# microsoft/UniVL

Measured on AMD Instinct MI355X. Metric: video-text pairs/sec (retrieval finetune, 48x48), higher is better.
Workload: dtype bf16; 1 GPU; YouCookII-shape retrieval finetune (FT-Joint) training step: BERT-base text encoder (12 L) + 6-layer visual encoder, max_words=48, max_frames=48, bs=4 per GPU, fwd+bwd+clip+BertAdam, dropout 0.10, random-init weights; kind=joint, per_gpu_batch=4, global_batch=4, max_words=48, max_frames=48, parallelism=dp1, hip_graph=True, graph_mode=whole, optimizer_pipelined=True, optimizer_riding=True, params=152602880

## Files before the change

### include/univl_hip.h

```cpp
#ifndef UNIVL_HIP_H
#define UNIVL_HIP_H
#include <stdint.h>

#ifdef __cplusplus
extern "C" {
#endif

#ifndef __HIP__
typedef struct ihipStream_t* hipStream_t;
#endif

#define UNIVL_DT_F32 0
#define UNIVL_DT_BF16 1

const char* univl_last_error(void);
int univl_version(void);
int univl_struct_size(int which);
int univl_device_info(int* cu_count, char* name, int name_len);
int univl_init(int device);
#define UNIVL_ZERO_MAX 16
int univl_zero_many(void* const* ptrs, const int64_t* bytes, int32_t n, hipStream_t stream);
int univl_copy_many(const void* const* srcs, void* const* dsts, const int64_t* bytes, int32_t n, hipStream_t stream);
int univl_destroy(void);
int univl_set_deterministic(int on);
int univl_get_deterministic(void);
int univl_allreduce_bucket(void* buf, size_t n, int dtype, int average, void* comm, hipStream_t side);

#define UNIVL_GEMM_ACCUM 1
#define UNIVL_GEMM_GELU_FWD 2
#define UNIVL_GEMM_GELU_BWD 4
#define UNIVL_GEMM_ATOMIC 8
#define UNIVL_GEMM_DBIAS_ATOMIC 16
#define UNIVL_GEMM_XCD_MAP 64
#define UNIVL_GEMM_PROBE_NOSTORE 128
#define UNIVL_GEMM_PROBE_NT_B 256
#define UNIVL_GEMM_AUX_F32 512
#define UNIVL_GEMM_NT_OUT 32
typedef struct UnivlGemm {
    int32_t dtype, trans_a, trans_b;
    int32_t M, N, K;
    const void* A; int64_t lda;
    const void* B; int64_t ldb;
    float* C32;
    void* C16;
    int64_t ldc;
    const float* bias;
    const float* R;
    int64_t ldr;
    void* aux;
    int64_t ldaux;
    float* dbias;
    float alpha;
    int32_t flags;
    int32_t ksplit;
    int32_t tile;
    float* sumsq; int32_t sumsq_rows; int32_t sumsq_stride;
    int32_t stages;
    int32_t waves;
    const void* A_lo; const void* B_lo; void* C16_lo;
} UnivlGemm;
int univl_gemm(const UnivlGemm* desc, hipStream_t stream);
#define UNIVL_GEMM_GROUP_MAX 4
int univl_gemm_group(const UnivlGemm* descs, int32_t n, hipStream_t stream);
int univl_gemm_group_limited(const UnivlGemm* d, int n, int max_blocks, hipStream_t stream);
int univl_gemm_pair(const UnivlGemm* dgrad, const UnivlGemm* wgrad, int32_t dry_run, hipStream_t stream);
int univl_gemm_tile_map(int32_t what, int32_t nx, int32_t ny, int32_t nz, int32_t gm, int32_t* out);

int univl_gemm256_layout(int32_t what, int32_t trans, int32_t idx, int32_t arg, int32_t* out);

typedef struct UnivlLayerNorm {
    int32_t dtype;
    int32_t rows, N;
    int32_t x_f64;
    const void* x;
    const float* residual;
    const float* pos;
    int32_t pos_period;
    const float* gamma; const float* beta;
    float eps;
    float* y;
    float* stats;
    float* out32;
    void* out16;
    float p_pre, p_post;
    uint64_t seed, off_pre, off_post;
    const uint64_t* seed_dev;
    const float* dout;
    float* dx32;
    float* dxd32;
    void* dxd16;
    float* dgamma; float* dbeta;
    float* dbias;
    float* dpos;
    void* out16_lo;
} UnivlLayerNorm;
int univl_layernorm_fwd(const UnivlLayerNorm* d, hipStream_t stream);
int univl_layernorm_bwd(const UnivlLayerNorm* d, hipStream_t stream);

typedef struct UnivlAttention {
    int32_t dtype;
    int32_t B, H, Sq, Sk;
    const void* q; int64_t ldq;
    const void* k; int64_t ldk;
    const void* v; int64_t ldv;
    const int64_t* key_mask;
    int32_t causal;
    void* out; int64_t ldo;
    float* lse;
    float p_drop; uint64_t seed, offset;
    const uint64_t* seed_dev;
    const void* dout; int64_t lddo;
    void* dq; int64_t lddq;
    void* dk; int64_t lddk;
    void* dv; int64_t lddv;
    int64_t bsk, bsv;
    void* out_lo;
} UnivlAttention;
int univl_attention_fwd(const UnivlAttention* d, hipStream_t stream);
int univl_attention_bwd(const UnivlAttention* d, hipStream_t stream);

int univl_attention_bwd_fused(const UnivlAttention* at, const UnivlGemm* odgrad, const UnivlGemm* owgrad, int32_t dry_run, hipStream_t stream);

int univl_attention_fwd_fused(const UnivlAttention* at, const UnivlGemm* qkv, const struct UnivlAdam* adam, int32_t chunk_begin,
                              int32_t chunk_count, int32_t max_blocks, int32_t dry_run, hipStream_t stream);

typedef struct UnivlEmbedText {
    int32_t dtype;
    int32_t B, S, N;
    const int64_t* ids; const int64_t* type_ids;
    const float* word; const float* pos; const float* type;
    const float* gamma; const float* beta; float eps;
    float* y; float* stats; float* out32; void* out16;
    float p_post; uint64_t seed, off_post;
    const uint64_t* seed_dev;
    const float* dout;
    float* dword; float* dpos; float* dtype_emb; float* dgamma; float* dbeta;
    float* drows;
    void* out16_lo;
} UnivlEmbedText;
int univl_embed_text_fwd(const UnivlEmbedText* d, hipStream_t stream);
int univl_embed_text_bwd(const UnivlEmbedText* d, hipStream_t stream);
int univl_rows_zero(float* table, int64_t rows_total, const int64_t* list, const int32_t* meta, hipStream_t stream);
int univl_rows_append(const int64_t* ids, int32_t n, int64_t* list, int32_t cap, int32_t* meta, int32_t reset, uint8_t* ever,
                      int64_t rows_total, hipStream_t stream);
int univl_rows_sumsq(const float* table, int64_t rows_total, const int64_t* list, const int32_t* meta, float* out, hipStream_t stream);
int univl_rows_gather_sum(const float* rows, int32_t n_rows, int32_t period, int32_t n, float* out, hipStream_t stream);
int univl_embed_scatter(const int64_t* ids, const float* rows, int64_t n, float scale, float* dword, hipStream_t stream);

typedef struct UnivlPool {
    int32_t B, S, N;
    const float* x; int64_t ldx_row;
    const int64_t* mask;
    int32_t skip_first, normalize;
    float* mean;
    float* out;
    const float* dout;
    float* dx;
    int32_t accumulate;
    const float* dsim; int64_t ldsim; const float* other; int32_t n_other; int32_t transpose; const float* gscale;
} UnivlPool;
int univl_pool_fwd(const UnivlPool* d, hipStream_t stream);
int univl_pool_bwd(const UnivlPool* d, hipStream_t stream);
int univl_pool_pair_fwd(const UnivlPool* a, const UnivlPool* b, hipStream_t stream);
int univl_pool_pair_bwd(const UnivlPool* a, const UnivlPool* b, hipStream_t stream);

int univl_maxmargin_loss(const float* sim, int32_t n, int32_t ld, float margin, const float* weight, float* loss,
                         float* dsim, hipStream_t stream);
int univl_crossen_loss(const float* sim, int32_t n, int32_t ld, float* loss, float* dsim, hipStream_t stream);
int univl_milnce_loss(const float* sim, int32_t batch_size, int32_t n_pair, int32_t ld, float* loss, float* dsim,
                      hipStream_t stream);
int univl_rank_counts(const float* sim, int32_t n, int64_t ld, int32_t* gt, int32_t* eq, hipStream_t stream);
int univl_scale_by_device_scalar(float* x, int64_t n, const float* s, hipStream_t stream);

int univl_pair_concat_fwd(const float* seq, const float* vis, const int64_t* amask, const int64_t* vmask,
                          const int32_t* tidx, const int32_t* vidx, int32_t P, int32_t W, int32_t F, float* out,
                          int64_t* out_mask, hipStream_t stream);
int univl_pair_concat_bwd(const float* dout, const int32_t* tidx, const int32_t* vidx, int32_t P, int32_t W, int32_t F,
                          float* dseq, float* dvis, hipStream_t stream);
int univl_postype_fwd(const float* pos, const float* type, int32_t W, int32_t S, float* out, hipStream_t stream);
int univl_postype_bwd(const float* dtable, int32_t W, int32_t S, float* dpos, float* dtype, hipStream_t stream);
int univl_tanh_fwd(const float* x, float* y, int64_t n, hipStream_t stream);
int univl_tanh_bwd(int32_t dtype, const float* dy, const float* y, void* dx, int64_t n, hipStream_t stream);
int univl_gelu_bwd(int32_t dtype, const float* dg, const void* u, void* du, int64_t n, hipStream_t stream);
int univl_colsum(int32_t dtype, const void* x, int64_t ld, int32_t rows, int32_t n, float* out, hipStream_t stream);
int univl_gather_rows(const void* src, void* dst, const int32_t* idx, int32_t rows, int64_t row_stride, int64_t copy_bytes,
                      hipStream_t stream);
int univl_log_softmax_rows(float* x, int32_t rows, int32_t n, int64_t ld, hipStream_t stream);
#define UNIVL_BEAM_MAX 8
#define UNIVL_BEAM_SLICES 8
typedef struct {
    const float* lp; int64_t ld;
    int32_t n_inst, n_bm, V;
    int32_t first_step;
    int32_t eos;
    const int32_t* eos_dev;
    int32_t t, Tmax;
    float* scores;
    uint8_t* done;
    int32_t* length;
    int64_t* tokens;
    int32_t* src;
    int32_t* hist_parents; int32_t* hist_tokens; float* hist_scores;
    void* ws; int64_t ws_bytes;
} UnivlBeamStep;
int univl_beam_step(const UnivlBeamStep* d, hipStream_t stream);
int univl_beam_backtrack(const int32_t* hist_parents, const int32_t* hist_tokens, const float* scores, const int32_t* length,
                         int32_t n_inst, int32_t n_bm, int32_t n_best, int32_t Tmax, int32_t* hyp, float* hyp_scores,
                         hipStream_t stream);
int univl_beam_captions(const int32_t* hyp, const int32_t* length, int32_t n_inst, int32_t n_best, int32_t Tmax, int32_t eos, int32_t pad,
                        const int32_t* eos_dev, int32_t* cap_tokens, int32_t* cap_len, hipStream_t stream);
#define UNIVL_TOPK_MAX 64
#define UNIVL_TOPK_SLICES_MAX 256
typedef struct UnivlSimTopk {
    const float* q; int64_t ldq;
    const float* g; int64_t ldg;
    int32_t Nq, Ng, H, k;
    int32_t slices;
    int32_t reserved;
    int32_t* idx; float* score;
    const int32_t* target;
    int32_t* gt; int32_t* eq;
    void* ws; int64_t ws_bytes;
} UnivlSimTopk;
int univl_sim_topk(const UnivlSimTopk* d, hipStream_t stream);
int64_t univl_sim_topk_workspace(int32_t Nq, int32_t Ng, int32_t k, int32_t slices);
int univl_sumsq_finish(const float* partials, const int32_t* seg, const int32_t* start, const int32_t* count, int32_t n,
                       float* out, hipStream_t stream);
int univl_scale_ct_by_device_scalar(int32_t dtype, void* x, int64_t n, const float* s, hipStream_t stream);
int univl_simdense_fwd(const float* x, const float* w, const float* b, int32_t rows, float* out, hipStream_t stream);
int univl_simdense_bwd(const float* ds, const float* x, const float* w, int32_t rows, float* dx, float* dw, float* db,
                       hipStream_t stream);
int univl_ce_loss(int32_t dtype, const float* logits, int64_t ld, const int64_t* labels, int32_t rows, int32_t V,
                  int32_t ignore_index, float* scratch2, float* loss, void* dlogits, int64_t lddl, hipStream_t stream);
typedef struct UnivlVocabCE {
    int32_t dtype, rows, V, K;
    const void* x; int64_t ldx;
    const void* table; int64_t ldt;
    const float* bias;
    const int64_t* labels;
    int32_t ignore_index, slots;
    float* partial;
    float* label_logit;
    float* lse;
    float* rowloss;
    float* scratch2;
    float* loss;
    const float* gout;
// ... 58 lines not shown
```

### univl_amd/_ab.py

```python
import os

KEYS = {
    "wgrad_ride": (1, "weight gradients ride in their dgrad's launch (univl_gemm_pair); 0: the layer's grouped launch"),
    "group_wgrad": (1, "a layer's non-riding weight gradients as ONE grouped launch; 0: one launch per member"),
    "pair_form": ("", "'square': round 2's 64 x 64 form of the pair launch"),
    "decoder_pair": (1, "pair launches in the decoder stack"),
    "splitk_tiles": (128, "split the contraction of the N = 768 products while the 64 x 64 output grid has fewer tiles than this"),
    "splitk_len": (384, "target slice depth of that split"),
    "splitk_maxwg": (512, "cap on tiles x slices of that split"),
    "splitk_dgrad_maxwg": (0, "cap on tiles x slices of the dgrad half of a pair launch (0: splitk_maxwg) -- so that dgrad + weight-gradient tiles fit one round of resident slots"),
    "splitk_target_wg": (180, "up to 48 output tiles (256 tokens): split the N = 768 products into round(target / tiles) slices of at least 256 (0: the splitk_len / splitk_maxwg policy of rounds 1-5)"),
    "splitk_target_wg_big": (264, "the same from 49 tiles up to splitk_tiles"),
    "ks_o_fwd": (0, "A/B: slices of the attention-output product (0: policy)"), "ks_ffn2_fwd": (0, "A/B: slices of the FFN2 forward product"),
    "ks_ffn1_dgrad": (0, "A/B: slices of the FFN1 dgrad"), "ks_qkv_dgrad": (0, "A/B: slices of the QKV dgrad"),
    "splitk_mid": (1, "three-slice split of the deep (K >= 2304) N = 768 products at 128 .. 255 tiles"),
    "splitk_mid_ks": (3, "slices of the deep (K >= 2304) N = 768 products in the splitk_mid regime up to 160 tiles"),
    "splitk_mid_ks_big": (2, "... from 161 tiles on"),
    "splitk_mid_ks_768": (1, "slices of the K = 768 N = 768 products in the splitk_mid regime"),
    "splitk_mid_tiles": (256, "upper tile bound of that regime"),
    "ln_fold": (1, "LayerNorm forward finished inside its product's launch (univl_gemm_ln) up to ln_fold_max_rows tokens"),
    "ln_fold_max_rows": (640, "... up to this many tokens (the library carries up to 1024).  Round 6, alternating on one box: 576 tokens 3.00 -> 2.92 ms (-2.6 %, both folds), 624 tokens -1.7 %, 672 +-0, 768 +0.5 % (profiles/r06u_ab_fold_768*.txt); rounds 4-5: 512"),
    "ln_fold_bwd": (1, "LayerNorm backward finished inside the dgrad pair launch (univl_gemm_pair_ln)"),
    "ln_fold_bwd_max": (640, "... up to this many tokens (383: round 4's range, the square pair form only)"),
    "wgrad_big_min": (0, "token count from which a layer's grouped weight gradients take the big tile (0: where every dgrad does)"),
    "attn_fuse_fwd": (1, "the q | k | v projection computed inside the attention forward launch (univl_attention_fwd_fused); 0: two launches"),
    "attn_fuse_bwd": (1, "the attention-output dgrad computed inside the attention backward launch (univl_attention_bwd_fused); 0: two launches"),
    "attn_fuse_fwd_max_seq": (64, "longest sequence the fused attention FORWARD launch is used for.  128: the round-6 form for 65 .. 128 positions (two workgroups per (batch row, head), bit-identical) -- measured NEUTRAL: caption 5.150 vs 5.150 ms, pretrain 9.09 vs 9.09, FT-Align 2.90 vs 2.90 with 18 launches fewer (profiles/r06t_ab_attn_big.txt), so the plans keep the two launches"),
    "attn_fuse_fwd_max_rows": (1536, "token count up to which the fused attention FORWARD launch is used (1536: -1.9 %, 3072: +0.7 %, profiles/r05ae)"),
    "attn_fuse_bwd_max_rows": (1535, "token count up to which the fused attention BACKWARD launch is used (1536: +1 %, 6144: +4.9 %)"),
    "g256": (1, "256 x 256 8-phase body (csrc/gemm256.h) for the grouped weight gradients / single products it is picked for; 0: the older tiles"),
    "g256_min_rows": (1536, "token count (a multiple of 256) from which the plans drop the pair launches for separate dgrads + the grouped 256-body launch"),
    "pairs": ("", "default of model.operand_pairs -- operand PAIRS (bf16 hi + lo, include/univl_hip.h: UnivlGemm.A_lo) in the encoder stacks' forward products: 'x' the activation operand, 'w' the weight operand, 'xw' both, '': plain bf16 operands"),
    "pairs_max_rows": (768, "... in stacks of at most this many tokens (16 pairs x 48): beyond, the matrix pipe is the bound and the extra terms cost step time"),
    "pairs_ks": ("same", "split of a paired N = 768 product: 'same' workgroup count as the plain product (slices nterm x as deep) | 'terms': every term cut like the plain product"),
    "gelu_pre_f32": (0, "A/B measurement: the FFN1 pre-activation saved for GELU' in fp32 instead of the compute type (encoder stacks)"),
    "vocab_ce": (1, "K16: the vocabulary classifier with the online log-softmax CE in its epilogue (univl_vocab_ce_fwd / _bwd: no [tokens, 30522] logits in training); 0: product -> logits -> univl_ce_loss"),
    "vocab_dgrad_split": (1, "split-K of the vocabulary dgrad (caption / pretrain heads)"),
    "fused_sim": (1, "pooling + similarity + loss heads as fused launches up to 256 rows"),
    "dpos_gather_min": (32, "rows per position from which position-table gradients are gathered instead of scatter-added"),
    "beam_step": (1, "caption decoding: Beam.advance as the device-side tail of each position's plan (univl_beam_step) -- CaptionBeamSearch's default beam_step='device'; 0: 'host', the ATen top-k / where path with one host read per position (the comparand)"),
    "adam_ride": ("1", "BertAdam chunks ride with the next forward's products; '0': side-stream form; 'force': one graph even with a captured exchange"),
    "tail_ride": (1, "chunks of cross layer 0 / decoder layer 0 ride in the last text / video layer's products; 0: launched in front of the forward"),
    "adam_lazy_rows": (1, "weight-decay-only shortcut for word-table rows that never had a gradient"),
    "adam_chunk": (0, "A/B: elements per workgroup of the BertAdam update (0: optimization.CHUNK = 8192)"),
    "adam_blocks": (0, "grid cap of the overlapped (non-riding) update"),
    "pipeline_opt": (0, "experimental pipelined optimizer"),
    "async_loss": (0, "experimental asynchronous loss read-back"),
    "fused_norms": (1, "gradient norms from the weight-gradient epilogues"),
    "sparse_rows": (1, "sparse bookkeeping of the word-table gradient"),
    "sparse_emb": (1, "sparse exchange of the word-table gradient under data parallelism"),
    "copy_kernel": (1, "input staging / loss hand-off as one copy kernel"),
    "auto_graph": (1, "the unchanged training loop switches to graph replay on its own"),
    "auto_dp": (1, "wrap in the bucketed reducer on its own when torch.distributed is initialised"),
    "dp_capture": (1, "capture the RCCL exchange into the step graph"),
    "dp_dryrun": (0, "measurement: the data-parallel schedule with the collectives not enqueued"),
    "stamps": (0, "device timestamps between the nodes of the step"),
    "probe_skip": ("", "a stack (bert | visual | cross) without its layer kernels"),
    "probe_no_ln": ("", "fwd | bwd | both: the encoder LayerNorm launches left out"),
    "poison": (0, "workspaces filled with NaN patterns"),
    "guard": (0, "guard words around workspaces"),
}

_allowed = False
_parsed = None
_legacy_checked = False

OPERATIONAL = {"auto_graph": "model.auto_graph = False", "auto_dp": "model.auto_dp = False", "dp_capture": "model.dp_capture = False",
               "adam_ride": "model.auto_ride = False"}


def _check_legacy():
    global _legacy_checked
    if _legacy_checked:
        return
    _legacy_checked = True
    for k in KEYS:
        name = "UNIVL_" + k.upper()
        if name in os.environ:
            how = ("set `%s` on the model (or UNIVL_AB=%s=... in a measurement harness)" % (OPERATIONAL[k], k)) if k in OPERATIONAL \
                else ("use UNIVL_AB=%s=... (measurement / test harnesses only)" % k)
            raise RuntimeError("%s is set but no longer read (it would be silently ignored): %s" % (name, how))


def allow():
    global _allowed
    _allowed = True


def _parse():
    global _parsed
    _check_legacy()
    raw = os.environ.get("UNIVL_AB", "")
    if _parsed is not None and _parsed[0] == raw:
        return _parsed[1]
    out = {}
    for item in [x for x in raw.split(",") if x.strip()]:
        if "=" not in item:
            raise RuntimeError("UNIVL_AB: expected key=value, got %r" % item)
        k, v = (s.strip() for s in item.split("=", 1))
        if k not in KEYS:
            raise RuntimeError("UNIVL_AB: unknown key %r (known: %s)" % (k, ", ".join(sorted(KEYS))))
        d = KEYS[k][0]
        out[k] = type(d)(v) if not isinstance(d, int) else int(v)
    if out and not _allowed:
        raise RuntimeError("UNIVL_AB=%r is set, but this process is not a measurement or test harness (univl_amd._ab.allow()): "
                           "A/B overrides of the plan builder are refused in training / evaluation runs" % raw)
    _parsed = (raw, out)
    return out


def get(key):
    if key not in KEYS:
        raise KeyError("univl_amd._ab: unknown key %r" % key)
    return _parse().get(key, KEYS[key][0])


def overrides():
    return dict(_parse())
```

### univl_amd/_lib.py

```python
import ctypes as C
import os

_HERE = os.path.dirname(os.path.abspath(__file__))
LIB_PATH = os.environ.get("UNIVL_LIB") or os.path.join(_HERE, "lib", "libunivl_hip.so")

DT_F32, DT_BF16 = 0, 1
GEMM_ACCUM, GEMM_GELU_FWD, GEMM_GELU_BWD, GEMM_DBIAS_ATOMIC, GEMM_NT_OUT, GEMM_AUX_F32 = 1, 2, 4, 16, 32, 512
GEMM_GROUP_MAX = 4
EUNSUPPORTED = -3

vp, i32, i64, f32, u64 = C.c_void_p, C.c_int32, C.c_int64, C.c_float, C.c_uint64


class Gemm(C.Structure):
    _fields_ = [("dtype", i32), ("trans_a", i32), ("trans_b", i32), ("M", i32), ("N", i32), ("K", i32),
                ("A", vp), ("lda", i64), ("B", vp), ("ldb", i64), ("C32", vp), ("C16", vp), ("ldc", i64),
                ("bias", vp), ("R", vp), ("ldr", i64), ("aux", vp), ("ldaux", i64), ("dbias", vp),
                ("alpha", f32), ("flags", i32), ("ksplit", i32), ("tile", i32), ("sumsq", vp), ("sumsq_rows", i32), ("sumsq_stride", i32),
                ("stages", i32), ("waves", i32), ("A_lo", vp), ("B_lo", vp), ("C16_lo", vp)]


class LayerNorm(C.Structure):
    _fields_ = [("dtype", i32), ("rows", i32), ("N", i32), ("x_f64", i32), ("x", vp), ("residual", vp),
                ("pos", vp), ("pos_period", i32), ("gamma", vp), ("beta", vp), ("eps", f32), ("y", vp),
                ("stats", vp), ("out32", vp), ("out16", vp), ("p_pre", f32), ("p_post", f32), ("seed", u64),
                ("off_pre", u64), ("off_post", u64), ("seed_dev", vp), ("dout", vp), ("dx32", vp), ("dxd32", vp), ("dxd16", vp),
                ("dgamma", vp), ("dbeta", vp), ("dbias", vp), ("dpos", vp), ("out16_lo", vp)]


class Attention(C.Structure):
    _fields_ = [("dtype", i32), ("B", i32), ("H", i32), ("Sq", i32), ("Sk", i32), ("q", vp), ("ldq", i64),
                ("k", vp), ("ldk", i64), ("v", vp), ("ldv", i64), ("key_mask", vp), ("causal", i32),
                ("out", vp), ("ldo", i64), ("lse", vp), ("p_drop", f32), ("seed", u64), ("offset", u64), ("seed_dev", vp),
                ("dout", vp), ("lddo", i64), ("dq", vp), ("lddq", i64), ("dk", vp), ("lddk", i64),
                ("dv", vp), ("lddv", i64), ("bsk", i64), ("bsv", i64), ("out_lo", vp)]


class EmbedText(C.Structure):
    _fields_ = [("dtype", i32), ("B", i32), ("S", i32), ("N", i32), ("ids", vp), ("type_ids", vp), ("word", vp),
                ("pos", vp), ("type", vp), ("gamma", vp), ("beta", vp), ("eps", f32), ("y", vp), ("stats", vp),
                ("out32", vp), ("out16", vp), ("p_post", f32), ("seed", u64), ("off_post", u64), ("seed_dev", vp), ("dout", vp),
                ("dword", vp), ("dpos", vp), ("dtype_emb", vp), ("dgamma", vp), ("dbeta", vp), ("drows", vp), ("out16_lo", vp)]


class Pool(C.Structure):
    _fields_ = [("B", i32), ("S", i32), ("N", i32), ("x", vp), ("ldx_row", i64), ("mask", vp),
                ("skip_first", i32), ("normalize", i32), ("mean", vp), ("out", vp), ("dout", vp), ("dx", vp), ("accumulate", i32),
                ("dsim", vp), ("ldsim", i64), ("other", vp), ("n_other", i32), ("transpose", i32), ("gscale", vp)]


class Seg(C.Structure):
    _fields_ = [("offset", i64), ("numel", i64), ("lr", f32), ("weight_decay", f32), ("max_grad_norm", f32),
                ("active", i32)]


class Adam(C.Structure):
    _fields_ = [("p", vp), ("g", vp), ("m", vp), ("v", vp), ("p16", vp), ("segs", vp), ("nseg", i32),
                ("chunk_seg", vp), ("chunk_off", vp), ("chunk_len", vp), ("nchunk", i32), ("sumsq", vp),
                ("coef", vp), ("step", vp), ("b1", f32), ("b2", f32), ("eps", f32), ("warmup", f32),
                ("t_total", i32), ("seg_scalars", vp), ("schedule", i32), ("row_flags", vp), ("flag_seg", i32), ("row_len", i32), ("p16_lo", vp)]


class VocabCE(C.Structure):
    _fields_ = [("dtype", i32), ("rows", i32), ("V", i32), ("K", i32), ("x", vp), ("ldx", i64), ("table", vp), ("ldt", i64), ("bias", vp),
                ("labels", vp), ("ignore_index", i32), ("slots", i32), ("partial", vp), ("label_logit", vp), ("lse", vp), ("rowloss", vp),
                ("scratch2", vp), ("loss", vp), ("gout", vp), ("dlogits", vp), ("lddl", i64)]


class BeamStep(C.Structure):
    _fields_ = [("lp", vp), ("ld", i64), ("n_inst", i32), ("n_bm", i32), ("V", i32), ("first_step", i32), ("eos", i32), ("eos_dev", vp),
                ("t", i32), ("Tmax", i32), ("scores", vp), ("done", vp), ("length", vp), ("tokens", vp), ("src", vp), ("hist_parents", vp),
                ("hist_tokens", vp), ("hist_scores", vp), ("ws", vp), ("ws_bytes", i64)]


class SimTopk(C.Structure):
    _fields_ = [("q", vp), ("ldq", i64), ("g", vp), ("ldg", i64), ("Nq", i32), ("Ng", i32), ("H", i32), ("k", i32), ("slices", i32),
                ("reserved", i32), ("idx", vp), ("score", vp), ("target", vp), ("gt", vp), ("eq", vp), ("ws", vp), ("ws_bytes", i64)]


BEAM_MAX, BEAM_SLICES = 8, 8
TOPK_MAX, TOPK_SLICES_MAX = 64, 256

_STRUCTS = [Gemm, LayerNorm, Attention, EmbedText, Pool, Seg, Adam, VocabCE, BeamStep, SimTopk]
_lib = None


def available():
    return os.path.exists(LIB_PATH)


def lib():
    global _lib
    if _lib is not None:
        return _lib
    if not os.path.exists(LIB_PATH):
        raise RuntimeError("libunivl_hip.so not found at %s -- run `python -c 'import __graft_entry__ as g; "
                           "g.build()'` (hipcc --offload-arch=gfx950).  univl_amd has no CPU fallback." % LIB_PATH)
    L = C.CDLL(LIB_PATH)
    L.univl_last_error.restype = C.c_char_p
    L.univl_struct_size.argtypes = [i32]
    for k, st in enumerate(_STRUCTS):
        n = L.univl_struct_size(k)
        if n != C.sizeof(st):
            raise RuntimeError("ABI mismatch for %s: library %d bytes, ctypes %d" % (st.__name__, n, C.sizeof(st)))
    for name in ("univl_vocab_ce_fwd", "univl_vocab_ce_bwd", "univl_gemm", "univl_layernorm_fwd", "univl_layernorm_bwd", "univl_attention_fwd",
                 "univl_attention_bwd", "univl_embed_text_fwd", "univl_embed_text_bwd", "univl_pool_fwd",
                 "univl_pool_bwd", "univl_bert_adam", "univl_beam_step", "univl_sim_topk"):
        getattr(L, name).argtypes = [vp, vp]
        getattr(L, name).restype = i32
    L.univl_pool_pair_fwd.argtypes = [vp, vp, vp]
    L.univl_pool_pair_bwd.argtypes = [vp, vp, vp]
    L.univl_gemm_group.argtypes = [vp, i32, vp]
    L.univl_gemm_group.restype = i32
    L.univl_gemm_group_limited.argtypes = [vp, i32, i32, vp]
    L.univl_gemm_pair.argtypes = [vp, vp, i32, vp]
    L.univl_gemm_rider.argtypes = [vp, vp, i32, i32, i32, vp]
    L.univl_gemm_rider_prime.argtypes = [vp]
    L.univl_gemm_rider_fits.argtypes = [vp]
    L.univl_gemm_ln.argtypes = [vp, vp, vp, vp, i32, i32, i32, i32, vp]
    L.univl_gemm_ln.restype = i32
    L.univl_gemm_pair_ln.argtypes = [vp, vp, vp, vp, i32, vp]
    L.univl_gemm_pair_ln.restype = i32
    L.univl_gemm_tile_map.argtypes = [i32, i32, i32, i32, i32, C.POINTER(i32)]
    L.univl_embed_scatter.argtypes = [vp, vp, i64, f32, vp, vp]
    L.univl_rows_gather_sum.argtypes = [vp, i32, i32, i32, vp, vp]
    L.univl_rows_zero.argtypes = [vp, i64, vp, vp, vp]
    L.univl_rows_append.argtypes = [vp, i32, vp, i32, vp, i32, vp, i64, vp]
    L.univl_rows_sumsq.argtypes = [vp, i64, vp, vp, vp, vp]
    L.univl_zero_many.argtypes = [vp, vp, i32, vp]
    L.univl_copy_many.argtypes = [vp, vp, vp, i32, vp]
    L.univl_maxmargin_loss.argtypes = [vp, i32, i32, f32, vp, vp, vp, vp]
    L.univl_crossen_loss.argtypes = [vp, i32, i32, vp, vp, vp]
    L.univl_milnce_loss.argtypes = [vp, i32, i32, i32, vp, vp, vp]
    L.univl_gather_rows.argtypes = [vp, vp, vp, i32, i64, i64, vp]
    L.univl_log_softmax_rows.argtypes = [vp, i32, i32, i64, vp]
    L.univl_beam_backtrack.argtypes = [vp, vp, vp, vp, i32, i32, i32, i32, vp, vp, vp]
    L.univl_beam_backtrack.restype = i32
    L.univl_beam_captions.argtypes = [vp, vp, i32, i32, i32, i32, i32, vp, vp, vp, vp]
    L.univl_beam_captions.restype = i32
    L.univl_rank_counts.argtypes = [vp, i32, i64, vp, vp, vp]
    L.univl_sim_topk_workspace.argtypes = [i32, i32, i32, i32]
    L.univl_sim_topk_workspace.restype = i64
    L.univl_scale_by_device_scalar.argtypes = [vp, i64, vp, vp]
    L.univl_pair_concat_fwd.argtypes = [vp, vp, vp, vp, vp, vp, i32, i32, i32, vp, vp, vp]
    L.univl_pair_concat_bwd.argtypes = [vp, vp, vp, i32, i32, i32, vp, vp, vp]
    L.univl_postype_fwd.argtypes = [vp, vp, i32, i32, vp, vp]
    L.univl_postype_bwd.argtypes = [vp, i32, i32, vp, vp, vp]
    L.univl_tanh_fwd.argtypes = [vp, vp, i64, vp]
    L.univl_tanh_bwd.argtypes = [i32, vp, vp, vp, i64, vp]
    L.univl_gelu_bwd.argtypes = [i32, vp, vp, vp, i64, vp]
    L.univl_colsum.argtypes = [i32, vp, i64, i32, i32, vp, vp]
    L.univl_scale_ct_by_device_scalar.argtypes = [i32, vp, i64, vp, vp]
    L.univl_simdense_fwd.argtypes = [vp, vp, vp, i32, vp, vp]
    L.univl_simdense_bwd.argtypes = [vp, vp, vp, i32, vp, vp, vp, vp]
    L.univl_ce_loss.argtypes = [i32, vp, i64, vp, i32, i32, i32, vp, vp, vp, i64, vp]
    L.univl_mfm_nce_loss.argtypes = [vp, i64, vp, vp, i32, vp, vp, vp, i64, vp]
    L.univl_grad_sumsq.argtypes = [vp, vp, i32, vp, vp, vp, i32, vp, vp]
    L.univl_sumsq_finish.argtypes = [vp, vp, vp, vp, i32, vp, vp]
    L.univl_clip_coef.argtypes = [vp, vp, i32, f32, vp, vp]
    L.univl_scale_grads.argtypes = [vp, vp, vp, vp, vp, i32, vp, vp]
    L.univl_cast_bf16.argtypes = [vp, vp, i64, vp]
    L.univl_cast_bf16_pair.argtypes = [vp, vp, vp, i64, vp]
    L.univl_cast_f32.argtypes = [vp, vp, i64, vp]
    L.univl_bert_adam_range.argtypes = [vp, i32, i32, i32, i32, vp]
    L.univl_bump_counter.argtypes = [vp, vp]
    L.univl_probe_layouts.argtypes = [vp, i32, vp]
    L.univl_stamp.argtypes = [vp, vp]
    L.univl_device_info.argtypes = [C.POINTER(i32), C.c_char_p, i32]
    L.univl_init.argtypes = [i32]
    L.univl_allreduce_bucket.argtypes = [vp, C.c_size_t, i32, i32, vp, vp]
    L.univl_set_deterministic.argtypes = [i32]
    _lib = L
    return L


def deterministic():
    return bool(lib().univl_get_deterministic())


def set_deterministic(on=True):
    check(lib().univl_set_deterministic(1 if on else 0), "set_deterministic")


EXPORTED = ["univl_last_error", "univl_version", "univl_struct_size", "univl_device_info", "univl_init", "univl_destroy",
            "univl_allreduce_bucket", "univl_set_deterministic", "univl_get_deterministic", "univl_gemm", "univl_gemm_group_limited", "univl_gemm_group", "univl_gemm_tile_map", "univl_gemm256_layout", "univl_gemm_pair", "univl_gemm_rider", "univl_gemm_rider_fits", "univl_gemm_rider_prime", "univl_gemm_ln", "univl_gemm_pair_ln",
            "univl_layernorm_fwd", "univl_layernorm_bwd", "univl_attention_fwd", "univl_attention_bwd", "univl_attention_bwd_fused", "univl_attention_fwd_fused",
            "univl_embed_text_fwd", "univl_embed_text_bwd", "univl_embed_scatter", "univl_rows_gather_sum", "univl_rows_zero", "univl_rows_append",
            "univl_rows_sumsq", "univl_zero_many", "univl_copy_many", "univl_pool_fwd", "univl_pool_bwd", "univl_pool_pair_fwd", "univl_pool_pair_bwd",
            "univl_maxmargin_loss", "univl_crossen_loss", "univl_milnce_loss", "univl_rank_counts", "univl_sim_topk", "univl_sim_topk_workspace", "univl_gather_rows", "univl_log_softmax_rows", "univl_beam_step", "univl_beam_backtrack", "univl_beam_captions", "univl_scale_by_device_scalar", "univl_pair_concat_fwd", "univl_pair_concat_bwd", "univl_postype_fwd", "univl_postype_bwd", "univl_tanh_fwd",
            "univl_tanh_bwd", "univl_gelu_bwd", "univl_colsum", "univl_scale_ct_by_device_scalar", "univl_simdense_fwd", "univl_simdense_bwd", "univl_ce_loss", "univl_vocab_ce_fwd", "univl_vocab_ce_bwd", "univl_mfm_nce_loss", "univl_grad_sumsq", "univl_sumsq_finish",
            "univl_clip_coef", "univl_scale_grads", "univl_bert_adam", "univl_bert_adam_range", "univl_cast_bf16", "univl_cast_bf16_pair", "univl_cast_f32", "univl_bump_counter", "univl_probe_layouts", "univl_stamp"]


def check(rc, what=""):
    if rc != 0:
        raise RuntimeError("libunivl_hip %s failed (%d): %s" % (what, rc, lib().univl_last_error().decode()))
```

### univl_amd/csrc/embed.hip

```cpp
#include "common.h"
#include "univl_hip.h"

namespace {

constexpr int N = 768;
constexpr int NV = N / 256;

template <typename TO>
__global__ __launch_bounds__(256) void embed_fwd_kernel(UnivlEmbedText p) {
    const int lane = threadIdx.x & 63, wave = threadIdx.x >> 6;
    const int row = blockIdx.x * 4 + wave;
    if (row >= p.B * p.S) return;
    const int s = row % p.S;
    const long id = p.ids[row];
    const long tt = (p.type && p.type_ids) ? p.type_ids[row] : 0;
    float v[NV][4];
#pragma unroll
    for (int j = 0; j < NV; ++j) {
        const int col = 4 * lane + 256 * j;
        const float4 a = *reinterpret_cast<const float4*>(p.word + id * N + col);
        const float4 b = *reinterpret_cast<const float4*>(p.pos + (long)s * N + col);
        v[j][0] = a.x + b.x; v[j][1] = a.y + b.y; v[j][2] = a.z + b.z; v[j][3] = a.w + b.w;
        if (p.type) {
            const float4 c = *reinterpret_cast<const float4*>(p.type + tt * N + col);
            v[j][0] += c.x; v[j][1] += c.y; v[j][2] += c.z; v[j][3] += c.w;
        }
        if (p.y) *reinterpret_cast<float4*>(p.y + (long)row * N + col) = make_float4(v[j][0], v[j][1], v[j][2], v[j][3]);
    }
    float sm = 0.f;
#pragma unroll
    for (int j = 0; j < NV; ++j) sm += (v[j][0] + v[j][1]) + (v[j][2] + v[j][3]);
    const float mean = wave_sum(sm) * (1.0f / N);
    float q = 0.f;
#pragma unroll
    for (int j = 0; j < NV; ++j)
#pragma unroll
        for (int e = 0; e < 4; ++e) { const float c = v[j][e] - mean; q += c * c; }
    const float rstd = 1.0f / sqrtf(wave_sum(q) * (1.0f / N) + p.eps);
    if (p.stats && lane == 0) { p.stats[2 * (long)row] = mean; p.stats[2 * (long)row + 1] = rstd; }
    const uint64_t* sp = p.seed_dev ? p.seed_dev : reinterpret_cast<const uint64_t*>(p.gamma);
    const uint64_t sdv = *sp;
    const uint64_t seed = p.seed + (p.seed_dev ? sdv : 0ull);
    const float inv_keep = p.p_post > 0.f ? 1.0f / (1.0f - p.p_post) : 1.0f;
#pragma unroll
    for (int j = 0; j < NV; ++j) {
        const int col = 4 * lane + 256 * j;
        const long o = (long)row * N + col;
        const float4 ga = *reinterpret_cast<const float4*>(p.gamma + col);
        const float4 be = *reinterpret_cast<const float4*>(p.beta + col);
        float r[4];
        r[0] = (v[j][0] - mean) * rstd * ga.x + be.x;
        r[1] = (v[j][1] - mean) * rstd * ga.y + be.y;
        r[2] = (v[j][2] - mean) * rstd * ga.z + be.z;
        r[3] = (v[j][3] - mean) * rstd * ga.w + be.w;
        if (p.p_post > 0.f) {
#pragma unroll
            for (int e = 0; e < 4; ++e) r[e] *= dropout_scale(seed, p.off_post, (uint64_t)(o + e), p.p_post, inv_keep);
        }
        if (p.out32) *reinterpret_cast<float4*>(p.out32 + o) = make_float4(r[0], r[1], r[2], r[3]);
        if (p.out16) {
            TO* d = reinterpret_cast<TO*>(p.out16) + o;
            if (sizeof(TO) == 2) {
                bf16x4_t w;
                w[0] = (__bf16)r[0]; w[1] = (__bf16)r[1]; w[2] = (__bf16)r[2]; w[3] = (__bf16)r[3];
                *reinterpret_cast<bf16x4_t*>(d) = w;
                if (p.out16_lo) {
                    bf16x4_t l;
                    l[0] = (__bf16)(r[0] - (float)w[0]); l[1] = (__bf16)(r[1] - (float)w[1]);
                    l[2] = (__bf16)(r[2] - (float)w[2]); l[3] = (__bf16)(r[3] - (float)w[3]);
                    *reinterpret_cast<bf16x4_t*>(reinterpret_cast<TO*>(p.out16_lo) + o) = l;
                }
            } else {
                *reinterpret_cast<float4*>(d) = make_float4(r[0], r[1], r[2], r[3]);
            }
        }
    }
}

template <bool DET = false>
__global__ __launch_bounds__(256) void embed_bwd_kernel(UnivlEmbedText p, float* det_part = nullptr, int* det_counter = nullptr) {
    __shared__ float red[4][N];
    const int lane = threadIdx.x & 63, wave = threadIdx.x >> 6;
    const int row = blockIdx.x * 4 + wave;
    const bool valid = row < p.B * p.S;
    float dgm[NV][4], dbt[NV][4], dxs[NV][4];
    int row_type = -1;
#pragma unroll
    for (int j = 0; j < NV; ++j)
#pragma unroll
        for (int e = 0; e < 4; ++e) { dgm[j][e] = 0.f; dbt[j][e] = 0.f; dxs[j][e] = 0.f; }
    if (valid) {
        const int s = row % p.S;
        const long id = p.ids[row];
        const long tt = (p.dtype_emb && p.type_ids) ? p.type_ids[row] : 0;
        const float mean = p.stats[2 * (long)row], rstd = p.stats[2 * (long)row + 1];
        const uint64_t* sp = p.seed_dev ? p.seed_dev : reinterpret_cast<const uint64_t*>(p.gamma);
    const uint64_t sdv = *sp;
    const uint64_t seed = p.seed + (p.seed_dev ? sdv : 0ull);
    const float inv_keep = p.p_post > 0.f ? 1.0f / (1.0f - p.p_post) : 1.0f;
        float dy[NV][4], xh[NV][4], ga[NV][4];
        float s1 = 0.f, s2 = 0.f;
#pragma unroll
        for (int j = 0; j < NV; ++j) {
            const int col = 4 * lane + 256 * j;
            const long o = (long)row * N + col;
            const float4 a = *reinterpret_cast<const float4*>(p.dout + o);
            const float4 yy = *reinterpret_cast<const float4*>(p.y + o);
            const float4 gg = *reinterpret_cast<const float4*>(p.gamma + col);
            dy[j][0] = a.x; dy[j][1] = a.y; dy[j][2] = a.z; dy[j][3] = a.w;
            ga[j][0] = gg.x; ga[j][1] = gg.y; ga[j][2] = gg.z; ga[j][3] = gg.w;
            xh[j][0] = (yy.x - mean) * rstd; xh[j][1] = (yy.y - mean) * rstd;
            xh[j][2] = (yy.z - mean) * rstd; xh[j][3] = (yy.w - mean) * rstd;
#pragma unroll
            for (int e = 0; e < 4; ++e) {
                if (p.p_post > 0.f) dy[j][e] *= dropout_scale(seed, p.off_post, (uint64_t)(o + e), p.p_post, inv_keep);
                const float gq = dy[j][e] * ga[j][e];
                s1 += gq; s2 += gq * xh[j][e];
                dgm[j][e] = dy[j][e] * xh[j][e];
                dbt[j][e] = dy[j][e];
            }
        }
        s1 = wave_sum(s1) * (1.0f / N);
        s2 = wave_sum(s2) * (1.0f / N);
#pragma unroll
        for (int j = 0; j < NV; ++j) {
            const int col = 4 * lane + 256 * j;
#pragma unroll
            for (int e = 0; e < 4; ++e) {
                const float dx = rstd * (dy[j][e] * ga[j][e] - s1 - xh[j][e] * s2);
                if (p.drows) p.drows[(long)row * N + col + e] = dx;
                else unsafeAtomicAdd(p.dword + id * N + col + e, dx);
                if (!DET && p.dpos) unsafeAtomicAdd(p.dpos + (long)s * N + col + e, dx);
                if (p.dtype_emb && tt > 1) unsafeAtomicAdd(p.dtype_emb + tt * N + col + e, dx);
                dxs[j][e] = dx;
            }
        }
        row_type = (int)tt;
    }
    if constexpr (DET) {
        __shared__ int last_flag;
        const long nb = gridDim.x;
#pragma unroll
        for (int t = 0; t < 2; ++t) {
            __syncthreads();
#pragma unroll
            for (int j = 0; j < NV; ++j)
#pragma unroll
                for (int e = 0; e < 4; ++e) red[wave][4 * lane + 256 * j + e] = t == 0 ? dgm[j][e] : dbt[j][e];
            __syncthreads();
            float* slot = det_part + ((long)t * nb + blockIdx.x) * N;
            for (int c = threadIdx.x; c < N; c += 256) slot[c] = (red[0][c] + red[1][c]) + (red[2][c] + red[3][c]);
        }
        if (det_last_block(det_counter, (int)nb, &last_flag)) {
#pragma unroll
            for (int t = 0; t < 2; ++t) {
                float* dst = t == 0 ? p.dgamma : p.dbeta;
                for (int c = threadIdx.x; c < N; c += 256) {
                    const float* q = det_part + (long)t * nb * N + c;
                    float acc = 0.f;
                    for (long b = 0; b < nb; ++b) acc += q[b * N];
                    dst[c] += acc;
                }
            }
        }
// ... 19 lines not shown

}

extern "C" int univl_embed_text_fwd(const UnivlEmbedText* d, hipStream_t stream) {
    UNIVL_ON_STREAM_DEVICE(stream);
    UNIVL_CHECK_ARG(d != nullptr, UNIVL_EINVAL, "univl_embed_text_fwd: null descriptor");
    UNIVL_CHECK_ARG(d->N == 768, UNIVL_EUNSUPPORTED, "univl_embed_text_fwd: N=%d (768 supported)", d->N);
    UNIVL_CHECK_ARG(d->B > 0 && d->S > 0 && d->ids && d->word && d->pos && d->gamma && d->beta && (d->out32 || d->out16),
                    UNIVL_EINVAL, "univl_embed_text_fwd: null / empty argument");
    dim3 grid((d->B * d->S + 3) / 4), block(256);
    if (d->dtype == UNIVL_DT_BF16) hipLaunchKernelGGL((embed_fwd_kernel<__bf16>), grid, block, 0, stream, *d);
    else hipLaunchKernelGGL((embed_fwd_kernel<float>), grid, block, 0, stream, *d);
    UNIVL_LAUNCH_CHECK();
    return UNIVL_OK;
}

namespace {
__global__ __launch_bounds__(256) void embed_scatter_det_kernel(const int64_t* ids, const float* rows, long n, float scale, float* dword) {
    const long t = blockIdx.x;
    const int64_t id = ids[t];
    int dup = 0;
    for (long j = threadIdx.x; j < t; j += 256) dup |= (ids[j] == id) ? 1 : 0;
    if (__syncthreads_or(dup)) return;
    float acc[NV] = {0.f, 0.f, 0.f};
    for (long u = t; u < n; ++u) {
        if (ids[u] != id) continue;
#pragma unroll
        for (int j = 0; j < NV; ++j) acc[j] += rows[u * N + threadIdx.x + 256 * j] * scale;
    }
#pragma unroll
    for (int j = 0; j < NV; ++j) dword[id * N + threadIdx.x + 256 * j] += acc[j];
}

__global__ __launch_bounds__(256) void embed_dpos_gather_kernel(const float* rows, int B, int S, float* dpos) {
    const long i = (long)blockIdx.x * 256 + threadIdx.x;
    if (i >= (long)S * N) return;
    const int s = (int)(i / N), c = (int)(i % N);
    float acc = 0.f;
    for (int b = 0; b < B; ++b) acc += rows[((long)b * S + s) * N + c];
    dpos[i] += acc;
}

__global__ __launch_bounds__(256) void embed_dtype_gather_kernel(const int64_t* type_ids, const float* rows, long n, float* dtype_emb) {
    const int c = blockIdx.x * 256 + threadIdx.x, k = blockIdx.y;
    float acc = 0.f;
    for (long t = 0; t < n; ++t) {
        const int64_t tt = type_ids ? type_ids[t] : 0;
        if (tt == k) acc += rows[t * N + c];
    }
    if (acc != 0.0f) dtype_emb[(long)k * N + c] += acc;
}

__global__ __launch_bounds__(256) void embed_scatter_kernel(const int64_t* ids, const float* rows, float scale, float* dword) {
    const long t = blockIdx.x;
    const long id = ids[t];
    for (int c = threadIdx.x; c < N; c += 256) unsafeAtomicAdd(dword + id * N + c, rows[t * N + c] * scale);
}
}

extern "C" int univl_embed_scatter(const int64_t* ids, const float* rows, int64_t n, float scale, float* dword, hipStream_t stream) {
    UNIVL_ON_STREAM_DEVICE(stream);
    UNIVL_CHECK_ARG(ids && rows && dword && n > 0, UNIVL_EINVAL, "univl_embed_scatter: bad argument");
    if (univl_deterministic()) hipLaunchKernelGGL(embed_scatter_det_kernel, dim3((unsigned)n), dim3(256), 0, stream, ids, rows, (long)n, scale, dword);
    else hipLaunchKernelGGL(embed_scatter_kernel, dim3((unsigned)n), dim3(256), 0, stream, ids, rows, scale, dword);
    UNIVL_LAUNCH_CHECK();
    return UNIVL_OK;
}

namespace {
constexpr int ROWS_GRID = 8192;

__global__ __launch_bounds__(256) void rows_zero_kernel(float* table, long rows_total, const int64_t* list, const int* meta) {
    const int n = meta[0], over = meta[1];
    if (!over && (int)blockIdx.x >= n) return;
    for (long r = over ? blockIdx.x : list[blockIdx.x]; r < rows_total; r += ROWS_GRID) {
        float4* p = reinterpret_cast<float4*>(table + r * N);
        for (int c = threadIdx.x; c < N / 4; c += 256) p[c] = float4{0.f, 0.f, 0.f, 0.f};
        if (!over) break;
    }
}

__global__ __launch_bounds__(256) void rows_append_kernel(const int64_t* ids, int n, int64_t* list, int cap, int* meta, int reset,
                                                          uint8_t* ever, long rows_total) {
    __shared__ int base, over;
    if (threadIdx.x == 0) {
        const int cur = reset ? 0 : meta[0];
        int ov = reset ? 0 : meta[1];
        if (cur + n > cap) ov = 1;
        base = cur; over = ov;
        meta[1] = ov;
        meta[0] = ov ? cur : cur + n;
    }
    __syncthreads();
    if (!over) for (int i = threadIdx.x; i < n; i += 256) list[base + i] = ids[i];
    if (ever) {
        if (over) for (long r = threadIdx.x; r < rows_total; r += 256) ever[r] = 1;
        else for (int i = threadIdx.x; i < n; i += 256) ever[ids[i]] = 1;
    }
}

__global__ __launch_bounds__(256) void rows_sumsq_kernel(const float* table, long rows_total, const int64_t* list, const int* meta,
                                                         float* out, float* det_part) {
    __shared__ float red[4];
    const int n = meta[0], over = meta[1];
    if (!over && (int)blockIdx.x >= n) { if (det_part && threadIdx.x == 0) det_part[blockIdx.x] = 0.f; return; }
    float acc = 0.f;
    if (over) {
        for (long r = blockIdx.x; r < rows_total; r += ROWS_GRID) {
            const float4* p = reinterpret_cast<const float4*>(table + r * N);
            for (int c = threadIdx.x; c < N / 4; c += 256) { const float4 v = p[c]; acc += (v.x * v.x + v.y * v.y) + (v.z * v.z + v.w * v.w); }
        }
    } else {
        const int64_t r = list[blockIdx.x];
        int dup = 0;
        for (int j = threadIdx.x; j < (int)blockIdx.x; j += 256) dup |= (list[j] == r) ? 1 : 0;
        if (__syncthreads_or(dup)) { if (det_part && threadIdx.x == 0) det_part[blockIdx.x] = 0.f; return; }
        const float4* p = reinterpret_cast<const float4*>(table + r * N);
        for (int c = threadIdx.x; c < N / 4; c += 256) { const float4 v = p[c]; acc += (v.x * v.x + v.y * v.y) + (v.z * v.z + v.w * v.w); }
    }
    acc = wave_sum(acc);
    if ((threadIdx.x & 63) == 0) red[threadIdx.x >> 6] = acc;
    __syncthreads();
    if (threadIdx.x == 0) {
        const float s = (red[0] + red[1]) + (red[2] + red[3]);
        if (det_part) det_part[blockIdx.x] = s;
        else unsafeAtomicAdd(out, s);
    }
}

__global__ __launch_bounds__(256) void rows_sumsq_finish_kernel(const float* part, int n, float* out) {
    __shared__ float red[4];
    float acc = 0.f;
    for (int i = threadIdx.x; i < n; i += 256) acc += part[i];
    acc = wave_sum(acc);
    if ((threadIdx.x & 63) == 0) red[threadIdx.x >> 6] = acc;
    __syncthreads();
    if (threadIdx.x == 0) out[0] += (red[0] + red[1]) + (red[2] + red[3]);
}
}

extern "C" int univl_rows_zero(float* table, int64_t rows_total, const int64_t* list, const int32_t* meta, hipStream_t stream) {
    UNIVL_ON_STREAM_DEVICE(stream);
    UNIVL_CHECK_ARG(table && list && meta && rows_total > 0 && aligned16(table), UNIVL_EINVAL, "univl_rows_zero: bad argument");
    hipLaunchKernelGGL(rows_zero_kernel, dim3(ROWS_GRID), dim3(256), 0, stream, table, (long)rows_total, list, meta);
    UNIVL_LAUNCH_CHECK();
    return UNIVL_OK;
}

extern "C" int univl_rows_append(const int64_t* ids, int32_t n, int64_t* list, int32_t cap, int32_t* meta, int32_t reset,
                                 uint8_t* ever, int64_t rows_total, hipStream_t stream) {
    UNIVL_ON_STREAM_DEVICE(stream);
    UNIVL_CHECK_ARG(ids && list && meta && n > 0 && cap > 0 && cap <= ROWS_GRID && (!ever || rows_total > 0), UNIVL_EINVAL,
                    "univl_rows_append: bad argument (cap <= %d)", ROWS_GRID);
    hipLaunchKernelGGL(rows_append_kernel, dim3(1), dim3(256), 0, stream, ids, n, list, cap, meta, reset, ever, (long)rows_total);
    UNIVL_LAUNCH_CHECK();
    return UNIVL_OK;
}

extern "C" int univl_rows_sumsq(const float* table, int64_t rows_total, const int64_t* list, const int32_t* meta, float* out,
                                hipStream_t stream) {
    UNIVL_ON_STREAM_DEVICE(stream);
    UNIVL_CHECK_ARG(table && list && meta && out && rows_total > 0 && aligned16(table), UNIVL_EINVAL, "univl_rows_sumsq: bad argument");
    float* part = nullptr;
    if (univl_deterministic()) {
        part = static_cast<float*>(univl_det_alloc(ROWS_GRID * sizeof(float)));
        if (!part) return UNIVL_EINVAL;
    }
    hipLaunchKernelGGL(rows_sumsq_kernel, dim3(ROWS_GRID), dim3(256), 0, stream, table, (long)rows_total, list, meta, out, part);
    if (part) hipLaunchKernelGGL(rows_sumsq_finish_kernel, dim3(1), dim3(256), 0, stream, part, ROWS_GRID, out);
    UNIVL_LAUNCH_CHECK();
    return UNIVL_OK;
}

extern "C" int univl_embed_text_bwd(const UnivlEmbedText* d, hipStream_t stream) {
    UNIVL_ON_STREAM_DEVICE(stream);
    UNIVL_CHECK_ARG(d != nullptr, UNIVL_EINVAL, "univl_embed_text_bwd: null descriptor");
    UNIVL_CHECK_ARG(d->N == 768, UNIVL_EUNSUPPORTED, "univl_embed_text_bwd: N=%d (768 supported)", d->N);
    UNIVL_CHECK_ARG(d->B > 0 && d->S > 0 && d->ids && d->dout && d->y && d->stats && d->gamma && d->dword && (d->dpos || d->drows) &&
                        d->dgamma && d->dbeta,
                    UNIVL_EINVAL, "univl_embed_text_bwd: null / empty argument");
    dim3 grid((d->B * d->S + 3) / 4), block(256);
    if (univl_deterministic()) {
        UnivlEmbedText q = *d;
        const long T = (long)d->B * d->S;
        float* part = static_cast<float*>(univl_det_alloc((size_t)2 * grid.x * N * sizeof(float)));
        int* counter = univl_det_counter();
        if (!part || !counter) return UNIVL_EINVAL;
        if (!q.drows) {
            q.drows = static_cast<float*>(univl_det_alloc((size_t)T * N * sizeof(float)));
            if (!q.drows) return UNIVL_EINVAL;
        }
        hipLaunchKernelGGL(embed_bwd_kernel<true>, grid, block, 0, stream, q, part, counter);
        if (!d->drows)
            hipLaunchKernelGGL(embed_scatter_det_kernel, dim3((unsigned)T), block, 0, stream, d->ids, q.drows, T, 1.0f, d->dword);
        if (d->dpos)
            hipLaunchKernelGGL(embed_dpos_gather_kernel, dim3((unsigned)(((long)d->S * N + 255) / 256)), block, 0, stream, q.drows, d->B, d->S, d->dpos);
        if (d->dtype_emb)
            hipLaunchKernelGGL(embed_dtype_gather_kernel, dim3(N / 256, 2), block, 0, stream, d->type_ids, q.drows, T, d->dtype_emb);
        UNIVL_LAUNCH_CHECK();
        return UNIVL_OK;
    }
    hipLaunchKernelGGL(embed_bwd_kernel<false>, grid, block, 0, stream, *d);
    UNIVL_LAUNCH_CHECK();
    return UNIVL_OK;
}
```

### univl_amd/csrc/misc.hip

```cpp
#include <stdarg.h>
#include <stdio.h>
#include <string.h>
#include <dlfcn.h>
#include <stdlib.h>
#include "common.h"
#include "univl_hip.h"

static thread_local char g_err[512] = "";

void univl_set_error(const char* fmt, ...) {
    va_list ap;
    va_start(ap, fmt);
    vsnprintf(g_err, sizeof(g_err), fmt, ap);
    va_end(ap);
}

extern "C" const char* univl_last_error(void) { return g_err; }
extern "C" int univl_version(void) { return 100; }

extern "C" int univl_struct_size(int which) {
    switch (which) {
        case 0: return (int)sizeof(UnivlGemm);
        case 1: return (int)sizeof(UnivlLayerNorm);
        case 2: return (int)sizeof(UnivlAttention);
        case 3: return (int)sizeof(UnivlEmbedText);
        case 4: return (int)sizeof(UnivlPool);
        case 5: return (int)sizeof(UnivlSeg);
        case 6: return (int)sizeof(UnivlAdam);
        case 7: return (int)sizeof(UnivlVocabCE);
        case 8: return (int)sizeof(UnivlBeamStep);
        case 9: return (int)sizeof(UnivlSimTopk);
        default: return -1;
    }
}

extern "C" int univl_device_info(int* cu_count, char* name, int name_len) {
    int dev = 0;
    hipError_t e = hipGetDevice(&dev);
    if (e != hipSuccess) { univl_set_error("hipGetDevice: %s", hipGetErrorString(e)); return (int)e; }
    hipDeviceProp_t prop;
    e = hipGetDeviceProperties(&prop, dev);
    if (e != hipSuccess) { univl_set_error("hipGetDeviceProperties: %s", hipGetErrorString(e)); return (int)e; }
    if (cu_count) *cu_count = prop.multiProcessorCount;
    if (name && name_len > 0) { strncpy(name, prop.gcnArchName, name_len - 1); name[name_len - 1] = 0; }
    return 0;
}

#include <mutex>
namespace {
struct DetArena { unsigned char* base = nullptr; size_t size = 0, head = 0; int* counters = nullptr; int next_counter = 0; };
constexpr int DET_COUNTERS = 1 << 16;
DetArena g_det[UNIVL_MAX_DEVICES];
std::mutex g_det_mutex;
int g_deterministic = 0;

DetArena* det_arena() {
    int dev = 0;
    if (hipGetDevice(&dev) != hipSuccess || dev < 0 || dev >= UNIVL_MAX_DEVICES) return nullptr;
    DetArena& a = g_det[dev];
    if (a.base == nullptr) {
        const char* e = getenv("UNIVL_DET_ARENA_MB");
        const size_t mb = e ? (size_t)atol(e) : 1024;
        void* p = nullptr;
        void* c = nullptr;
        if (hipMalloc(&p, mb << 20) != hipSuccess) { (void)hipGetLastError(); return nullptr; }
        if (hipMalloc(&c, DET_COUNTERS * sizeof(int)) != hipSuccess || hipMemset(c, 0, DET_COUNTERS * sizeof(int)) != hipSuccess ||
            hipDeviceSynchronize() != hipSuccess) {
            (void)hipGetLastError(); (void)hipFree(p); if (c) (void)hipFree(c); return nullptr;
        }
        a.base = static_cast<unsigned char*>(p); a.size = mb << 20; a.head = 0;
        a.counters = static_cast<int*>(c); a.next_counter = 0;
    }
    return &a;
}
}

bool univl_deterministic() { return g_deterministic != 0; }

void* univl_det_alloc(size_t bytes) {
    std::lock_guard<std::mutex> lock(g_det_mutex);
    DetArena* a = det_arena();
    bytes = (bytes + 255) & ~(size_t)255;
    if (a == nullptr || bytes > a->size / 4) {
        univl_set_error("deterministic mode: no scratch ring on this device (call univl_set_deterministic(1) on it outside a stream "
                        "capture; a single request must fit a quarter of UNIVL_DET_ARENA_MB), %zu bytes asked", bytes);
        return nullptr;
    }
    if (a->head + bytes > a->size) a->head = 0;
    void* p = a->base + a->head;
    a->head += bytes;
    return p;
}

int* univl_det_counter() {
    std::lock_guard<std::mutex> lock(g_det_mutex);
    DetArena* a = det_arena();
    if (a == nullptr) { univl_set_error("deterministic mode: no counter pool on this device"); return nullptr; }
    int* c = a->counters + a->next_counter;
    a->next_counter = (a->next_counter + 1) % DET_COUNTERS;
    return c;
}

extern "C" int univl_set_deterministic(int on) {
    std::lock_guard<std::mutex> lock(g_det_mutex);
    g_deterministic = on ? 1 : 0;
    if (on && det_arena() == nullptr) {
        univl_set_error("univl_set_deterministic: cannot allocate the scratch ring (UNIVL_DET_ARENA_MB) on the current device");
        return UNIVL_EINVAL;
    }
    return UNIVL_OK;
}

extern "C" int univl_get_deterministic(void) { return g_deterministic; }

namespace {
struct ZeroList { unsigned char* ptr[UNIVL_ZERO_MAX]; long bytes[UNIVL_ZERO_MAX]; };
__global__ __launch_bounds__(256) void zero_many_kernel(ZeroList z) {
    unsigned char* p = z.ptr[blockIdx.y];
    const long n16 = z.bytes[blockIdx.y] >> 4;
    u32x4_t* q = reinterpret_cast<u32x4_t*>(p);
    for (long i = (long)blockIdx.x * 256 + threadIdx.x; i < n16; i += (long)gridDim.x * 256) q[i] = u32x4_t{0u, 0u, 0u, 0u};
    if (blockIdx.x == 0) for (long i = (n16 << 4) + threadIdx.x; i < z.bytes[blockIdx.y]; i += 256) p[i] = 0;
}
}

extern "C" int univl_zero_many(void* const* ptrs, const int64_t* bytes, int32_t n, hipStream_t stream) {
    UNIVL_ON_STREAM_DEVICE(stream);
    UNIVL_CHECK_ARG(ptrs && bytes && n >= 1 && n <= UNIVL_ZERO_MAX, UNIVL_EINVAL, "univl_zero_many: n=%d (1..%d)", n, UNIVL_ZERO_MAX);
    ZeroList z;
    long most = 0;
    for (int i = 0; i < n; ++i) {
        UNIVL_CHECK_ARG(ptrs[i] && bytes[i] > 0 && aligned16(ptrs[i]), UNIVL_EALIGN, "univl_zero_many: buffer %d must be non-empty and 16-byte aligned", i);
        z.ptr[i] = static_cast<unsigned char*>(ptrs[i]);
        z.bytes[i] = bytes[i];
        most = bytes[i] > most ? bytes[i] : most;
    }
    long gx = (most / 16 + 2047) / 2048;
    gx = gx < 1 ? 1 : (gx > 1024 ? 1024 : gx);
    hipLaunchKernelGGL(zero_many_kernel, dim3((unsigned)gx, n), dim3(256), 0, stream, z);
    UNIVL_LAUNCH_CHECK();
    return UNIVL_OK;
}

namespace {
struct CopyList { const unsigned char* src[UNIVL_ZERO_MAX]; unsigned char* dst[UNIVL_ZERO_MAX]; long bytes[UNIVL_ZERO_MAX]; };
__global__ __launch_bounds__(256) void copy_many_kernel(CopyList c) {
    const unsigned char* s = c.src[blockIdx.y];
    unsigned char* d = c.dst[blockIdx.y];
    const long nb = c.bytes[blockIdx.y];
    const bool vec = ((((uintptr_t)s) | ((uintptr_t)d)) & 15) == 0;
    const long n16 = vec ? (nb >> 4) : 0;
    const u32x4_t* sv = reinterpret_cast<const u32x4_t*>(s);
    u32x4_t* dv = reinterpret_cast<u32x4_t*>(d);
    for (long i = (long)blockIdx.x * 256 + threadIdx.x; i < n16; i += (long)gridDim.x * 256) dv[i] = sv[i];
    if (blockIdx.x == 0) for (long i = (n16 << 4) + threadIdx.x; i < nb; i += 256) d[i] = s[i];
}
}

extern "C" int univl_copy_many(const void* const* srcs, void* const* dsts, const int64_t* bytes, int32_t n, hipStream_t stream) {
    UNIVL_ON_STREAM_DEVICE(stream);
    UNIVL_CHECK_ARG(srcs && dsts && bytes && n >= 1 && n <= UNIVL_ZERO_MAX, UNIVL_EINVAL, "univl_copy_many: n=%d (1..%d)", n, UNIVL_ZERO_MAX);
    CopyList c;
    long most = 0;
    for (int i = 0; i < n; ++i) {
        UNIVL_CHECK_ARG(srcs[i] && dsts[i] && bytes[i] > 0, UNIVL_EINVAL, "univl_copy_many: buffer %d is null or empty", i);
        c.src[i] = static_cast<const unsigned char*>(srcs[i]);
        c.dst[i] = static_cast<unsigned char*>(dsts[i]);
        c.bytes[i] = bytes[i];
        most = bytes[i] > most ? bytes[i] : most;
    }
    for (int i = n; i < UNIVL_ZERO_MAX; ++i) { c.src[i] = c.src[0]; c.dst[i] = c.dst[0]; c.bytes[i] = 0; }
    long gx = (most / 16 + 1023) / 1024;
    gx = gx < 1 ? 1 : (gx > 2048 ? 2048 : gx);
    hipLaunchKernelGGL(copy_many_kernel, dim3((unsigned)gx, n), dim3(256), 0, stream, c);
    UNIVL_LAUNCH_CHECK();
    return UNIVL_OK;
}

extern "C" int univl_init(int device) {
    int n = 0;
    hipError_t e = hipGetDeviceCount(&n);
    if (e != hipSuccess) { univl_set_error("hipGetDeviceCount: %s", hipGetErrorString(e)); return (int)e; }
    UNIVL_CHECK_ARG(device >= 0 && device < n, UNIVL_EINVAL, "univl_init: device %d of %d", device, n);
    hipDeviceProp_t prop;
    e = hipGetDeviceProperties(&prop, device);
    if (e != hipSuccess) { univl_set_error("hipGetDeviceProperties: %s", hipGetErrorString(e)); return (int)e; }
    UNIVL_CHECK_ARG(strncmp(prop.gcnArchName, "gfx950", 6) == 0, UNIVL_EUNSUPPORTED,
                    "univl_init: device %d is %s; libunivl_hip holds gfx950 (MI355X) code only", device, prop.gcnArchName);
    return UNIVL_OK;
}

typedef int (*nccl_allreduce_fn)(const void*, void*, size_t, int, int, void*, hipStream_t);
static void* g_rccl_handle = nullptr;
static nccl_allreduce_fn g_allreduce = nullptr;

extern "C" int univl_destroy(void) {
    {
        std::lock_guard<std::mutex> lock(g_det_mutex);
        for (DetArena& a : g_det) {
            if (a.base) (void)hipFree(a.base);
            if (a.counters) (void)hipFree(a.counters);
            a = DetArena();
        }
    }
    g_allreduce = nullptr;
    if (g_rccl_handle) { dlclose(g_rccl_handle); g_rccl_handle = nullptr; }
    return UNIVL_OK;
}

extern "C" int univl_allreduce_bucket(void* buf, size_t n, int dtype, int average, void* comm, hipStream_t side) {
    UNIVL_ON_STREAM_DEVICE(side);
    UNIVL_CHECK_ARG(buf && comm && n > 0 && (dtype == UNIVL_F32 || dtype == UNIVL_BF16), UNIVL_EINVAL,
                    "univl_allreduce_bucket: bad argument");
    if (!g_allreduce) {
        void* sym = dlsym(RTLD_DEFAULT, "ncclAllReduce");
        if (!sym) {
            for (const char* name : {"librccl.so.1", "librccl.so", "/opt/rocm/lib/librccl.so.1"}) {
                g_rccl_handle = dlopen(name, RTLD_NOW | RTLD_LOCAL);
                if (g_rccl_handle) break;
            }
            if (g_rccl_handle) sym = dlsym(g_rccl_handle, "ncclAllReduce");
        }
// ... 78 lines not shown
```

### univl_amd/csrc/simloss.hip

```cpp
#include "common.h"
#include "univl_hip.h"

namespace {

__device__ __forceinline__ float block_sum(float v, float* red) {
    v = wave_sum(v);
    const int lane = threadIdx.x & 63, wave = threadIdx.x >> 6;
    __syncthreads();
    if (lane == 0) red[wave] = v;
    __syncthreads();
    return (red[0] + red[1]) + (red[2] + red[3]);
}
__device__ __forceinline__ float block_max(float v, float* red) {
    v = wave_max(v);
    const int lane = threadIdx.x & 63, wave = threadIdx.x >> 6;
    __syncthreads();
    if (lane == 0) red[wave] = v;
    __syncthreads();
    return fmaxf(fmaxf(red[0], red[1]), fmaxf(red[2], red[3]));
}

constexpr int PN = 768, PC = PN / 256;

__device__ __forceinline__ float pool_weight(const UnivlPool& p, int b, int s) {
    float w = p.mask ? (float)p.mask[(long)b * p.S + s] : 1.0f;
    if (p.skip_first && s == 0) w = 0.0f;
    return w;
}

constexpr int PCHUNK = 256;

__device__ __forceinline__ float stage_weights(const UnivlPool& p, int b, int s0, float* wts, float* red) {
    const int s = s0 + threadIdx.x;
    const float w = (s < p.S) ? pool_weight(p, b, s) : 0.0f;
    wts[threadIdx.x] = w;
    return block_sum(w, red);
}

__device__ __forceinline__ void pool_fwd_body(const UnivlPool& p, const int b, float* red, float* wts) {
    const int t = threadIdx.x;
    float acc[PC] = {0.f, 0.f, 0.f};
    float cnt = 0.f;
    for (int s0 = 0; s0 < p.S; s0 += PCHUNK) {
        cnt += stage_weights(p, b, s0, wts, red);
        const int n = min(PCHUNK, p.S - s0);
        const float* x = p.x + ((long)b * p.S + s0) * p.ldx_row + t;
#pragma unroll 8
        for (int s = 0; s < n; ++s) {
            const float w = wts[s];
#pragma unroll
            for (int j = 0; j < PC; ++j) {
                const float v = x[(long)s * p.ldx_row + 256 * j];
                acc[j] += (w != 0.0f) ? v * w : 0.0f;
            }
        }
        __syncthreads();
    }
    if (!p.skip_first && cnt == 0.0f) cnt = 1.0f;
    float sq = 0.f;
#pragma unroll
    for (int j = 0; j < PC; ++j) { acc[j] /= cnt; sq += acc[j] * acc[j]; }
    float inv = 1.0f;
    if (p.normalize) inv = 1.0f / fmaxf(sqrtf(block_sum(sq, red)), 1e-12f);
#pragma unroll
    for (int j = 0; j < PC; ++j) {
        if (p.mean) p.mean[(long)b * PN + t + 256 * j] = acc[j];
        p.out[(long)b * PN + t + 256 * j] = acc[j] * inv;
    }
}

__global__ __launch_bounds__(256) void pool_fwd_kernel(UnivlPool p) {
    __shared__ float red[4];
    __shared__ float wts[PCHUNK];
    pool_fwd_body(p, blockIdx.x, red, wts);
}

__global__ __launch_bounds__(256) void pool_pair_fwd_kernel(UnivlPool a, UnivlPool b) {
    __shared__ float red[4];
    __shared__ float wts[PCHUNK];
    if ((int)blockIdx.x < a.B) pool_fwd_body(a, blockIdx.x, red, wts);
    else pool_fwd_body(b, (int)blockIdx.x - a.B, red, wts);
}

__device__ __forceinline__ void pool_bwd_body(const UnivlPool& p, const int b, const int chunk, float* red, float* wts, float* mine) {
    const int t = threadIdx.x;
    if (chunk * PCHUNK >= p.S) return;
    float cnt = 0.f;
    for (int s0 = 0; s0 < p.S; s0 += PCHUNK) {
        cnt += stage_weights(p, b, s0, wts, red);
        if (s0 == chunk * PCHUNK) mine[t] = wts[t];
        __syncthreads();
    }
    if (!p.skip_first && cnt == 0.0f) cnt = 1.0f;
    float m[PC], d[PC];
    float sq = 0.f, dot = 0.f;
#pragma unroll
    for (int j = 0; j < PC; ++j) {
        m[j] = p.mean[(long)b * PN + t + 256 * j];
        d[j] = p.dsim ? 0.0f : p.dout[(long)b * PN + t + 256 * j];
    }
    if (p.dsim) {
        const float gs = p.gscale ? p.gscale[0] : 1.0f;
        for (int k = 0; k < p.n_other; ++k) {
            const float w = p.transpose ? p.dsim[(long)k * p.ldsim + b] : p.dsim[(long)b * p.ldsim + k];
#pragma unroll
            for (int j = 0; j < PC; ++j) d[j] += w * p.other[(long)k * PN + t + 256 * j];
        }
#pragma unroll
        for (int j = 0; j < PC; ++j) d[j] *= gs;
    }
#pragma unroll
    for (int j = 0; j < PC; ++j) {
        sq += m[j] * m[j];
        dot += m[j] * d[j];
    }
    if (p.normalize) {
        const float nrm = fmaxf(sqrtf(block_sum(sq, red)), 1e-12f);
        const float dd = block_sum(dot, red) / (nrm * nrm);
#pragma unroll
        for (int j = 0; j < PC; ++j) d[j] = (d[j] - m[j] * dd) / nrm;
    }
    const float inv_cnt = 1.0f / cnt;
    const int s0 = chunk * PCHUNK, n = min(PCHUNK, p.S - s0);
    float* dx = p.dx + ((long)b * p.S + s0) * PN + t;
    if (p.accumulate) {
        constexpr int UB = 8;
        for (int s0b = 0; s0b < n; s0b += UB) {
            float old[UB][PC];
#pragma unroll
            for (int u = 0; u < UB; ++u) {
                const int s = min(s0b + u, n - 1);
#pragma unroll
                for (int j = 0; j < PC; ++j) old[u][j] = dx[(long)s * PN + 256 * j];
            }
#pragma unroll
            for (int u = 0; u < UB; ++u) {
                const int s = s0b + u;
                if (s < n) {
                    const float w = mine[s] * inv_cnt;
#pragma unroll
                    for (int j = 0; j < PC; ++j) dx[(long)s * PN + 256 * j] = old[u][j] + d[j] * w;
                }
            }
        }
    } else {
#pragma unroll 4
        for (int s = 0; s < n; ++s) {
            const float w = mine[s] * inv_cnt;
#pragma unroll
            for (int j = 0; j < PC; ++j) dx[(long)s * PN + 256 * j] = d[j] * w;
        }
    }
}

__global__ __launch_bounds__(256) void pool_bwd_kernel(UnivlPool p) {
    __shared__ float red[4];
    __shared__ float wts[PCHUNK];
    __shared__ float mine[PCHUNK];
    pool_bwd_body(p, blockIdx.x, blockIdx.y, red, wts, mine);
}

__global__ __launch_bounds__(256) void pool_pair_bwd_kernel(UnivlPool a, UnivlPool b) {
    __shared__ float red[4];
    __shared__ float wts[PCHUNK];
    __shared__ float mine[PCHUNK];
    if ((int)blockIdx.x < a.B) pool_bwd_body(a, blockIdx.x, blockIdx.y, red, wts, mine);
    else pool_bwd_body(b, (int)blockIdx.x - a.B, blockIdx.y, red, wts, mine);
}

__global__ __launch_bounds__(256) void maxmargin_kernel(const float* x, int n, int ld, float margin, const float* w,
                                                        float* loss, float* dx) {
    extern __shared__ float diag_acc[];
    __shared__ float red[4];
    const float inv = 1.0f / ((float)n * (float)n);
    for (int i = threadIdx.x; i < n; i += 256) diag_acc[i] = 0.f;
    __syncthreads();
    float acc = 0.f;
    for (int e = threadIdx.x; e < n * n; e += 256) {
        const int i = e / n, j = e % n;
        const float v = x[(long)i * ld + j], wi = w ? w[e] : 1.0f;
        const float a = margin + v - x[(long)i * ld + i];
        const float b = margin + v - x[(long)j * ld + j];
        float g = 0.f;
        if (a > 0.f) { acc += wi * a; g += wi; atomicAdd(&diag_acc[i], -wi); }
        if (b > 0.f) { acc += wi * b; g += wi; atomicAdd(&diag_acc[j], -wi); }
        dx[(long)i * ld + j] = g * inv;
    }
    const float total = block_sum(acc, red);
    if (threadIdx.x == 0) loss[0] = total * inv;
    __syncthreads();
    for (int i = threadIdx.x; i < n; i += 256) dx[(long)i * ld + i] += diag_acc[i] * inv;
}

__global__ __launch_bounds__(256) void crossen_kernel(const float* x, int n, int ld, float* loss, float* dx) {
    __shared__ float red[4];
    float total = 0.f;
    for (int i = 0; i < n; ++i) {
        float mx = -INFINITY;
        for (int j = threadIdx.x; j < n; j += 256) mx = fmaxf(mx, x[(long)i * ld + j]);
        mx = block_max(mx, red);
        float s = 0.f;
        for (int j = threadIdx.x; j < n; j += 256) s += expf(x[(long)i * ld + j] - mx);
        s = block_sum(s, red);
        const float lse = mx + logf(s);
        total += lse - x[(long)i * ld + i];
        for (int j = threadIdx.x; j < n; j += 256)
            dx[(long)i * ld + j] = (expf(x[(long)i * ld + j] - lse) - (i == j ? 1.0f : 0.0f)) / (float)n;
    }
    if (threadIdx.x == 0) loss[0] = total / (float)n;
}

__global__ __launch_bounds__(256) void milnce_kernel(const float* x, int bs, int np, int ld, float* loss, float* dx) {
    __shared__ float red[4];
    const int n = bs * np;
    for (int e = threadIdx.x; e < n * n; e += 256) dx[(long)(e / n) * ld + (e % n)] = 0.f;
    __syncthreads();
    float total = 0.f;
    for (int bb = 0; bb < bs; ++bb) {
        const int i = bb * np + np / 2;
        const int lo = bb * np, hi = lo + np;
        float mx = -INFINITY;
        for (int j = threadIdx.x; j < 2 * n; j += 256) {
            float v;
            if (j < n) v = x[(long)j * ld + i];
            else { const int jj = j - n; v = (jj >= lo && jj < hi) ? -INFINITY : x[(long)i * ld + jj]; }
            mx = fmaxf(mx, v);
        }
        mx = block_max(mx, red);
        float sden = 0.f, snum = 0.f;
        for (int j = threadIdx.x; j < 2 * n; j += 256) {
            if (j < n) {
                const float e = expf(x[(long)j * ld + i] - mx);
                sden += e;
                if (j >= lo && j < hi) snum += e;
            } else {
                const int jj = j - n;
                if (!(jj >= lo && jj < hi)) sden += expf(x[(long)i * ld + jj] - mx);
            }
        }
        sden = block_sum(sden, red);
        snum = block_sum(snum, red);
        total += logf(sden) - logf(snum);
        const float wgt = 1.0f / (float)bs;
        __syncthreads();
        for (int j = threadIdx.x; j < 2 * n; j += 256) {
            if (j < n) {
                const float e = expf(x[(long)j * ld + i] - mx);
                float g = e / sden;
                if (j >= lo && j < hi) g -= e / snum;
                dx[(long)j * ld + i] += wgt * g;
            }
        }
        __syncthreads();
        for (int j = threadIdx.x; j < n; j += 256) {
            if (!(j >= lo && j < hi)) dx[(long)i * ld + j] += wgt * expf(x[(long)i * ld + j] - mx) / sden;
        }
        __syncthreads();
    }
    if (threadIdx.x == 0) loss[0] = total / (float)bs;
}

__global__ void scale_dev_kernel(float* x, long n, const float* s) {
    const float k = s[0];
    for (long i = (long)blockIdx.x * 256 + threadIdx.x; i < n; i += (long)gridDim.x * 256) x[i] *= k;
}

}

extern "C" int univl_scale_by_device_scalar(float* x, int64_t n, const float* s, hipStream_t stream) {
    UNIVL_ON_STREAM_DEVICE(stream);
    UNIVL_CHECK_ARG(x && s && n > 0, UNIVL_EINVAL, "univl_scale_by_device_scalar: bad argument");
    long blocks = (n + 255) / 256;
    if (blocks > 1024) blocks = 1024;
    hipLaunchKernelGGL(scale_dev_kernel, dim3((unsigned)blocks), dim3(256), 0, stream, x, (long)n, s);
    UNIVL_LAUNCH_CHECK();
    return UNIVL_OK;
}

__global__ __launch_bounds__(256) void rank_counts_kernel(const float* x, int n, long ld, int* gt, int* eq) {
    __shared__ int red[8];
    const int i = blockIdx.x, t = threadIdx.x;
    const float* row = x + (long)i * ld;
    const float d = row[i];
    int g = 0, e = 0;
    for (int j = t; j < n; j += 256) {
        const float v = row[j];
        g += v > d ? 1 : 0;
        e += v == d ? 1 : 0;
    }
#pragma unroll
    for (int o = 32; o > 0; o >>= 1) { g += __shfl_down(g, o, 64); e += __shfl_down(e, o, 64); }
    if ((t & 63) == 0) { red[t >> 6] = g; red[4 + (t >> 6)] = e; }
    __syncthreads();
    if (t == 0) {
        gt[i] = (red[0] + red[1]) + (red[2] + red[3]);
        eq[i] = (red[4] + red[5]) + (red[6] + red[7]);
    }
}

extern "C" int univl_rank_counts(const float* sim, int32_t n, int64_t ld, int32_t* gt, int32_t* eq, hipStream_t stream) {
    UNIVL_ON_STREAM_DEVICE(stream);
    UNIVL_CHECK_ARG(sim && gt && eq && n > 0 && ld >= n, UNIVL_EINVAL, "univl_rank_counts: bad argument");
    hipLaunchKernelGGL(rank_counts_kernel, dim3(n), dim3(256), 0, stream, sim, n, (long)ld, gt, eq);
    UNIVL_LAUNCH_CHECK();
    return UNIVL_OK;
}

extern "C" int univl_pool_fwd(const UnivlPool* d, hipStream_t stream) {
    UNIVL_ON_STREAM_DEVICE(stream);
    UNIVL_CHECK_ARG(d && d->N == 768 && d->B > 0 && d->S > 0 && d->x && d->out, UNIVL_EINVAL, "univl_pool_fwd: bad argument (N must be 768)");
    hipLaunchKernelGGL(pool_fwd_kernel, dim3(d->B), dim3(256), 0, stream, *d);
    UNIVL_LAUNCH_CHECK();
    return UNIVL_OK;
}

static int pool_bwd_check(const UnivlPool* d, const char* who) {
    UNIVL_CHECK_ARG(d && d->N == 768 && d->B > 0 && d->S > 0 && d->mean && d->dx && (d->dout || (d->dsim && d->other && d->n_other > 0)),
                    UNIVL_EINVAL, "%s: bad argument", who);
    return UNIVL_OK;
}

extern "C" int univl_pool_bwd(const UnivlPool* d, hipStream_t stream) {
    UNIVL_ON_STREAM_DEVICE(stream);
    const int rc = pool_bwd_check(d, "univl_pool_bwd");
    if (rc) return rc;
    hipLaunchKernelGGL(pool_bwd_kernel, dim3(d->B, (d->S + PCHUNK - 1) / PCHUNK), dim3(256), 0, stream, *d);
    UNIVL_LAUNCH_CHECK();
    return UNIVL_OK;
}

extern "C" int univl_pool_pair_fwd(const UnivlPool* a, const UnivlPool* b, hipStream_t stream) {
    UNIVL_ON_STREAM_DEVICE(stream);
    UNIVL_CHECK_ARG(a && b && a->N == 768 && b->N == 768 && a->B > 0 && b->B > 0 && a->S > 0 && b->S > 0 && a->x && b->x && a->out && b->out,
                    UNIVL_EINVAL, "univl_pool_pair_fwd: bad argument (N must be 768)");
    hipLaunchKernelGGL(pool_pair_fwd_kernel, dim3(a->B + b->B), dim3(256), 0, stream, *a, *b);
    UNIVL_LAUNCH_CHECK();
    return UNIVL_OK;
}

extern "C" int univl_pool_pair_bwd(const UnivlPool* a, const UnivlPool* b, hipStream_t stream) {
    UNIVL_ON_STREAM_DEVICE(stream);
    int rc = pool_bwd_check(a, "univl_pool_pair_bwd");
    if (rc) return rc;
    rc = pool_bwd_check(b, "univl_pool_pair_bwd");
    if (rc) return rc;
    const int smax = a->S > b->S ? a->S : b->S;
    hipLaunchKernelGGL(pool_pair_bwd_kernel, dim3(a->B + b->B, (smax + PCHUNK - 1) / PCHUNK), dim3(256), 0, stream, *a, *b);
    UNIVL_LAUNCH_CHECK();
    return UNIVL_OK;
}

extern "C" int univl_maxmargin_loss(const float* sim, int32_t n, int32_t ld, float margin, const float* weight, float* loss,
                                    float* dsim, hipStream_t stream) {
    UNIVL_ON_STREAM_DEVICE(stream);
    UNIVL_CHECK_ARG(sim && loss && dsim && n > 0 && n <= 8192 && ld >= n, UNIVL_EINVAL, "univl_maxmargin_loss: bad argument");
    hipLaunchKernelGGL(maxmargin_kernel, dim3(1), dim3(256), n * sizeof(float), stream, sim, n, ld, margin, weight, loss, dsim);
    UNIVL_LAUNCH_CHECK();
    return UNIVL_OK;
}

extern "C" int univl_crossen_loss(const float* sim, int32_t n, int32_t ld, float* loss, float* dsim, hipStream_t stream) {
    UNIVL_ON_STREAM_DEVICE(stream);
    UNIVL_CHECK_ARG(sim && loss && dsim && n > 0 && ld >= n, UNIVL_EINVAL, "univl_crossen_loss: bad argument");
    hipLaunchKernelGGL(crossen_kernel, dim3(1), dim3(256), 0, stream, sim, n, ld, loss, dsim);
    UNIVL_LAUNCH_CHECK();
    return UNIVL_OK;
}

extern "C" int univl_milnce_loss(const float* sim, int32_t batch_size, int32_t n_pair, int32_t ld, float* loss, float* dsim,
                                 hipStream_t stream) {
    UNIVL_ON_STREAM_DEVICE(stream);
    UNIVL_CHECK_ARG(sim && loss && dsim && batch_size > 0 && n_pair > 0 && ld >= batch_size * n_pair, UNIVL_EINVAL, "univl_milnce_loss: bad argument");
    hipLaunchKernelGGL(milnce_kernel, dim3(1), dim3(256), 0, stream, sim, batch_size, n_pair, ld, loss, dsim);
    UNIVL_LAUNCH_CHECK();
    return UNIVL_OK;
}
```

### univl_amd/engine.py

```python
import contextlib
import ctypes as C
import gc
import os
import weakref

import torch

from . import _ab, _lib, ops

@contextlib.contextmanager
def no_gc():
    was = gc.isenabled()
    gc.disable()
    try:
        yield
    finally:
        if was:
            gc.enable()


GUARDED = []


def _workspace(dev, zeros=False):
# ... 181 lines not shown
                ops.cast_bf16_pair(self.p32, self.p16, self.p16lo)
            else:
                ops.cast_bf16(self.p32, self.p16)
        self.shadow_valid = True

    def attach_grads(self, used_names):
        for n in used_names:
            p, gv = self.params[n], self.g(n)
            if p.grad is not gv:
                p.grad = gv


class GradState:

    def __init__(self, flat, fresh, fuse_sumsq=False):
        self.flat, self.fresh, self.written = flat, fresh, set()
        self.fuse_sumsq, self.covered = bool(fuse_sumsq), set()
        self.slots, self.entries = 0, []

    def sumsq_args(self, names, rows_per_tensor, cols):
        if isinstance(names, str):
            names = [names]
        if not self.fuse_sumsq or any(self.flat.is_atomic(n) for n in names) or rows_per_tensor % 128 != 0:
            return {}
        if any(n in self.covered for n in names):
            raise RuntimeError("fused gradient norms: %s has a second writer in this backward" % (names,))
        self.covered.update(names)
        stride = (rows_per_tensor // 64) * ((cols + 63) // 64) * 4
        start = self.slots
        for t, n in enumerate(names):
            self.entries.append((self.flat.seg_of[n], start + t * stride, stride))
        self.slots += stride * len(names)
        if self.slots > self.flat.partials.numel():
            raise RuntimeError("fused gradient norms: partial-sum buffer too small")
        return dict(sumsq=self.flat.partials[start:], sumsq_rows=rows_per_tensor if len(names) > 1 else 0, sumsq_stride=stride)

    def acc(self, name):
        if self.flat.is_atomic(name):
            return True
        a = (not self.fresh) or (name in self.written)
        self.written.add(name)
        return a

    def finish(self, plan):
        if not self.entries:
            return
        dev = self.flat.device
        seg, start, count = (torch.tensor(x, dtype=torch.int32, device=dev) for x in zip(*self.entries))
        out = self.flat.sumsq
        plan.add_callable(lambda: ops.sumsq_finish(self.flat.partials, seg, start, count, out))


class Plan:

    def __init__(self):
        self.ops = []
        self.keep = []
        self.descs = {}
        self.external = {}
        self._side = {}
        self._segments = None
        self.rider_keys = set()
        self.riders = None

    def add_gemm_rider(self, desc, key, slot, nslots, stream=0):
        self.keep.append(desc)
        self.descs[len(self.ops)] = [desc]
        self.rider_keys.add(key)
        self.ops.append(("rider", _lib.lib().univl_gemm_rider, (desc, key, int(slot), int(nslots)), "univl_gemm_rider", stream))

    def add_gemm_ln(self, desc, ln_desc, counters, key=None, slot=0, nslots=1, stream=0):
        self.keep += [desc, ln_desc, counters]
        self.descs[len(self.ops)] = [desc]
        if key is not None:
            self.rider_keys.add(key)
        self.ops.append(("gemm_ln", _lib.lib().univl_gemm_ln, (desc, ln_desc, counters, key, int(slot), int(nslots)), "univl_gemm_ln", stream))

    def add(self, fn_name, desc, stream=0):
        fn = getattr(_lib.lib(), fn_name)
        self.keep.append(desc)
        self.descs[len(self.ops)] = [desc]
        self.ops.append(("call", fn, C.byref(desc), fn_name, stream))

    def add_pair_call(self, fn_name, da, db, stream=0):
        fn = getattr(_lib.lib(), fn_name)
        self.keep += [da, db]
        self.descs[len(self.ops)] = [da, db]
        self.ops.append(("call2", fn, (da, db), fn_name, stream))

    def add_gemm_group(self, descs, stream=0, max_blocks=0):
        fn = _lib.lib().univl_gemm_group_limited
        if not _ab.get("group_wgrad"):
            for d in descs:
                self.add("univl_gemm", d, stream)
            return
        for i in range(0, len(descs), _lib.GEMM_GROUP_MAX):
            chunk = descs[i:i + _lib.GEMM_GROUP_MAX]
            arr = (_lib.Gemm * len(chunk))(*chunk)
            self.keep.append(arr)
            self.descs[len(self.ops)] = list(chunk)
            self.ops.append(("group", fn, (arr, len(chunk), int(max_blocks)), "univl_gemm_group", stream))

    def add_gemm_pair(self, dgrad, wgrad, stream=0):
        fn = _lib.lib().univl_gemm_pair
        arr = (_lib.Gemm * 2)(dgrad, wgrad)
        self.keep.append(arr)
        self.descs[len(self.ops)] = [dgrad, wgrad]
        self.ops.append(("pair", fn, arr, "univl_gemm_pair", stream))

    def add_attn_fwd_fused(self, attn, qkv, key=None, slot=0, nslots=1, stream=0):
        self.keep += [attn, qkv]
        self.descs[len(self.ops)] = [qkv]
        if key is not None:
            self.rider_keys.add(key)
        self.ops.append(("attn_fwd_fused", _lib.lib().univl_attention_fwd_fused, (attn, qkv, key, int(slot), int(nslots)), "univl_attention_fwd_fused", stream))

    def add_attn_bwd_fused(self, attn, odgrad, owgrad, stream=0):
        self.keep += [attn, odgrad, owgrad]
        self.descs[len(self.ops)] = [odgrad] + ([owgrad] if owgrad is not None else [])
        self.ops.append(("attn_fused", _lib.lib().univl_attention_bwd_fused, (attn, odgrad, owgrad), "univl_attention_bwd_fused", stream))

    def add_gemm_pair_ln(self, dgrad, wgrad, ln_desc, counters, stream=0):
        arr = (_lib.Gemm * 2)(dgrad, wgrad)
        self.keep += [arr, ln_desc, counters]
        self.descs[len(self.ops)] = [dgrad, wgrad]
        self.ops.append(("pair_ln", _lib.lib().univl_gemm_pair_ln, (arr, ln_desc, counters), "univl_gemm_pair_ln", stream))

    def add_zeros(self, tensors, stream=0):
        ts = [t for t in tensors if t is not None and t.numel() > 0]
        if ts:
            self.add_callable(lambda: ops.zero_many(ts), stream)

    def add_callable(self, f, stream=0, eager=False, with_streams=False):
        kind = "eager" if eager else ("pys" if with_streams else "py")
        self.ops.append((kind, f, None, getattr(f, "__name__", "callable"), stream))

    def wait_point(self, key, stream=0):
        self.ops.append(("wait", key, None, "wait", stream))

    def record(self, key, stream=0):
        self.ops.append(("record", key, None, "record", stream))

    def fork(self, src, dst):
        if src != dst:
            self.ops.append(("dep", src, dst, "dep", 0))

    def join(self, src, dst):
        self.fork(src, dst)

    def _stream(self, idx, cur):
        if idx == 0:
            return cur
        st = self._side.get(idx)
        if st is None or st.device != cur.device:
            st = torch.cuda.Stream(device=cur.device)
            self._side[idx] = st
        return st

    def _run_ops(self, ops_, cur, forked=None):
        handles, events = {}, {}
        forked = set() if forked is None else set(forked)
        for op in ops_:
            kind, a, b, name, sidx = op
            if kind == "call":
                h = handles.get(sidx)
                if h is None:
                    h = handles[sidx] = C.c_void_p(self._stream(sidx, cur).cuda_stream)
                rc = a(b, h)
                if rc != 0:
                    _lib.check(rc, name)
            elif kind == "call2":
                h = handles.get(sidx)
                if h is None:
                    h = handles[sidx] = C.c_void_p(self._stream(sidx, cur).cuda_stream)
                rc = a(C.byref(b[0]), C.byref(b[1]), h)
                if rc != 0:
                    _lib.check(rc, name)
            elif kind == "group":
                h = handles.get(sidx)
                if h is None:
                    h = handles[sidx] = C.c_void_p(self._stream(sidx, cur).cuda_stream)
                rc = a(b[0], b[1], b[2], h)
                if rc != 0:
                    _lib.check(rc, name)
            elif kind == "rider":
                h = handles.get(sidx)
                if h is None:
                    h = handles[sidx] = C.c_void_p(self._stream(sidx, cur).cuda_stream)
                desc, key, slot, nslots = b
                rd = self.riders
                rng = rd["ranges"].get(key) if rd else None
                if rng is not None and (key, slot) in rd["used"]:
                    rng = None
                if rng is None:
                    rc = _lib.lib().univl_gemm(C.byref(desc), h)
                else:
                    rd["used"].add((key, slot))
                    lo, hi = rng[0] + rng[1] * slot // nslots, rng[0] + rng[1] * (slot + 1) // nslots
                    rc = a(C.byref(desc), C.byref(rd["desc"]), lo, hi - lo, int(rd.get("max_blocks", 0)), h)
                if rc != 0:
                    _lib.check(rc, name)
            elif kind == "gemm_ln":
                h = handles.get(sidx)
                if h is None:
                    h = handles[sidx] = C.c_void_p(self._stream(sidx, cur).cuda_stream)
                desc, lnd, ctr, key, slot, nslots = b
                rd = self.riders
                rng = rd["ranges"].get(key) if (rd and key is not None) else None
                if rng is not None and (key, slot) in rd["used"]:
                    rng = None
                L_ = _lib.lib()
                if rng is None:
                    rc = a(C.byref(desc), C.byref(lnd), C.c_void_p(ctr.data_ptr()), None, 0, 0, 0, 0, h)
                    if rc == _lib.EUNSUPPORTED:
                        rc = L_.univl_gemm(C.byref(desc), h) or L_.univl_layernorm_fwd(C.byref(lnd), h)
                else:
                    rd["used"].add((key, slot))
                    lo, hi = rng[0] + rng[1] * slot // nslots, rng[0] + rng[1] * (slot + 1) // nslots
                    rc = a(C.byref(desc), C.byref(lnd), C.c_void_p(ctr.data_ptr()), C.byref(rd["desc"]), lo, hi - lo, int(rd.get("max_blocks", 0)), 0, h)
                    if rc == _lib.EUNSUPPORTED:
                        rc = (L_.univl_gemm_rider(C.byref(desc), C.byref(rd["desc"]), lo, hi - lo, int(rd.get("max_blocks", 0)), h)
                              or L_.univl_layernorm_fwd(C.byref(lnd), h))
                if rc != 0:
                    _lib.check(rc, name)
            elif kind == "pair_ln":
                h = handles.get(sidx)
                if h is None:
                    h = handles[sidx] = C.c_void_p(self._stream(sidx, cur).cuda_stream)
                arr, lnd, ctr = b
                rc = a(C.byref(arr[0]), C.byref(arr[1]), C.byref(lnd), C.c_void_p(ctr.data_ptr()), 0, h)
                if rc == _lib.EUNSUPPORTED:
                    rc = _lib.lib().univl_gemm_pair(C.byref(arr[0]), C.byref(arr[1]), 0, h) or _lib.lib().univl_layernorm_bwd(C.byref(lnd), h)
                if rc != 0:
                    _lib.check(rc, name)
            elif kind == "pair":
                h = handles.get(sidx)
                if h is None:
                    h = handles[sidx] = C.c_void_p(self._stream(sidx, cur).cuda_stream)
                rc = a(C.byref(b[0]), C.byref(b[1]), 0, h)
                if rc != 0:
                    _lib.check(rc, name)
            elif kind == "attn_fwd_fused":
                h = handles.get(sidx)
                if h is None:
                    h = handles[sidx] = C.c_void_p(self._stream(sidx, cur).cuda_stream)
                at, qd, key, slot, nslots = b
                rd = self.riders
                rng = rd["ranges"].get(key) if (rd and key is not None) else None
                if rng is not None and (key, slot) in rd["used"]:
                    rng = None
                if rng is None:
                    rc = a(C.byref(at), C.byref(qd), None, 0, 0, 0, 0, h)
                else:
                    rd["used"].add((key, slot))
                    lo, hi = rng[0] + rng[1] * slot // nslots, rng[0] + rng[1] * (slot + 1) // nslots
                    rc = a(C.byref(at), C.byref(qd), C.byref(rd["desc"]), lo, hi - lo, int(rd.get("max_blocks", 0)), 0, h)
                if rc != 0:
                    _lib.check(rc, name)
# ... 637 lines not shown
```

### univl_amd/ops.py

```python
import ctypes as C

import torch

from . import _lib
from ._lib import DT_BF16, DT_F32

_BYREF = C.byref


def _stream():
    return C.c_void_p(torch.cuda.current_stream().cuda_stream)


def _p(t):
    return None if t is None else C.c_void_p(t.data_ptr())


def dtype_code(dtype):
    if dtype == torch.float32:
        return DT_F32
    if dtype == torch.bfloat16:
        return DT_BF16
    raise RuntimeError("univl_amd: unsupported compute dtype %s (float32 or bfloat16)" % dtype)

# ... 84 lines not shown
    rc = _lib.lib().univl_gemm_pair_ln(_BYREF(dgrad), _BYREF(wgrad), _BYREF(ln), C.c_void_p(counters.data_ptr()), int(bool(dry_run)), _stream())
    if rc == _lib.EUNSUPPORTED:
        return False
    _lib.check(rc, "gemm_pair_ln")
    return True


def layernorm_desc(dtype, rows, N, *, x=None, x_f64=False, residual=None, pos=None, pos_period=0, gamma=None,
                   beta=None, eps=1e-12, y=None, stats=None, out32=None, out16=None, p_pre=0.0, p_post=0.0, seed=0,
                   off_pre=0, off_post=0, seed_dev=None, dout=None, dx32=None, dxd32=None, dxd16=None, dgamma=None,
                   dbeta=None, dbias=None, dpos=None, out16_lo=None):
    d = _lib.LayerNorm()
    d.dtype, d.rows, d.N, d.x_f64 = dtype, rows, N, int(x_f64)
    d.x, d.residual, d.pos, d.pos_period = _p(x), _p(residual), _p(pos), pos_period
    d.gamma, d.beta, d.eps = _p(gamma), _p(beta), eps
    d.y, d.stats, d.out32, d.out16 = _p(y), _p(stats), _p(out32), _p(out16)
    d.p_pre, d.p_post, d.seed, d.off_pre, d.off_post, d.seed_dev = p_pre, p_post, seed, off_pre, off_post, _p(seed_dev)
    d.dout, d.dx32, d.dxd32, d.dxd16 = _p(dout), _p(dx32), _p(dxd32), _p(dxd16)
    d.dgamma, d.dbeta, d.dbias, d.dpos = _p(dgamma), _p(dbeta), _p(dbias), _p(dpos)
    d.out16_lo = _p(out16_lo)
    return d


def layernorm_fwd(**kw):
    d = layernorm_desc(**kw)
    _lib.check(_lib.lib().univl_layernorm_fwd(_BYREF(d), _stream()), "layernorm_fwd")


def layernorm_bwd(**kw):
    d = layernorm_desc(**kw)
    _lib.check(_lib.lib().univl_layernorm_bwd(_BYREF(d), _stream()), "layernorm_bwd")


def attention_desc(dtype, B, H, Sq, Sk, q, ldq, k, ldk, v, ldv, out, ldo, lse, *, key_mask=None, causal=False,
                   p_drop=0.0, seed=0, offset=0, seed_dev=None, dout=None, lddo=0, dq=None, lddq=0, dk=None, lddk=0,
                   dv=None, lddv=0, bsk=0, bsv=0, out_lo=None):
    def ptr(t):
        if t is None:
            return None
        if isinstance(t, tuple):
            return C.c_void_p(t[0].data_ptr() + t[1] * t[0].element_size())
        return C.c_void_p(t.data_ptr())
    d = _lib.Attention()
    d.dtype, d.B, d.H, d.Sq, d.Sk = dtype, B, H, Sq, Sk
    d.q, d.ldq, d.k, d.ldk, d.v, d.ldv = ptr(q), ldq, ptr(k), ldk, ptr(v), ldv
    d.key_mask, d.causal = _p(key_mask), int(causal)
    d.out, d.ldo, d.lse = ptr(out), ldo, _p(lse)
    d.p_drop, d.seed, d.offset, d.seed_dev = p_drop, seed, offset, _p(seed_dev)
    d.dout, d.lddo, d.dq, d.lddq, d.dk, d.lddk, d.dv, d.lddv = ptr(dout), lddo, ptr(dq), lddq, ptr(dk), lddk, ptr(dv), lddv
    d.bsk, d.bsv = bsk, bsv
    d.out_lo = ptr(out_lo)
    return d


def attention_fwd(*a, **kw):
    d = attention_desc(*a, **kw)
    _lib.check(_lib.lib().univl_attention_fwd(_BYREF(d), _stream()), "attention_fwd")


def attention_bwd(*a, **kw):
    d = attention_desc(*a, **kw)
    _lib.check(_lib.lib().univl_attention_bwd(_BYREF(d), _stream()), "attention_bwd")


def attention_bwd_fused(attn, odgrad, owgrad=None, dry_run=False):
    rc = _lib.lib().univl_attention_bwd_fused(_BYREF(attn), _BYREF(odgrad), _BYREF(owgrad) if owgrad is not None else None,
                                              int(bool(dry_run)), _stream())
    if rc == _lib.EUNSUPPORTED:
        return False
    _lib.check(rc, "attention_bwd_fused")
    return True


def attention_fwd_fused(attn, qkv, dry_run=False):
    rc = _lib.lib().univl_attention_fwd_fused(_BYREF(attn), _BYREF(qkv), None, 0, 0, 0, int(bool(dry_run)), _stream())
    if rc == _lib.EUNSUPPORTED:
        return False
    _lib.check(rc, "attention_fwd_fused")
    return True


def embed_text_desc(dtype, B, S, ids, word, pos, gamma, beta, *, type_ids=None, type_emb=None, eps=1e-12, y=None,
                    stats=None, out32=None, out16=None, p_post=0.0, seed=0, off_post=0, seed_dev=None, dout=None,
                    dword=None, dpos=None, dtype_emb=None, dgamma=None, dbeta=None, drows=None, out16_lo=None):
    d = _lib.EmbedText()
    d.dtype, d.B, d.S, d.N = dtype, B, S, 768
    d.ids, d.type_ids = _p(ids), _p(type_ids)
    d.word, d.pos, d.type = _p(word), _p(pos), _p(type_emb)
    d.gamma, d.beta, d.eps = _p(gamma), _p(beta), eps
    d.y, d.stats, d.out32, d.out16 = _p(y), _p(stats), _p(out32), _p(out16)
    d.p_post, d.seed, d.off_post, d.seed_dev = p_post, seed, off_post, _p(seed_dev)
    d.dout, d.dword, d.dpos, d.dtype_emb, d.dgamma, d.dbeta = _p(dout), _p(dword), _p(dpos), _p(dtype_emb), _p(dgamma), _p(dbeta)
    d.drows = _p(drows)
    d.out16_lo = _p(out16_lo)
    return d


def embed_text_fwd(*a, **kw):
    d = embed_text_desc(*a, **kw)
    _lib.check(_lib.lib().univl_embed_text_fwd(_BYREF(d), _stream()), "embed_text_fwd")


def embed_text_bwd(*a, **kw):
    d = embed_text_desc(*a, **kw)
    _lib.check(_lib.lib().univl_embed_text_bwd(_BYREF(d), _stream()), "embed_text_bwd")


def pool_desc(B, S, x, mask, *, skip_first, normalize, mean=None, out=None, dout=None, dx=None, ldx_row=768, accumulate=False,
              dsim=None, other=None, n_other=0, transpose=False, gscale=None):
    d = _lib.Pool()
    d.B, d.S, d.N = B, S, 768
    d.x, d.ldx_row, d.mask = _p(x), ldx_row, _p(mask)
    d.skip_first, d.normalize = int(skip_first), int(normalize)
    d.mean, d.out, d.dout, d.dx = _p(mean), _p(out), _p(dout), _p(dx)
    d.accumulate = int(accumulate)
    d.dsim, d.ldsim = _p(dsim), (dsim.stride(0) if dsim is not None else 0)
    d.other, d.n_other, d.transpose, d.gscale = _p(other), int(n_other), int(bool(transpose)), _p(gscale)
    return d


def pool_fwd(*a, **kw):
    d = pool_desc(*a, **kw)
    _lib.check(_lib.lib().univl_pool_fwd(_BYREF(d), _stream()), "pool_fwd")


def pool_bwd(*a, **kw):
    d = pool_desc(*a, **kw)
    _lib.check(_lib.lib().univl_pool_bwd(_BYREF(d), _stream()), "pool_bwd")


def pool_pair_fwd(da, db):
    _lib.check(_lib.lib().univl_pool_pair_fwd(_BYREF(da), _BYREF(db), _stream()), "pool_pair_fwd")


def pool_pair_bwd(da, db):
    _lib.check(_lib.lib().univl_pool_pair_bwd(_BYREF(da), _BYREF(db), _stream()), "pool_pair_bwd")


def maxmargin_loss(sim, margin, weight, loss, dsim):
    n = sim.shape[0]
    assert dsim.stride(0) == sim.stride(0)
    _lib.check(_lib.lib().univl_maxmargin_loss(_p(sim), n, sim.stride(0), margin, _p(weight), _p(loss), _p(dsim), _stream()), "maxmargin")


def crossen_loss(sim, loss, dsim):
    assert dsim.stride(0) == sim.stride(0)
    _lib.check(_lib.lib().univl_crossen_loss(_p(sim), sim.shape[0], sim.stride(0), _p(loss), _p(dsim), _stream()), "crossen")


def milnce_loss(sim, batch_size, n_pair, loss, dsim):
    assert dsim.stride(0) == sim.stride(0)
    _lib.check(_lib.lib().univl_milnce_loss(_p(sim), batch_size, n_pair, sim.stride(0), _p(loss), _p(dsim), _stream()), "milnce")


def scale_by_device_scalar(x, s):
    _lib.check(_lib.lib().univl_scale_by_device_scalar(_p(x), x.numel(), _p(s), _stream()), "scale_by_device_scalar")


def zero_many(tensors):
    import ctypes as C
    L = _lib.lib()
    for i in range(0, len(tensors), 16):
        ts = tensors[i:i + 16]
        ptrs = (C.c_void_p * len(ts))(*[t.data_ptr() for t in ts])
        sizes = (C.c_int64 * len(ts))(*[t.numel() * t.element_size() for t in ts])
        _lib.check(L.univl_zero_many(ptrs, sizes, len(ts), _stream()), "zero_many")


def copy_many(pairs):
    import ctypes as C
    L = _lib.lib()
    for i in range(0, len(pairs), 16):
        ps = pairs[i:i + 16]
        srcs = (C.c_void_p * len(ps))(*[s.data_ptr() for _, s in ps])
        dsts = (C.c_void_p * len(ps))(*[d.data_ptr() for d, _ in ps])
        sizes = (C.c_int64 * len(ps))(*[d.numel() * d.element_size() for d, _ in ps])
        _lib.check(L.univl_copy_many(srcs, dsts, sizes, len(ps), _stream()), "copy_many")


def rows_zero(table, lst, meta):
    _lib.check(_lib.lib().univl_rows_zero(_p(table), table.shape[0], _p(lst), _p(meta), _stream()), "rows_zero")


def rows_append(ids, lst, meta, reset, ever=None):
    _lib.check(_lib.lib().univl_rows_append(_p(ids), ids.numel(), _p(lst), lst.numel(), _p(meta), int(bool(reset)), _p(ever),
                                            0 if ever is None else ever.numel(), _stream()), "rows_append")


def rows_sumsq(table, lst, meta, out):
    _lib.check(_lib.lib().univl_rows_sumsq(_p(table), table.shape[0], _p(lst), _p(meta), _p(out), _stream()), "rows_sumsq")


def embed_scatter(ids, rows, scale, dword):
    _require_gpu(ids, rows, dword)
    _lib.check(_lib.lib().univl_embed_scatter(_p(ids), _p(rows), ids.numel(), float(scale), _p(dword), _stream()), "embed_scatter")


def rows_gather_sum(rows, period, out):
    _require_gpu(rows, out)
    _lib.check(_lib.lib().univl_rows_gather_sum(_p(rows), rows.shape[0], int(period), rows.shape[1], _p(out), _stream()), "rows_gather_sum")


def sumsq_finish(partials, seg, start, count, out):
    _lib.check(_lib.lib().univl_sumsq_finish(_p(partials), _p(seg), _p(start), _p(count), seg.numel(), _p(out), _stream()),
               "sumsq_finish")


def gather_rows(src, dst, idx, rows, row_stride_bytes, copy_bytes):
    _require_gpu(src, dst, idx)
    _lib.check(_lib.lib().univl_gather_rows(_p(src), _p(dst), _p(idx), rows, row_stride_bytes, copy_bytes, _stream()), "gather_rows")


def log_softmax_rows(x, n):
    _require_gpu(x)
    _lib.check(_lib.lib().univl_log_softmax_rows(_p(x), x.shape[0], n, x.stride(0), _stream()), "log_softmax_rows")


def beam_ws(n_inst, n_bm, device):
    return torch.empty(n_inst * n_bm * _lib.BEAM_SLICES * n_bm * 2, dtype=torch.float32, device=device)


def beam_step_desc(lp, V, n_inst, n_bm, t, *, scores, done, length, tokens, src, hist_parents, hist_tokens, hist_scores, ws, eos=-1,
                   eos_dev=None, first_step=None):
    _require_gpu(lp, scores, done, length, tokens, src, hist_parents, hist_tokens, hist_scores, ws, eos_dev)
    R = n_inst * n_bm
    assert lp.dtype == torch.float32 and lp.dim() == 2 and lp.stride(1) == 1 and lp.shape[0] >= R
    assert scores.dtype == torch.float32 and scores.numel() == R and scores.is_contiguous()
    assert done.dtype in (torch.uint8, torch.bool) and done.numel() == n_inst
    assert length.dtype == torch.int32 and length.numel() == n_inst
    assert tokens.dtype == torch.int64 and tokens.numel() == R and src.dtype == torch.int32 and src.numel() == R
    Tmax = hist_parents.shape[0]
    for h, dt_ in ((hist_parents, torch.int32), (hist_tokens, torch.int32), (hist_scores, torch.float32)):
        assert h.dtype == dt_ and h.is_contiguous() and h.shape[0] == Tmax and h.numel() == Tmax * R
    assert eos_dev is None or eos_dev.dtype == torch.int32
    d = _lib.BeamStep()
    d.lp, d.ld, d.n_inst, d.n_bm, d.V = _p(lp), lp.stride(0), n_inst, n_bm, V
    d.first_step, d.eos, d.eos_dev, d.t, d.Tmax = int(t == 0 if first_step is None else first_step), int(eos), _p(eos_dev), t, Tmax
    d.scores, d.done, d.length, d.tokens, d.src = _p(scores), _p(done), _p(length), _p(tokens), _p(src)
    d.hist_parents, d.hist_tokens, d.hist_scores = _p(hist_parents), _p(hist_tokens), _p(hist_scores)
    d.ws, d.ws_bytes = _p(ws), ws.numel() * ws.element_size()
    return d


def beam_step(*a, **kw):
    d = beam_step_desc(*a, **kw)
    _lib.check(_lib.lib().univl_beam_step(_BYREF(d), _stream()), "beam_step")


def beam_backtrack(hist_parents, hist_tokens, scores, length, n_best):
# ... 164 lines not shown
```

### univl_amd/steps.py

```python
import os

import numpy as np
import torch

from . import _ab, _lib, ops
from .engine import DecoderStack, EncoderStack, GradState, Plan, _SiteCounter, _gemm_desc

H = 768


def _e(dev):
    from .engine import _workspace
    return _workspace(dev, zeros=True)


class Ctx:

    def __init__(self, model, training):
        self.model, self.fl, self.training = model, model.flat, training
        self.tc = model.task_config
        self.dev, self.ct, self.dt = self.fl.device, self.fl.compute_dtype, self.fl.dt
        self.bf = self.ct == torch.bfloat16
        self.p = model.dropout_prob if training else 0.0
        self.seed, self.seed_dev = model._seed, model._seed_dev
        self.sites = _SiteCounter()
        self.e = _e(self.dev)
        self.red = model._reducer
        self.stamps = {} if _ab.get("stamps") else None
        if self.stamps is not None:
            self.stamp_buf = torch.zeros(64, dtype=torch.int64, device=self.dev)
            model._stamps = (self.stamps, self.stamp_buf)

    def stamp(self, plan, name, stream=0):
        if self.stamps is None:
            return
        slot = self.stamps.setdefault(name, len(self.stamps))
        buf = self.stamp_buf
        plan.add_callable(lambda: ops.stamp(buf[slot:slot + 1]), stream)


def stage_input(dst, src):
    src = torch.as_tensor(src)
    if src.dtype != dst.dtype:
        src = src.to(dst.dtype)
    dst.copy_(src.reshape(dst.shape), non_blocking=True)


def stage_inputs(pairs):
    fast = []
    use_kernel = bool(_ab.get("copy_kernel"))
    for dst, src in pairs:
        src = torch.as_tensor(src)
        if (use_kernel and src.device == dst.device and dst.is_cuda and src.dtype == dst.dtype and src.numel() == dst.numel()
                and src.is_contiguous() and dst.is_contiguous()):
            if src.data_ptr() != dst.data_ptr():
                fast.append((dst, src))
        else:
            stage_input(dst, src)
    if fast:
        ops.copy_many(fast)


class EncoderPass:

    def __init__(self, cx, B, W, F, s_text=0, s_vis=2, normalized_input=False, branches=("text", "vis")):
        self.cx, self.B, self.W, self.F = cx, B, W, F
        self.branches = tuple(branches)
        assert self.branches in (("text", "vis"), ("text",), ("vis",)), branches
        if self.branches != ("text", "vis"):
            self._init_single(cx, B, W, F, s_text, bool(normalized_input))
            return
        self.normalized_input = bool(normalized_input)
        e, ct, bf, fl = cx.e, cx.ct, cx.bf, cx.fl
        D = cx.tc.video_dim
        self.D, self.Tt, self.Tv = D, B * W, B * F
        self.ST, self.SV = s_text, s_vis
        i64 = torch.int64
        self.ids, self.type_ids, self.amask = e(B, W, dtype=i64), e(B, W, dtype=i64), e(B, W, dtype=i64)
        self.video, self.vmask = e(B * F, D, dtype=torch.float64), e(B, F, dtype=i64)
        self.vy, self.vst, self.vn32 = e(self.Tv, D), e(self.Tv, 2), e(self.Tv, D)
        self.vn_op = e(self.Tv, D, dtype=ct) if bf else self.vn32
        self.ve, self.vest, self.v0_32 = e(self.Tv, H), e(self.Tv, 2), e(self.Tv, H)
        self.v0_16 = e(self.Tv, H, dtype=ct) if bf else self.v0_32
        self.te, self.test, self.t0_32 = e(self.Tt, H), e(self.Tt, 2), e(self.Tt, H)
        self.t0_16 = e(self.Tt, H, dtype=ct) if bf else self.t0_32
        self.dseq, self.dvis = e(self.Tt, H), e(self.Tv, H)
        self.de_op = e(self.Tv, H, dtype=ct)
        self.dvnorm = e(self.Tv, D)
        m = cx.model
        self.text = EncoderStack(fl, "bert", m.bert_config.num_hidden_layers, B, W, self.amask, cx.p, cx.seed_dev, cx.sites,
                                 s_main=s_text, s_side=s_text)
        self.vis = EncoderStack(fl, "visual", m.visual_config.num_hidden_layers, B, F, self.vmask, cx.p, cx.seed_dev, cx.sites,
                                s_main=s_vis, s_side=s_vis)
        self.off_t, self.off_v = cx.sites.next(), cx.sites.next()
        self.t0_lo = e(self.Tt, H, dtype=ct) if self.text.pair_x else None
        self.v0_lo = e(self.Tv, H, dtype=ct) if self.vis.pair_x else None
        self.vn_lo = e(self.Tv, D, dtype=ct) if (self.vis.pair_x and not self.normalized_input) else None
        self.seq_out, self.seq_out16 = self.text.output()
        self.vis_out, self.vis_out16 = self.vis.output()

    def _init_single(self, cx, B, W, F, stream, normalized_input):
        self.normalized_input = normalized_input
        e, ct, bf, fl, m = cx.e, cx.ct, cx.bf, cx.fl, cx.model
        D = cx.tc.video_dim
        self.D, self.Tt, self.Tv = D, B * W, B * F
        self.ST = self.SV = stream
        i64 = torch.int64
        self.text = self.vis = self.seq_out = self.seq_out16 = self.vis_out = self.vis_out16 = None
        self.t0_lo = self.v0_lo = self.vn_lo = None
        if self.branches == ("text",):
            self.ids, self.type_ids, self.amask = e(B, W, dtype=i64), e(B, W, dtype=i64), e(B, W, dtype=i64)
            self.te, self.test, self.t0_32 = e(self.Tt, H), e(self.Tt, 2), e(self.Tt, H)
            self.t0_16 = e(self.Tt, H, dtype=ct) if bf else self.t0_32
            self.text = EncoderStack(fl, "bert", m.bert_config.num_hidden_layers, B, W, self.amask, cx.p, cx.seed_dev, cx.sites,
                                     s_main=stream, s_side=stream)
            self.off_t = cx.sites.next()
            self.t0_lo = e(self.Tt, H, dtype=ct) if self.text.pair_x else None
            self.seq_out, self.seq_out16 = self.text.output()
        else:
            self.video, self.vmask = e(B * F, D, dtype=torch.float64), e(B, F, dtype=i64)
            self.vy, self.vst, self.vn32 = e(self.Tv, D), e(self.Tv, 2), e(self.Tv, D)
            self.vn_op = e(self.Tv, D, dtype=ct) if bf else self.vn32
            self.ve, self.vest, self.v0_32 = e(self.Tv, H), e(self.Tv, 2), e(self.Tv, H)
            self.v0_16 = e(self.Tv, H, dtype=ct) if bf else self.v0_32
            self.vis = EncoderStack(fl, "visual", m.visual_config.num_hidden_layers, B, F, self.vmask, cx.p, cx.seed_dev, cx.sites,
                                    s_main=stream, s_side=stream)
            self.off_v = cx.sites.next()
            self.v0_lo = e(self.Tv, H, dtype=ct) if self.vis.pair_x else None
            self.vn_lo = e(self.Tv, D, dtype=ct) if (self.vis.pair_x and not normalized_input) else None
            self.vis_out, self.vis_out16 = self.vis.output()

    def load_text(self, input_ids, token_type_ids, attention_mask):
        stage_inputs([(self.ids, input_ids), (self.type_ids, token_type_ids), (self.amask, attention_mask)])

    def load_video(self, video, video_mask):
        stage_inputs([(self.vn32 if self.normalized_input else self.video, video), (self.vmask, video_mask)])

    N = dict(nv_g="normalize_video.visual_norm2d.weight", nv_b="normalize_video.visual_norm2d.bias",
             vw="visual.embeddings.word_embeddings.weight", vb="visual.embeddings.word_embeddings.bias",
             vpos="visual.embeddings.position_embeddings.weight", vlg="visual.embeddings.LayerNorm.weight",
             vlb="visual.embeddings.LayerNorm.bias", bw="bert.embeddings.word_embeddings.weight",
             bp="bert.embeddings.position_embeddings.weight", bt="bert.embeddings.token_type_embeddings.weight",
             blg="bert.embeddings.LayerNorm.weight", blb="bert.embeddings.LayerNorm.bias")

    def load(self, input_ids, token_type_ids, attention_mask, video, video_mask):
        B, W, F = self.B, self.W, self.F
        stage_inputs([(self.ids, input_ids), (self.type_ids, token_type_ids), (self.amask, attention_mask),
                      (self.vn32 if self.normalized_input else self.video, video), (self.vmask, video_mask)])

    def build_forward(self, fwd):
        cx, n, fl, dt, bf = self.cx, self.N, self.cx.fl, self.cx.dt, self.cx.bf
        W32, p, B, W, F, D, Tv = fl.w32, cx.p, self.B, self.W, self.F, self.D, self.Tv
        ST, SV = self.ST, self.SV
        both, stacks = self.branches == ("text", "vis"), [st for st in (self.text, self.vis) if st is not None]
        fwd.add_zeros([st.yarena for st in stacks if st.zero_y] + [st.ln_ctr for st in stacks if st.ln_ctr is not None], ST)
        if both:
            cx.stamp(fwd, "f_fork", ST)
            fwd.fork(ST, SV)
            cx.stamp(fwd, "f_vis_start", SV)
        if self.vis is not None:
            if self.normalized_input:
                if bf:
                    fwd.add_callable(lambda: ops.cast_bf16(self.vn32, self.vn_op), SV)
            else:
                fwd.add("univl_layernorm_fwd", ops.layernorm_desc(
                    dt, Tv, D, x=self.video, x_f64=True, gamma=W32(n["nv_g"]), beta=W32(n["nv_b"]), y=self.vy, stats=self.vst,
                    out32=self.vn32, out16=self.vn_op if bf else None, out16_lo=self.vn_lo), SV)
            fwd.add("univl_gemm", _gemm_desc(dt, self.vn_op, D, fl.wop(n["vw"]), D, Tv, H, D, out32=self.ve, ldc=H, bias=W32(n["vb"]),
                                             a_lo=self.vn_lo, b_lo=fl.wlo(n["vw"]) if self.vis.pair_w else None), SV)
            fwd.add("univl_layernorm_fwd", ops.layernorm_desc(
                dt, Tv, H, x=self.ve, pos=W32(n["vpos"]), pos_period=F, gamma=W32(n["vlg"]), beta=W32(n["vlb"]), y=self.ve,
                stats=self.vest, out32=self.v0_32, out16=self.v0_16 if bf else None, p_post=p, seed=cx.seed, off_post=self.off_v,
                seed_dev=cx.seed_dev, out16_lo=self.v0_lo), SV)
        if self.text is not None:
            cx.stamp(fwd, "f_text_start", ST)
            fwd.add("univl_embed_text_fwd", ops.embed_text_desc(
                dt, B, W, self.ids, W32(n["bw"]), W32(n["bp"]), W32(n["blg"]), W32(n["blb"]), type_ids=self.type_ids,
                type_emb=W32(n["bt"]), y=self.te, stats=self.test, out32=self.t0_32, out16=self.t0_16 if bf else None, p_post=p,
                seed=cx.seed, off_post=self.off_t, seed_dev=cx.seed_dev, out16_lo=self.t0_lo), ST)
        if self.vis is not None:
            self.vis.build_forward(fwd, self.v0_32, self.v0_16, cx.training, zero_arena=False, x16_lo=self.v0_lo)
            cx.stamp(fwd, "f_vis_end", SV)
        if self.text is not None:
            self.text.build_forward(fwd, self.t0_32, self.t0_16, cx.training, zero_arena=False, x16_lo=self.t0_lo)
            cx.stamp(fwd, "f_text_end", ST)
        if both:
            fwd.join(SV, ST)
            cx.stamp(fwd, "f_join", ST)

    def zero_list(self):
        return ([self.dseq, self.dvis, self.dvnorm] + [st.garena for st in (self.text, self.vis) if st.zero_g] +
                [st.ln_ctr_b for st in (self.text, self.vis) if st.ln_ctr_b is not None])

    def build_backward(self, bwd, gs, hook=None):
        cx, n, fl, dt = self.cx, self.N, self.cx.fl, self.cx.dt
        W32, G, p, B, W, F, D, Tv = fl.w32, fl.g, cx.p, self.B, self.W, self.F, self.D, self.Tv
        ST, SV = self.ST, self.SV
        cx.stamp(bwd, "b_fork", ST)
        bwd.fork(ST, SV)
        cx.stamp(bwd, "b_vis_start", SV)
        cx.stamp(bwd, "b_text_start", ST)
        gv = self.vis.backward_layers(bwd, self.dvis, self.v0_32, self.v0_16, gs, cx.training, layer_hook=hook, zero_arena=False)
        gt = self.text.backward_layers(bwd, self.dseq, self.t0_32, self.t0_16, gs, cx.training, layer_hook=hook, zero_arena=False)
        ratio = max(1, int(round(self.text.L / max(1, self.vis.L))))
        done_t = done_v = False
        while not (done_t and done_v):
            for _ in range(ratio):
                if not done_t and next(gt, None) is None:
                    done_t = True
                    self._text_tail(bwd, self.text.bwd_out)
                    cx.stamp(bwd, "b_text_end", ST)
            if not done_v and next(gv, None) is None:
                done_v = True
                self._video_tail(bwd, gs, self.vis.bwd_out)
                cx.stamp(bwd, "b_vis_end", SV)
        bwd.join(SV, ST)
        cx.stamp(bwd, "b_join", ST)

    def _gather_dpos(self):
        thr = _ab.get("dpos_gather_min")
        return thr > 0 and self.B >= thr

    def _video_tail(self, bwd, gs, dxv):
        cx, n, fl, dt = self.cx, self.N, self.cx.fl, self.cx.dt
        W32, G, p, F, D, Tv, SV = fl.w32, fl.g, cx.p, self.F, self.D, self.Tv, self.SV
        gather = self._gather_dpos()
        if gather and getattr(self, "dxe", None) is None:
            self.dxe = cx.e(Tv, H)
        bwd.add("univl_layernorm_bwd", ops.layernorm_desc(
            dt, Tv, H, gamma=W32(n["vlg"]), y=self.ve, stats=self.vest, dout=dxv, dxd16=self.de_op, dgamma=G(n["vlg"]),
            dbeta=G(n["vlb"]), dbias=G(n["vb"]), dpos=None if gather else G(n["vpos"]), dx32=self.dxe if gather else None,
            pos_period=F, p_post=p, seed=cx.seed, off_post=self.off_v, seed_dev=cx.seed_dev), SV)
        if gather:
            bwd.add_callable(lambda: ops.rows_gather_sum(self.dxe, F, G(n["vpos"])[:F]), SV)
        bwd.add("univl_gemm", _gemm_desc(dt, self.de_op, H, self.vn_op, D, H, D, Tv, trans_a=1, trans_b=1, out32=G(n["vw"]),
                                         ldc=D, accumulate=gs.acc(n["vw"])), SV)
        bwd.add("univl_gemm", _gemm_desc(dt, self.de_op, H, fl.wop(n["vw"]), D, Tv, D, H, trans_b=1, out32=self.dvnorm, ldc=D,
                                         accumulate=True), SV)
        bwd.add("univl_layernorm_bwd", ops.layernorm_desc(
            dt, Tv, D, gamma=W32(n["nv_g"]), y=self.vy, stats=self.vst, dout=self.dvnorm, dgamma=G(n["nv_g"]), dbeta=G(n["nv_b"])), SV)

    def _text_tail(self, bwd, dxt):
        cx, n, fl, dt = self.cx, self.N, self.cx.fl, self.cx.dt
        W32, G, p, B, W, ST = fl.w32, fl.g, cx.p, self.B, self.W, self.ST
        sparse = getattr(self, "sparse_word_grad", False)
        gather = self._gather_dpos()
        if (sparse or gather) and getattr(self, "drows", None) is None:
            self.drows = cx.e(self.Tt, H)
        bwd.add("univl_embed_text_bwd", ops.embed_text_desc(
            dt, B, W, self.ids, W32(n["bw"]), W32(n["bp"]), W32(n["blg"]), W32(n["blb"]), type_ids=self.type_ids,
            type_emb=W32(n["bt"]), y=self.te, stats=self.test, p_post=p, seed=cx.seed, off_post=self.off_t,
            seed_dev=cx.seed_dev, dout=dxt, dword=G(n["bw"]), dpos=None if gather else G(n["bp"]), dtype_emb=G(n["bt"]),
            dgamma=G(n["blg"]), dbeta=G(n["blb"]), drows=self.drows if (sparse or gather) else None), ST)
        if gather:
            bwd.add_callable(lambda: ops.rows_gather_sum(self.drows, W, G(n["bp"])[:W]), ST)
            if not sparse:
                bwd.add_callable(lambda: ops.embed_scatter(self.ids.view(-1), self.drows, 1.0, G(n["bw"])), ST)
        rows = getattr(self, "word_rows", None)
        if rows is not None and not sparse:
            lst, meta, reset = rows
            bwd.add_callable(lambda: ops.rows_append(self.ids.view(-1), lst, meta, reset, cx.fl.word_ever), ST)


class SimLoss:

    def __init__(self, cx, kind, n):
        self.cx, self.kind, self.n = cx, kind, n
        self.loss = cx.e(1)
        tc = cx.tc
        self.wts = None
        if kind == "maxmargin":
            bsz = tc.batch_size // tc.n_gpu
            if tc.negative_weighting and tc.n_pair > 1 and bsz > 1:
                easy = 1 - tc.hard_negative_rate
                alpha = easy / ((bsz - 1) * (1 - easy))
                mm = np.kron((1 - alpha) * np.eye(bsz) + alpha, np.ones((tc.n_pair, tc.n_pair))) * (bsz * (1 - easy))
                self.wts = torch.tensor(mm, dtype=torch.float32, device=cx.dev).contiguous()

    def build(self, fwd, sim, dsim):
        tc, n = self.cx.tc, self.n
        if self.kind == "milnce":
            bs, npair = n // tc.n_pair, tc.n_pair
            fwd.add_callable(lambda: ops.milnce_loss(sim, bs, npair, self.loss, dsim))
        elif self.kind == "crossen":
            fwd.add_callable(lambda: ops.crossen_loss(sim, self.loss, dsim))
        else:
            margin, wts = float(tc.margin), self.wts
            fwd.add_callable(lambda: ops.maxmargin_loss(sim, margin, wts, self.loss, dsim))


class JointSim:

    def __init__(self, cx, enc, loss_kind):
        self.cx, self.enc = cx, enc
        B = enc.B
        e = cx.e
        self.ldp = (B + 3) // 4 * 4
        self.tmean, self.tn, self.vmean, self.vn = e(B, H), e(self.ldp, H), e(B, H), e(self.ldp, H)
        self.sim, self.dsim = e(self.ldp, self.ldp), e(self.ldp, self.ldp)
        self.dtn, self.dvn = e(B, H), e(B, H)
        self.norm = not bool(cx.tc.use_mil)
        self.fused = bool(_ab.get("fused_sim")) and B <= 256
        self.lossfn = SimLoss(cx, loss_kind, B)
        self.loss = self.lossfn.loss

    def build_forward(self, fwd):
        enc, B = self.enc, self.enc.B
        dt_ = ops.pool_desc(B, enc.W, enc.seq_out, enc.amask, skip_first=True, normalize=self.norm, mean=self.tmean, out=self.tn)
        dv_ = ops.pool_desc(B, enc.F, enc.vis_out, enc.vmask, skip_first=False, normalize=self.norm, mean=self.vmean, out=self.vn)
        if self.fused:
            fwd.add_pair_call("univl_pool_pair_fwd", dt_, dv_)
        else:
            fwd.add("univl_pool_fwd", dt_)
            fwd.add("univl_pool_fwd", dv_)
        fwd.add("univl_gemm", _gemm_desc(_lib.DT_F32, self.tn, H, self.vn, H, B, B, H, out32=self.sim, ldc=self.ldp))
        self.lossfn.build(fwd, self.sim[:B], self.dsim[:B])

    def build_backward(self, bwd, gout):
        enc, B, ldp = self.enc, self.enc.B, self.ldp
        if self.fused:
            bwd.add_pair_call(
                "univl_pool_pair_bwd",
                ops.pool_desc(B, enc.W, enc.seq_out, enc.amask, skip_first=True, normalize=self.norm, mean=self.tmean, out=self.tn,
                              dx=enc.dseq, accumulate=True, dsim=self.dsim, other=self.vn, n_other=B, transpose=False, gscale=gout),
                ops.pool_desc(B, enc.F, enc.vis_out, enc.vmask, skip_first=False, normalize=self.norm, mean=self.vmean, out=self.vn,
                              dx=enc.dvis, accumulate=True, dsim=self.dsim, other=self.tn, n_other=B, transpose=True, gscale=gout))
            return
        bwd.add_callable(lambda: ops.scale_by_device_scalar(self.dsim, gout))
        bwd.add("univl_gemm", _gemm_desc(_lib.DT_F32, self.dsim, ldp, self.vn, H, B, H, B, trans_b=1, out32=self.dtn, ldc=H))
        bwd.add("univl_gemm", _gemm_desc(_lib.DT_F32, self.dsim, ldp, self.tn, H, B, H, B, trans_a=1, trans_b=1, out32=self.dvn, ldc=H))
        bwd.add("univl_pool_bwd", ops.pool_desc(B, enc.W, enc.seq_out, enc.amask, skip_first=True, normalize=self.norm,
                                                mean=self.tmean, out=self.tn, dout=self.dtn, dx=enc.dseq, accumulate=True))
        bwd.add("univl_pool_bwd", ops.pool_desc(B, enc.F, enc.vis_out, enc.vmask, skip_first=False, normalize=self.norm,
                                                mean=self.vmean, out=self.vn, dout=self.dvn, dx=enc.dvis, accumulate=True))


class CrossRun:

    def __init__(self, cx, enc, tidx, vidx, stream=0):
        self.cx, self.enc = cx, enc
        self.P = len(tidx)
        self.W, self.F = enc.W, enc.F
        self.S = S = enc.W + enc.F
        self.T = T = self.P * S
        e, ct, bf, fl = cx.e, cx.ct, cx.bf, cx.fl
        self.sm = stream
        self.tidx = torch.tensor(list(tidx), dtype=torch.int32, device=cx.dev)
        self.vidx = torch.tensor(list(vidx), dtype=torch.int32, device=cx.dev)
        self.cmask = e(self.P, S, dtype=torch.int64)
        self.concat, self.cst = e(T, H), e(T, 2)
        self.c0_32 = e(T, H)
        self.c0_16 = e(T, H, dtype=ct) if bf else self.c0_32
        self.postype, self.dpostype = e(S, H), e(S, H)
        self.dcross = e(T, H)
        self.dconcat = e(T, H)
        L = cx.model.cross_config.num_hidden_layers
        self.stack = EncoderStack(fl, "cross", L, self.P, S, self.cmask, cx.p, cx.seed_dev, cx.sites, s_main=stream, s_side=stream)
        self.off = cx.sites.next()
        self.out32, self.out16 = self.stack.output()

    N = dict(pos="cross.embeddings.position_embeddings.weight", typ="cross.embeddings.token_type_embeddings.weight",
             lg="cross.embeddings.LayerNorm.weight", lb="cross.embeddings.LayerNorm.bias")

    def build_forward(self, fwd):
        cx, enc, n, fl, dt, sm = self.cx, self.enc, self.N, self.cx.fl, self.cx.dt, self.sm
        W32 = fl.w32
        P, W, F, S, T = self.P, self.W, self.F, self.S, self.T
        fwd.add_callable(lambda: ops.postype_fwd(W32(n["pos"]), W32(n["typ"]), W, S, self.postype), sm)
        fwd.add_callable(lambda: ops.pair_concat_fwd(enc.seq_out, enc.vis_out, enc.amask, enc.vmask, self.tidx, self.vidx, P, W, F,
                                                     self.concat, self.cmask), sm)
        fwd.add("univl_layernorm_fwd", ops.layernorm_desc(
            dt, T, H, x=self.concat, pos=self.postype, pos_period=S, gamma=W32(n["lg"]), beta=W32(n["lb"]), y=self.concat,
            stats=self.cst, out32=self.c0_32, out16=self.c0_16 if cx.bf else None, p_post=cx.p, seed=cx.seed, off_post=self.off,
            seed_dev=cx.seed_dev), sm)
        self.stack.build_forward(fwd, self.c0_32, self.c0_16, cx.training)

    def zero_list(self):
        return [self.dcross, self.dpostype]

    def build_backward(self, bwd, gs, hook=None):
        cx, enc, n, fl, dt, sm = self.cx, self.enc, self.N, self.cx.fl, self.cx.dt, self.sm
        W32, G = fl.w32, fl.g
        P, W, F, S, T = self.P, self.W, self.F, self.S, self.T
        dx0 = self.stack.build_backward(bwd, self.dcross, self.c0_32, self.c0_16, gs, cx.training, layer_hook=hook)
        bwd.add("univl_layernorm_bwd", ops.layernorm_desc(
            dt, T, H, gamma=W32(n["lg"]), y=self.concat, stats=self.cst, dout=dx0, dx32=self.dconcat, dgamma=G(n["lg"]),
            dbeta=G(n["lb"]), dpos=self.dpostype, pos_period=S, p_post=cx.p, seed=cx.seed, off_post=self.off,
            seed_dev=cx.seed_dev), sm)
        bwd.add_callable(lambda: ops.pair_concat_bwd(self.dconcat, self.tidx, self.vidx, P, W, F, enc.dseq, enc.dvis), sm)
        bwd.add_callable(lambda: ops.postype_bwd(self.dpostype, W, S, G(n["pos"]), G(n["typ"])), sm)


class PoolerSim:

    def __init__(self, cx, run, Bt, Bv, loss_kind):
        self.cx, self.run, self.Bt, self.Bv = cx, run, Bt, Bv
        e, ct = cx.e, cx.ct
        P = run.P
        self.pre, self.pooled, self.sim, self.dsim = e(P, H), e(P, H), e(P), e(P)
        self.dpooled, self.dpre = e(P, H), e(P, H, dtype=ct)
        self.lossfn = SimLoss(cx, loss_kind, Bt) if loss_kind else None
        self.loss = self.lossfn.loss if self.lossfn else None

    N = dict(pw="cross.pooler.dense.weight", pb="cross.pooler.dense.bias", sw="similarity_dense.weight", sb="similarity_dense.bias")

    def build_forward(self, fwd):
        cx, run, n, fl, dt = self.cx, self.run, self.N, self.cx.fl, self.cx.dt
        P, S = run.P, run.S
        x0 = run.out16
# ... 234 lines not shown
        W32, G = fl.w32, fl.g
        B, W, F, Tv, D, ldl = self.B, self.W, self.F, self.Tv, self.D, self.ldl
        dl = self.dlogits_ct
        bwd.add_callable(lambda: ops.scale_ct(dl, gout), sm)
        bwd.add("univl_gemm", _gemm_desc(dt, dl, ldl, self.clean.vn_op, D, Tv, D, Tv, trans_b=1, out16=self.dscores, ldc=D), sm)
        bwd.add("univl_gemm", _gemm_desc(dt, dl, ldl, self.scores, D, Tv, D, Tv, trans_a=1, trans_b=1, out32=self.clean.dvnorm, ldc=D,
                                         accumulate=True), sm)
        bwd.add_callable(lambda: ops.colsum(self.dscores, G(n["bias"])), sm)
        bwd.add("univl_gemm", _gemm_desc(dt, self.dscores, D, fl.wop(n["vw"]), D, Tv, H, D, out32=self.dh, ldc=H), sm)
        bwd.add("univl_gemm", _gemm_desc(dt, self.h16, H, self.dscores, D, H, D, Tv, trans_a=1, trans_b=1, out32=G(n["vw"]), ldc=D,
                                         accumulate=gs.acc(n["vw"])), sm)
        bwd.add("univl_layernorm_bwd", ops.layernorm_desc(dt, Tv, H, gamma=W32(n["lg"]), y=self.hy, stats=self.hst, dout=self.dh,
                                                          dx32=self.dg, dgamma=G(n["lg"]), dbeta=G(n["lb"])), sm)
        bwd.add_callable(lambda: ops.gelu_bwd(self.dg, self.u, self.du), sm)
        bwd.add("univl_gemm", _gemm_desc(dt, self.du, H, self.vpart16, H, H, H, Tv, trans_a=1, trans_b=1, out32=G(n["tw"]), ldc=H,
                                         accumulate=gs.acc(n["tw"]), dbias=G(n["tb"])), sm)
        bwd.add("univl_gemm", _gemm_desc(dt, self.du, H, fl.wop(n["tw"]), H, Tv, H, H, trans_b=1, out32=self.dvpart, ldc=H), sm)
        self.mlm.build_backward(bwd, gs, gout, self.tpart16, self.dtpart, accumulate_dx=False)
        bwd.add_callable(lambda: ops.pair_concat_fwd(self.dtpart, self.dvpart, run.enc.amask, run.enc.vmask, self.arange, self.arange,
                                                     B, W, F, run.dcross, None), sm)


class Step:

    def __init__(self, cx):
        self.cx = cx
        self.loss, self.gout = cx.e(1), cx.e(1)
        self.gout.fill_(1.0)
        self.fwd = Plan()
        self.bwd = {}
        self.loss_terms = []
        self.calls = 0

    def finish_forward(self):
        self.fwd.wait_point("all")
        terms = self.loss_terms
        if len(terms) == 1:
            self.loss = terms[0]
        else:
            def add():
                torch.add(terms[0], terms[1], out=self.loss)
                for t in terms[2:]:
                    self.loss.add_(t)
            self.fwd.add_callable(add)

    def backward_plan(self, fresh):
        if fresh not in self.bwd:
            self.bwd[fresh] = self._build_bwd(fresh)
        return self.bwd[fresh]


def _ddp_hook(cx, fl, model, kind):
    red = cx.red
    if red is None:
        return None, None, None
    from .parallel import BucketSchedule, layer_buckets
    buckets = layer_buckets(fl, model.used_parameter_names(kind))
    sched = BucketSchedule(float(os.environ.get("UNIVL_BUCKET_MB", "80")) * 2 ** 20)

    def emit(plan):
        ranges = sched.take()
        if ranges:
            if red.capturable:
                plan.add_callable(lambda streams: red.reduce_ranges(ranges, after=streams), with_streams=True)
            else:
                plan.add_callable(lambda: red.reduce_ranges(ranges), eager=True)

    def hook(plan, prefix, l, stream):
        key = (prefix, l)
        if key in buckets["layers"] and sched.add(*buckets["layers"][key]):
            emit(plan)
    return hook, buckets, (sched, emit)


def build_step(model, kind, B, W, F, training):
    cx = Ctx(model, training)
    fl, tc = cx.fl, cx.tc
    st = Step(cx)
    st.kind, st.B, st.W, st.F = kind, B, W, F
    fwd = st.fwd
    fwd.external = model._param_events
    fwd.wait_point("base")
    cx.stamp(fwd, "f_begin")
    if cx.p > 0:
        fwd.add_callable(lambda: ops.bump_counter(cx.seed_dev))
    branches = {"features_text": ("text",), "features_vis": ("vis",), "features_vis_shaped": ("vis",)}.get(kind, ("text", "vis"))
    st.enc = enc = EncoderPass(cx, B, W, F, normalized_input=kind in ("features_shaped", "features_vis_shaped"), branches=branches)
    if _ab.get("tail_ride"):
        if kind in ("align", "caption", "pretrain", "pretrain_nocap") and model.cross is not None:
            enc.text.tail_key = ("layer", "cross", 0)
        if kind in ("caption", "pretrain") and model.decoder is not None:
            enc.vis.tail_key = ("layer", "decoder", 0)
    enc.build_forward(fwd)
    st.fwd_encoders_len = len(fwd)
    stage_two = bool(model._stage_two)
    loss_kind = "crossen" if stage_two else ("milnce" if tc.use_mil else "maxmargin")
    pre_kind = "milnce" if tc.use_mil else "maxmargin"
    st.enc_m = st.joint = st.run_pairs = st.pooler = st.run_rows = st.decoder = st.heads = st.run_heads = None
    pairs = [(i, j) for i in range(B) for j in range(B)]
    rows = list(range(B))
    if kind == "joint":
        st.joint = JointSim(cx, enc, loss_kind)
        st.joint.build_forward(fwd)
        st.loss_terms.append(st.joint.loss)
    elif kind == "align":
        st.run_pairs = CrossRun(cx, enc, [a for a, _ in pairs], [b for _, b in pairs])
        st.run_pairs.build_forward(fwd)
        st.pooler = PoolerSim(cx, st.run_pairs, B, B, loss_kind)
        st.pooler.build_forward(fwd)
        st.loss_terms.append(st.pooler.loss)
    elif kind == "caption":
        st.run_rows = CrossRun(cx, enc, rows, rows)
        st.run_rows.build_forward(fwd)
        st.decoder = DecoderRun(cx, st.run_rows, W)
        st.decoder.build_forward(fwd)
        st.loss_terms.append(st.decoder.loss)
    elif kind in ("pretrain", "pretrain_nocap"):
        st.enc_m = enc_m = EncoderPass(cx, B, W, F)
        enc_m.build_forward(fwd)
        st.run_heads = CrossRun(cx, enc_m, rows, rows)
        st.run_heads.build_forward(fwd)
        st.heads = PretrainHeads(cx, st.run_heads, enc)
        st.heads.build_forward(fwd)
        st.loss_terms += [st.heads.mlm.loss, st.heads.nce_loss]
        st.joint = JointSim(cx, enc, pre_kind)
        st.joint.build_forward(fwd)
        st.loss_terms.append(st.joint.loss)
        if kind == "pretrain":
            st.run_rows = CrossRun(cx, enc_m, rows, rows)
            st.run_rows.build_forward(fwd)
            st.decoder = DecoderRun(cx, st.run_rows, W)
            st.decoder.build_forward(fwd)
            st.loss_terms.append(st.decoder.loss)
        st.run_pairs = CrossRun(cx, enc_m, [a for a, _ in pairs], [b for _, b in pairs])
        st.run_pairs.build_forward(fwd)
        st.pooler = PoolerSim(cx, st.run_pairs, B, B, loss_kind)
        st.pooler.build_forward(fwd)
        st.loss_terms.append(st.pooler.loss)
    elif kind in ("features", "features_shaped", "features_text", "features_vis", "features_vis_shaped"):
        pass
    else:
        raise ValueError(kind)
    cx.stamp(fwd, "f_end")
    if st.loss_terms:
        st.finish_forward()
    else:
        fwd.wait_point("all")

    def build_bwd(fresh):
        bwd = Plan()
        sparse = (cx.red is not None and kind in ("joint", "align") and bool(_ab.get("sparse_emb")))
        enc.sparse_word_grad = sparse
        fuse = (cx.red is None and kind in ("joint", "align", "caption") and bool(_ab.get("fused_norms")))
        gs = GradState(fl, fresh, fuse_sumsq=fuse)
        hook, buckets, sched = _ddp_hook(cx, fl, model, kind)
        cross_runs = [r for r in (st.run_pairs, st.run_rows, st.run_heads) if r is not None]
        last_cross = cross_runs[-1] if cross_runs else None
        hook_for = lambda r: hook if r is last_cross else None
        world = 1 if cx.red is None else max(1, cx.red.world)
        rows_mode = (kind in ("joint", "align") and bool(_ab.get("sparse_rows"))
                     and (cx.red is None or sparse)
                     and enc.Tt * (world if sparse else 1) <= fl.WORD_ROWS_CAP)
        zeros = [fl.sumsq, fl.partials] if fuse else []
        enc.word_rows = None
        if rows_mode:
            lst, meta = fl.word_rows()
            enc.word_rows = (lst, meta, fresh)
            if fresh:
                zeros += fl.v_region_without_word_table()
                bwd.add_callable(lambda: ops.rows_zero(fl.g(fl.WORD), lst, meta))
        elif fresh:
            zeros.append(fl.g32[:fl.v_end])
        zeros += enc.zero_list()
        if st.enc_m is not None:
            zeros += st.enc_m.zero_list()
        for r in (st.run_pairs, st.run_rows):
            if r is not None:
                zeros += r.zero_list()
        if st.run_heads is not None:
            zeros.append(st.run_heads.dpostype)
        cx.stamp(bwd, "b_begin")
        bwd.add_zeros(zeros)
        g = st.gout
        if st.pooler is not None:
            st.pooler.build_backward(bwd, gs, g)
            st.run_pairs.build_backward(bwd, gs, hook_for(st.run_pairs))
        if st.decoder is not None:
            st.decoder.build_backward(bwd, gs, g)
            st.run_rows.build_backward(bwd, gs, hook_for(st.run_rows))
        if st.heads is not None:
            st.heads.build_backward(bwd, gs, g)
            st.run_heads.build_backward(bwd, gs, hook_for(st.run_heads))
        if st.joint is not None:
            st.joint.build_backward(bwd, g)
        if st.enc_m is not None:
            st.enc_m.build_backward(bwd, gs, None)
        enc.build_backward(bwd, gs, hook)
        if cx.red is not None:
            red, tail = cx.red, buckets["tail"]
            if sparse:
                from .parallel import subtract_range
                wname = EncoderPass.N["bw"]
                wo, wk, _ = fl.index[wname]
                tail = subtract_range(tail, wo, wo + (wk + 63) // 64 * 64)
                world = max(1, red.world)
                ids_all = torch.zeros(world, enc.Tt, dtype=torch.int64, device=cx.dev)
                rows_all = torch.zeros(world, enc.Tt, H, device=cx.dev)
                st.sparse_exchange = dict(tokens=enc.Tt, bytes=rows_all.numel() * 4 + ids_all.numel() * 8)

                def gather_tokens():
                    red.gather(enc.ids.view(-1), ids_all)
                    red.gather(enc.drows, rows_all)
                if red.capturable:
                    bwd.add_callable(lambda streams: (red.gather(enc.ids.view(-1), ids_all, after=streams),
                                                      red.gather(enc.drows, rows_all)), with_streams=True)
                else:
                    bwd.add_callable(gather_tokens, eager=True)
            for (s0, e0) in tail:
                sched[0].add(s0, e0)
            sched[1](bwd)
            bwd.add_callable(red.join, eager=not red.capturable)
            if sparse:
                bwd.add_callable(lambda: ops.embed_scatter(ids_all.view(-1), rows_all.view(-1, H), 1.0 / world, fl.g(wname)))
                if rows_mode:
                    bwd.add_callable(lambda: ops.rows_append(ids_all.view(-1), lst, meta, fresh, fl.word_ever))
            st.exchange_points = list(sched[0].cuts)
        gs.finish(bwd)
        cx.stamp(bwd, "b_end")
        bwd.fused_names = frozenset(gs.covered)
        bwd.rows_mode = rows_mode
        return bwd

    st._build_bwd = build_bwd
    return st
```

Before: 1860 pairs/s.

## Fold joint head, backward clears, counter bump and row bookkeeping into existing launches

The FT-Joint similarity head forward (pooling, similarity product, loss and dsim) becomes one launch. The buffer clears at the start of backward now run inside the similarity-head backward, which writes dseq/dvis directly instead of accumulating into cleared buffers. The dropout counter bump moves into the forward clearing kernel, and word-row bookkeeping becomes an extra workgroup of the embedding backward. Together these remove several small launches and graph nodes from a step that is dominated by launch latency at batch 4. The cost is larger, more complex kernels and new ordering dependencies, since the clears now wait on the head backward.

```diff
diff --git a/include/univl_hip.h b/include/univl_hip.h
--- a/include/univl_hip.h
+++ b/include/univl_hip.h
@@ -19,7 +19,7 @@
 int univl_device_info(int* cu_count, char* name, int name_len);
 int univl_init(int device);
 #define UNIVL_ZERO_MAX 16
-int univl_zero_many(void* const* ptrs, const int64_t* bytes, int32_t n, hipStream_t stream);
+int univl_zero_many(void* const* ptrs, const int64_t* bytes, int32_t n, uint64_t* bump, hipStream_t stream);
 int univl_copy_many(const void* const* srcs, void* const* dsts, const int64_t* bytes, int32_t n, hipStream_t stream);
 int univl_destroy(void);
 int univl_set_deterministic(int on);
@@ -137,6 +137,7 @@
     float* dword; float* dpos; float* dtype_emb; float* dgamma; float* dbeta;
     float* drows;
     void* out16_lo;
+    int64_t* rows_list; int32_t* rows_meta; uint8_t* rows_ever; int64_t rows_total; int32_t rows_cap, rows_reset;
 } UnivlEmbedText;
 int univl_embed_text_fwd(const UnivlEmbedText* d, hipStream_t stream);
 int univl_embed_text_bwd(const UnivlEmbedText* d, hipStream_t stream);
@@ -162,7 +163,14 @@
 int univl_pool_fwd(const UnivlPool* d, hipStream_t stream);
 int univl_pool_bwd(const UnivlPool* d, hipStream_t stream);
 int univl_pool_pair_fwd(const UnivlPool* a, const UnivlPool* b, hipStream_t stream);
-int univl_pool_pair_bwd(const UnivlPool* a, const UnivlPool* b, hipStream_t stream);
+typedef struct UnivlClears {
+    void* ptr[UNIVL_ZERO_MAX]; int64_t bytes[UNIVL_ZERO_MAX]; int32_t n_zero;
+    float* table; int64_t rows_total; const int64_t* list; const int32_t* meta;
+} UnivlClears;
+int univl_pool_pair_bwd(const UnivlPool* a, const UnivlPool* b, const UnivlClears* clears, hipStream_t stream);
+enum { UNIVL_SIM_MAXMARGIN = 0, UNIVL_SIM_CROSSEN = 1, UNIVL_SIM_MILNCE = 2 };
+int univl_pool_pair_sim_loss(const UnivlPool* a, const UnivlPool* b, float* sim, float* dsim, int32_t ld, int32_t kind, float margin,
+                             const float* weight, int32_t n_pair, float* loss, int32_t* counter, hipStream_t stream);
 
 int univl_maxmargin_loss(const float* sim, int32_t n, int32_t ld, float margin, const float* weight, float* loss,
                          float* dsim, hipStream_t stream);
diff --git a/univl_amd/_ab.py b/univl_amd/_ab.py
--- a/univl_amd/_ab.py
+++ b/univl_amd/_ab.py
@@ -37,6 +37,11 @@
     "vocab_ce": (1, "K16: the vocabulary classifier with the online log-softmax CE in its epilogue (univl_vocab_ce_fwd / _bwd: no [tokens, 30522] logits in training); 0: product -> logits -> univl_ce_loss"),
     "vocab_dgrad_split": (1, "split-K of the vocabulary dgrad (caption / pretrain heads)"),
     "fused_sim": (1, "pooling + similarity + loss heads as fused launches up to 256 rows"),
+    "sim_fold": (1, "FT-Joint head forward: pooling, similarity, loss and d loss / d sim in ONE launch (univl_pool_pair_sim_loss) up to sim_fold_max_rows pairs; 0: pooling, fp32 product and loss as three launches"),
+    "sim_fold_max_rows": (16, "... up to this many pairs: ONE workgroup multiplies the B x B x 768 similarity (the library carries up to 32; measurements: profiles/sim_head_fold.txt)"),
+    "bwd_clears_ride": (1, "the clears at the head of the FT-Joint backward (univl_zero_many, univl_rows_zero) ride in the similarity-head backward launch, which then writes dseq / dvis instead of adding to cleared buffers; 0: two launches in front of it"),
+    "bump_in_clear": (1, "the dropout counter is advanced by the forward's clearing launch; 0: a univl_bump_counter launch in front of it"),
+    "rows_append_in_embed": (1, "the word-table row bookkeeping (univl_rows_append) as an extra workgroup of the text-embedding backward; 0: a launch behind it"),
     "dpos_gather_min": (32, "rows per position from which position-table gradients are gathered instead of scatter-added"),
     "beam_step": (1, "caption decoding: Beam.advance as the device-side tail of each position's plan (univl_beam_step) -- CaptionBeamSearch's default beam_step='device'; 0: 'host', the ATen top-k / where path with one host read per position (the comparand)"),
     "adam_ride": ("1", "BertAdam chunks ride with the next forward's products; '0': side-stream form; 'force': one graph even with a captured exchange"),
diff --git a/univl_amd/_lib.py b/univl_amd/_lib.py
--- a/univl_amd/_lib.py
+++ b/univl_amd/_lib.py
@@ -7,6 +7,7 @@
 DT_F32, DT_BF16 = 0, 1
 GEMM_ACCUM, GEMM_GELU_FWD, GEMM_GELU_BWD, GEMM_DBIAS_ATOMIC, GEMM_NT_OUT, GEMM_AUX_F32 = 1, 2, 4, 16, 32, 512
 GEMM_GROUP_MAX = 4
+SIM_KIND = {"maxmargin": 0, "crossen": 1, "milnce": 2}
 EUNSUPPORTED = -3
 
 vp, i32, i64, f32, u64 = C.c_void_p, C.c_int32, C.c_int64, C.c_float, C.c_uint64
@@ -40,13 +41,18 @@
     _fields_ = [("dtype", i32), ("B", i32), ("S", i32), ("N", i32), ("ids", vp), ("type_ids", vp), ("word", vp),
                 ("pos", vp), ("type", vp), ("gamma", vp), ("beta", vp), ("eps", f32), ("y", vp), ("stats", vp),
                 ("out32", vp), ("out16", vp), ("p_post", f32), ("seed", u64), ("off_post", u64), ("seed_dev", vp), ("dout", vp),
-                ("dword", vp), ("dpos", vp), ("dtype_emb", vp), ("dgamma", vp), ("dbeta", vp), ("drows", vp), ("out16_lo", vp)]
+                ("dword", vp), ("dpos", vp), ("dtype_emb", vp), ("dgamma", vp), ("dbeta", vp), ("drows", vp), ("out16_lo", vp),
+                ("rows_list", vp), ("rows_meta", vp), ("rows_ever", vp), ("rows_total", i64), ("rows_cap", i32), ("rows_reset", i32)]
 
 
 class Pool(C.Structure):
     _fields_ = [("B", i32), ("S", i32), ("N", i32), ("x", vp), ("ldx_row", i64), ("mask", vp),
                 ("skip_first", i32), ("normalize", i32), ("mean", vp), ("out", vp), ("dout", vp), ("dx", vp), ("accumulate", i32),
                 ("dsim", vp), ("ldsim", i64), ("other", vp), ("n_other", i32), ("transpose", i32), ("gscale", vp)]
+
+
+class Clears(C.Structure):
+    _fields_ = [("ptr", vp * 16), ("bytes", i64 * 16), ("n_zero", i32), ("table", vp), ("rows_total", i64), ("list", vp), ("meta", vp)]
 
 
 class Seg(C.Structure):
@@ -81,7 +87,7 @@
 BEAM_MAX, BEAM_SLICES = 8, 8
 TOPK_MAX, TOPK_SLICES_MAX = 64, 256
 
-_STRUCTS = [Gemm, LayerNorm, Attention, EmbedText, Pool, Seg, Adam, VocabCE, BeamStep, SimTopk]
+_STRUCTS = [Gemm, LayerNorm, Attention, EmbedText, Pool, Seg, Adam, VocabCE, BeamStep, SimTopk, Clears]
 _lib = None
 
 
@@ -109,7 +115,8 @@
         getattr(L, name).argtypes = [vp, vp]
         getattr(L, name).restype = i32
     L.univl_pool_pair_fwd.argtypes = [vp, vp, vp]
-    L.univl_pool_pair_bwd.argtypes = [vp, vp, vp]
+    L.univl_pool_pair_bwd.argtypes = [vp, vp, vp, vp]
+    L.univl_pool_pair_sim_loss.argtypes = [vp, vp, vp, vp, i32, i32, f32, vp, i32, vp, vp, vp]
     L.univl_gemm_group.argtypes = [vp, i32, vp]
     L.univl_gemm_group.restype = i32
     L.univl_gemm_group_limited.argtypes = [vp, i32, i32, vp]
@@ -127,7 +134,7 @@
     L.univl_rows_zero.argtypes = [vp, i64, vp, vp, vp]
     L.univl_rows_append.argtypes = [vp, i32, vp, i32, vp, i32, vp, i64, vp]
     L.univl_rows_sumsq.argtypes = [vp, i64, vp, vp, vp, vp]
-    L.univl_zero_many.argtypes = [vp, vp, i32, vp]
+    L.univl_zero_many.argtypes = [vp, vp, i32, vp, vp]
     L.univl_copy_many.argtypes = [vp, vp, vp, i32, vp]
     L.univl_maxmargin_loss.argtypes = [vp, i32, i32, f32, vp, vp, vp, vp]
     L.univl_crossen_loss.argtypes = [vp, i32, i32, vp, vp, vp]
@@ -186,7 +193,7 @@
             "univl_allreduce_bucket", "univl_set_deterministic", "univl_get_deterministic", "univl_gemm", "univl_gemm_group_limited", "univl_gemm_group", "univl_gemm_tile_map", "univl_gemm256_layout", "univl_gemm_pair", "univl_gemm_rider", "univl_gemm_rider_fits", "univl_gemm_rider_prime", "univl_gemm_ln", "univl_gemm_pair_ln",
             "univl_layernorm_fwd", "univl_layernorm_bwd", "univl_attention_fwd", "univl_attention_bwd", "univl_attention_bwd_fused", "univl_attention_fwd_fused",
             "univl_embed_text_fwd", "univl_embed_text_bwd", "univl_embed_scatter", "univl_rows_gather_sum", "univl_rows_zero", "univl_rows_append",
-            "univl_rows_sumsq", "univl_zero_many", "univl_copy_many", "univl_pool_fwd", "univl_pool_bwd", "univl_pool_pair_fwd", "univl_pool_pair_bwd",
+            "univl_rows_sumsq", "univl_zero_many", "univl_copy_many", "univl_pool_fwd", "univl_pool_bwd", "univl_pool_pair_fwd", "univl_pool_pair_bwd", "univl_pool_pair_sim_loss",
             "univl_maxmargin_loss", "univl_crossen_loss", "univl_milnce_loss", "univl_rank_counts", "univl_sim_topk", "univl_sim_topk_workspace", "univl_gather_rows", "univl_log_softmax_rows", "univl_beam_step", "univl_beam_backtrack", "univl_beam_captions", "univl_scale_by_device_scalar", "univl_pair_concat_fwd", "univl_pair_concat_bwd", "univl_postype_fwd", "univl_postype_bwd", "univl_tanh_fwd",
             "univl_tanh_bwd", "univl_gelu_bwd", "univl_colsum", "univl_scale_ct_by_device_scalar", "univl_simdense_fwd", "univl_simdense_bwd", "univl_ce_loss", "univl_vocab_ce_fwd", "univl_vocab_ce_bwd", "univl_mfm_nce_loss", "univl_grad_sumsq", "univl_sumsq_finish",
             "univl_clip_coef", "univl_scale_grads", "univl_bert_adam", "univl_bert_adam_range", "univl_cast_bf16", "univl_cast_bf16_pair", "univl_cast_f32", "univl_bump_counter", "univl_probe_layouts", "univl_stamp"]
diff --git a/univl_amd/csrc/clear_body.h b/univl_amd/csrc/clear_body.h
--- /dev/null
+++ b/univl_amd/csrc/clear_body.h
@@ -0,0 +1,29 @@
+#pragma once
+#include "common.h"
+#include "univl_hip.h"
+
+struct ZeroList { unsigned char* ptr[UNIVL_ZERO_MAX]; long bytes[UNIVL_ZERO_MAX]; };
+
+__device__ __forceinline__ void zero_many_body(const ZeroList& z, const long x, const int y, const long gx) {
+    unsigned char* p = z.ptr[y];
+    const long n16 = z.bytes[y] >> 4;
+    u32x4_t* q = reinterpret_cast<u32x4_t*>(p);
+    for (long i = x * 256 + threadIdx.x; i < n16; i += gx * 256) q[i] = u32x4_t{0u, 0u, 0u, 0u};
+    if (x == 0) for (long i = (n16 << 4) + threadIdx.x; i < z.bytes[y]; i += 256) p[i] = 0;
+}
+
+static inline long zero_many_gx(long most) {
+    long gx = (most / 16 + 2047) / 2048;
+    return gx < 1 ? 1 : (gx > 1024 ? 1024 : gx);
+}
+
+__device__ __forceinline__ void rows_zero_body(float* table, const long rows_total, const int64_t* list, const int* meta, const long x,
+                                               const long gx) {
+    const int over = meta[1];
+    const long n = over ? rows_total : (long)meta[0];
+    for (long k = x; k < n; k += gx) {
+        const long r = over ? k : (long)list[k];
+        float4* p = reinterpret_cast<float4*>(table + r * 768);
+        for (int c = threadIdx.x; c < 768 / 4; c += 256) p[c] = float4{0.f, 0.f, 0.f, 0.f};
+    }
+}
diff --git a/univl_amd/csrc/embed.hip b/univl_amd/csrc/embed.hip
--- a/univl_amd/csrc/embed.hip
+++ b/univl_amd/csrc/embed.hip
@@ -77,9 +77,33 @@
     }
 }
 
+__device__ __forceinline__ void rows_append_body(const int64_t* ids, int n, int64_t* list, int cap, int* meta, int reset, uint8_t* ever,
+                                                 long rows_total, int* base_over) {
+    if (threadIdx.x == 0) {
+        const int cur = reset ? 0 : meta[0];
+        int ov = reset ? 0 : meta[1];
+        if (cur + n > cap) ov = 1;
+        base_over[0] = cur; base_over[1] = ov;
+        meta[1] = ov;
+        meta[0] = ov ? cur : cur + n;
+    }
+    __syncthreads();
+    const int base = base_over[0], over = base_over[1];
+    if (!over) for (int i = threadIdx.x; i < n; i += 256) list[base + i] = ids[i];
+    if (ever) {
+        if (over) for (long r = threadIdx.x; r < rows_total; r += 256) ever[r] = 1;
+        else for (int i = threadIdx.x; i < n; i += 256) ever[ids[i]] = 1;
+    }
+}
+
 template <bool DET = false>
 __global__ __launch_bounds__(256) void embed_bwd_kernel(UnivlEmbedText p, float* det_part = nullptr, int* det_counter = nullptr) {
     __shared__ float red[4][N];
+    if (!DET && p.rows_list && (int)blockIdx.x * 4 >= p.B * p.S) {
+        rows_append_body(p.ids, p.B * p.S, p.rows_list, p.rows_cap, p.rows_meta, p.rows_reset, p.rows_ever, (long)p.rows_total,
+                         reinterpret_cast<int*>(&red[0][0]));
+        return;
+    }
     const int lane = threadIdx.x & 63, wave = threadIdx.x >> 6;
     const int row = blockIdx.x * 4 + wave;
     const bool valid = row < p.B * p.S;
@@ -265,21 +289,8 @@
 
 __global__ __launch_bounds__(256) void rows_append_kernel(const int64_t* ids, int n, int64_t* list, int cap, int* meta, int reset,
                                                           uint8_t* ever, long rows_total) {
-    __shared__ int base, over;
-    if (threadIdx.x == 0) {
-        const int cur = reset ? 0 : meta[0];
-        int ov = reset ? 0 : meta[1];
-        if (cur + n > cap) ov = 1;
-        base = cur; over = ov;
-        meta[1] = ov;
-        meta[0] = ov ? cur : cur + n;
-    }
-    __syncthreads();
-    if (!over) for (int i = threadIdx.x; i < n; i += 256) list[base + i] = ids[i];
-    if (ever) {
-        if (over) for (long r = threadIdx.x; r < rows_total; r += 256) ever[r] = 1;
-        else for (int i = threadIdx.x; i < n; i += 256) ever[ids[i]] = 1;
-    }
+    __shared__ int base_over[2];
+    rows_append_body(ids, n, list, cap, meta, reset, ever, rows_total, base_over);
 }
 
 __global__ __launch_bounds__(256) void rows_sumsq_kernel(const float* table, long rows_total, const int64_t* list, const int* meta,
@@ -362,6 +373,8 @@
     UNIVL_CHECK_ARG(d->B > 0 && d->S > 0 && d->ids && d->dout && d->y && d->stats && d->gamma && d->dword && (d->dpos || d->drows) &&
                         d->dgamma && d->dbeta,
                     UNIVL_EINVAL, "univl_embed_text_bwd: null / empty argument");
+    UNIVL_CHECK_ARG(!d->rows_list || (d->rows_meta && d->rows_cap > 0 && d->rows_cap <= ROWS_GRID && (!d->rows_ever || d->rows_total > 0)),
+                    UNIVL_EINVAL, "univl_embed_text_bwd: bad row-list argument (cap <= %d)", ROWS_GRID);
     dim3 grid((d->B * d->S + 3) / 4), block(256);
     if (univl_deterministic()) {
         UnivlEmbedText q = *d;
@@ -380,9 +393,13 @@
             hipLaunchKernelGGL(embed_dpos_gather_kernel, dim3((unsigned)(((long)d->S * N + 255) / 256)), block, 0, stream, q.drows, d->B, d->S, d->dpos);
         if (d->dtype_emb)
             hipLaunchKernelGGL(embed_dtype_gather_kernel, dim3(N / 256, 2), block, 0, stream, d->type_ids, q.drows, T, d->dtype_emb);
+        if (d->rows_list)
+            hipLaunchKernelGGL(rows_append_kernel, dim3(1), block, 0, stream, d->ids, (int)T, d->rows_list, d->rows_cap, d->rows_meta, d->rows_reset,
+                               d->rows_ever, (long)d->rows_total);
         UNIVL_LAUNCH_CHECK();
         return UNIVL_OK;
     }
+    if (d->rows_list) grid.x += 1;
     hipLaunchKernelGGL(embed_bwd_kernel<false>, grid, block, 0, stream, *d);
     UNIVL_LAUNCH_CHECK();
     return UNIVL_OK;
diff --git a/univl_amd/csrc/misc.hip b/univl_amd/csrc/misc.hip
--- a/univl_amd/csrc/misc.hip
+++ b/univl_amd/csrc/misc.hip
@@ -5,6 +5,7 @@
 #include <stdlib.h>
 #include "common.h"
 #include "univl_hip.h"
+#include "clear_body.h"
 
 static thread_local char g_err[512] = "";
 
@@ -30,6 +31,7 @@
         case 7: return (int)sizeof(UnivlVocabCE);
         case 8: return (int)sizeof(UnivlBeamStep);
         case 9: return (int)sizeof(UnivlSimTopk);
+        case 10: return (int)sizeof(UnivlClears);
         default: return -1;
     }
 }
@@ -114,17 +116,13 @@
 extern "C" int univl_get_deterministic(void) { return g_deterministic; }
 
 namespace {
-struct ZeroList { unsigned char* ptr[UNIVL_ZERO_MAX]; long bytes[UNIVL_ZERO_MAX]; };
-__global__ __launch_bounds__(256) void zero_many_kernel(ZeroList z) {
-    unsigned char* p = z.ptr[blockIdx.y];
-    const long n16 = z.bytes[blockIdx.y] >> 4;
-    u32x4_t* q = reinterpret_cast<u32x4_t*>(p);
-    for (long i = (long)blockIdx.x * 256 + threadIdx.x; i < n16; i += (long)gridDim.x * 256) q[i] = u32x4_t{0u, 0u, 0u, 0u};
-    if (blockIdx.x == 0) for (long i = (n16 << 4) + threadIdx.x; i < z.bytes[blockIdx.y]; i += 256) p[i] = 0;
-}
-}
-
-extern "C" int univl_zero_many(void* const* ptrs, const int64_t* bytes, int32_t n, hipStream_t stream) {
+__global__ __launch_bounds__(256) void zero_many_kernel(ZeroList z, uint64_t* bump) {
+    zero_many_body(z, blockIdx.x, blockIdx.y, gridDim.x);
+    if (bump && blockIdx.x == 0 && blockIdx.y == 0 && threadIdx.x == 0) bump[0] += 1;
+}
+}
+
+extern "C" int univl_zero_many(void* const* ptrs, const int64_t* bytes, int32_t n, uint64_t* bump, hipStream_t stream) {
     UNIVL_ON_STREAM_DEVICE(stream);
     UNIVL_CHECK_ARG(ptrs && bytes && n >= 1 && n <= UNIVL_ZERO_MAX, UNIVL_EINVAL, "univl_zero_many: n=%d (1..%d)", n, UNIVL_ZERO_MAX);
     ZeroList z;
@@ -135,9 +133,7 @@
         z.bytes[i] = bytes[i];
         most = bytes[i] > most ? bytes[i] : most;
     }
-    long gx = (most / 16 + 2047) / 2048;
-    gx = gx < 1 ? 1 : (gx > 1024 ? 1024 : gx);
-    hipLaunchKernelGGL(zero_many_kernel, dim3((unsigned)gx, n), dim3(256), 0, stream, z);
+    hipLaunchKernelGGL(zero_many_kernel, dim3((unsigned)zero_many_gx(most), n), dim3(256), 0, stream, z, bump);
     UNIVL_LAUNCH_CHECK();
     return UNIVL_OK;
 }
diff --git a/univl_amd/csrc/simloss.hip b/univl_amd/csrc/simloss.hip
--- a/univl_amd/csrc/simloss.hip
+++ b/univl_amd/csrc/simloss.hip
@@ -1,5 +1,6 @@
 #include "common.h"
 #include "univl_hip.h"
+#include "clear_body.h"
 
 namespace {
 
@@ -37,6 +38,7 @@
     return block_sum(w, red);
 }
 
+template <bool XC = false>
 __device__ __forceinline__ void pool_fwd_body(const UnivlPool& p, const int b, float* red, float* wts) {
     const int t = threadIdx.x;
     float acc[PC] = {0.f, 0.f, 0.f};
@@ -65,7 +67,8 @@
 #pragma unroll
     for (int j = 0; j < PC; ++j) {
         if (p.mean) p.mean[(long)b * PN + t + 256 * j] = acc[j];
-        p.out[(long)b * PN + t + 256 * j] = acc[j] * inv;
+        if (XC) __hip_atomic_store(p.out + (long)b * PN + t + 256 * j, acc[j] * inv, __ATOMIC_RELAXED, __HIP_MEMORY_SCOPE_AGENT);
+        else p.out[(long)b * PN + t + 256 * j] = acc[j] * inv;
     }
 }
 
@@ -148,7 +151,7 @@
         for (int s = 0; s < n; ++s) {
             const float w = mine[s] * inv_cnt;
 #pragma unroll
-            for (int j = 0; j < PC; ++j) dx[(long)s * PN + 256 * j] = d[j] * w;
+            for (int j = 0; j < PC; ++j) dx[(long)s * PN + 256 * j] = fmaf(d[j], w, 0.0f);
         }
     }
 }
@@ -168,19 +171,35 @@
     else pool_bwd_body(b, (int)blockIdx.x - a.B, blockIdx.y, red, wts, mine);
 }
 
-__global__ __launch_bounds__(256) void maxmargin_kernel(const float* x, int n, int ld, float margin, const float* w,
-                                                        float* loss, float* dx) {
-    extern __shared__ float diag_acc[];
-    __shared__ float red[4];
+struct ClearRide { ZeroList z; long zgx; int nz; float* table; long rows_total; const int64_t* list; const int* meta; int rows_gx; };
+
+__global__ __launch_bounds__(256) void pool_pair_bwd_clears_kernel(UnivlPool a, UnivlPool b, ClearRide c, int np) {
+    __shared__ float red[4];
+    __shared__ float wts[PCHUNK];
+    __shared__ float mine[PCHUNK];
+    const int id = blockIdx.x;
+    if (id < np) {
+        const int rows = a.B + b.B, r = id % rows, chunk = id / rows;
+        if (r < a.B) pool_bwd_body(a, r, chunk, red, wts, mine);
+        else pool_bwd_body(b, r - a.B, chunk, red, wts, mine);
+        return;
+    }
+    const long zid = id - np, nzb = c.zgx * c.nz;
+    if (zid < nzb) zero_many_body(c.z, zid % c.zgx, (int)(zid / c.zgx), c.zgx);
+    else rows_zero_body(c.table, c.rows_total, c.list, c.meta, zid - nzb, c.rows_gx);
+}
+
+__device__ __forceinline__ void maxmargin_body(const float* x, int ldx, int n, int ld, float margin, const float* w, float* loss,
+                                               float* dx, float* diag_acc, float* red) {
     const float inv = 1.0f / ((float)n * (float)n);
     for (int i = threadIdx.x; i < n; i += 256) diag_acc[i] = 0.f;
     __syncthreads();
     float acc = 0.f;
     for (int e = threadIdx.x; e < n * n; e += 256) {
         const int i = e / n, j = e % n;
-        const float v = x[(long)i * ld + j], wi = w ? w[e] : 1.0f;
-        const float a = margin + v - x[(long)i * ld + i];
-        const float b = margin + v - x[(long)j * ld + j];
+        const float v = x[(long)i * ldx + j], wi = w ? w[e] : 1.0f;
+        const float a = margin + v - x[(long)i * ldx + i];
+        const float b = margin + v - x[(long)j * ldx + j];
         float g = 0.f;
         if (a > 0.f) { acc += wi * a; g += wi; atomicAdd(&diag_acc[i], -wi); }
         if (b > 0.f) { acc += wi * b; g += wi; atomicAdd(&diag_acc[j], -wi); }
@@ -192,26 +211,36 @@
     for (int i = threadIdx.x; i < n; i += 256) dx[(long)i * ld + i] += diag_acc[i] * inv;
 }
 
-__global__ __launch_bounds__(256) void crossen_kernel(const float* x, int n, int ld, float* loss, float* dx) {
-    __shared__ float red[4];
+__global__ __launch_bounds__(256) void maxmargin_kernel(const float* x, int n, int ld, float margin, const float* w,
+                                                        float* loss, float* dx) {
+    extern __shared__ float diag_acc[];
+    __shared__ float red[4];
+    maxmargin_body(x, ld, n, ld, margin, w, loss, dx, diag_acc, red);
+}
+
+__device__ __forceinline__ void crossen_body(const float* x, int ldx, int n, int ld, float* loss, float* dx, float* red) {
     float total = 0.f;
     for (int i = 0; i < n; ++i) {
         float mx = -INFINITY;
-        for (int j = threadIdx.x; j < n; j += 256) mx = fmaxf(mx, x[(long)i * ld + j]);
+        for (int j = threadIdx.x; j < n; j += 256) mx = fmaxf(mx, x[(long)i * ldx + j]);
         mx = block_max(mx, red);
         float s = 0.f;
-        for (int j = threadIdx.x; j < n; j += 256) s += expf(x[(long)i * ld + j] - mx);
+        for (int j = threadIdx.x; j < n; j += 256) s += expf(x[(long)i * ldx + j] - mx);
         s = block_sum(s, red);
         const float lse = mx + logf(s);
-        total += lse - x[(long)i * ld + i];
+        total += lse - x[(long)i * ldx + i];
         for (int j = threadIdx.x; j < n; j += 256)
-            dx[(long)i * ld + j] = (expf(x[(long)i * ld + j] - lse) - (i == j ? 1.0f : 0.0f)) / (float)n;
+            dx[(long)i * ld + j] = (expf(x[(long)i * ldx + j] - lse) - (i == j ? 1.0f : 0.0f)) / (float)n;
     }
     if (threadIdx.x == 0) loss[0] = total / (float)n;
 }
 
-__global__ __launch_bounds__(256) void milnce_kernel(const float* x, int bs, int np, int ld, float* loss, float* dx) {
-    __shared__ float red[4];
+__global__ __launch_bounds__(256) void crossen_kernel(const float* x, int n, int ld, float* loss, float* dx) {
+    __shared__ float red[4];
+    crossen_body(x, ld, n, ld, loss, dx, red);
+}
+
+__device__ __forceinline__ void milnce_body(const float* x, int ldx, int bs, int np, int ld, float* loss, float* dx, float* red) {
     const int n = bs * np;
     for (int e = threadIdx.x; e < n * n; e += 256) dx[(long)(e / n) * ld + (e % n)] = 0.f;
     __syncthreads();
@@ -222,20 +251,20 @@
         float mx = -INFINITY;
         for (int j = threadIdx.x; j < 2 * n; j += 256) {
             float v;
-            if (j < n) v = x[(long)j * ld + i];
-            else { const int jj = j - n; v = (jj >= lo && jj < hi) ? -INFINITY : x[(long)i * ld + jj]; }
+            if (j < n) v = x[(long)j * ldx + i];
+            else { const int jj = j - n; v = (jj >= lo && jj < hi) ? -INFINITY : x[(long)i * ldx + jj]; }
             mx = fmaxf(mx, v);
         }
         mx = block_max(mx, red);
         float sden = 0.f, snum = 0.f;
         for (int j = threadIdx.x; j < 2 * n; j += 256) {
             if (j < n) {
-                const float e = expf(x[(long)j * ld + i] - mx);
+                const float e = expf(x[(long)j * ldx + i] - mx);
                 sden += e;
                 if (j >= lo && j < hi) snum += e;
             } else {
                 const int jj = j - n;
-                if (!(jj >= lo && jj < hi)) sden += expf(x[(long)i * ld + jj] - mx);
+                if (!(jj >= lo && jj < hi)) sden += expf(x[(long)i * ldx + jj] - mx);
             }
         }
         sden = block_sum(sden, red);
@@ -245,7 +274,7 @@
         __syncthreads();
         for (int j = threadIdx.x; j < 2 * n; j += 256) {
             if (j < n) {
-                const float e = expf(x[(long)j * ld + i] - mx);
+                const float e = expf(x[(long)j * ldx + i] - mx);
                 float g = e / sden;
                 if (j >= lo && j < hi) g -= e / snum;
                 dx[(long)j * ld + i] += wgt * g;
@@ -253,11 +282,70 @@
         }
         __syncthreads();
         for (int j = threadIdx.x; j < n; j += 256) {
-            if (!(j >= lo && j < hi)) dx[(long)i * ld + j] += wgt * expf(x[(long)i * ld + j] - mx) / sden;
+            if (!(j >= lo && j < hi)) dx[(long)i * ld + j] += wgt * expf(x[(long)i * ldx + j] - mx) / sden;
         }
         __syncthreads();
     }
     if (threadIdx.x == 0) loss[0] = total / (float)bs;
+}
+
+__global__ __launch_bounds__(256) void milnce_kernel(const float* x, int bs, int np, int ld, float* loss, float* dx) {
+    __shared__ float red[4];
+    milnce_body(x, ld, bs, np, ld, loss, dx, red);
+}
+
+constexpr int SIM_FOLD_MAX = 32;
+struct SimHead {
+    float* sim; float* dsim; float* loss; const float* weight; int* counter;
+    int n, ld, kind, n_pair; float margin;
+};
+
+__device__ __forceinline__ void sim_row_load(const float* base, int row, int lane, u32x4_t (&v)[PC]) {
+    const __amdgpu_buffer_rsrc_t rs = __builtin_amdgcn_make_buffer_rsrc(const_cast<float*>(base + (long)row * PN), 0, PN * 4, 0x00020000);
+#pragma unroll
+    for (int j = 0; j < PC; ++j) v[j] = __builtin_amdgcn_raw_buffer_load_b128(rs, (4 * lane + 256 * j) * 4, 0, 16);
+}
+
+__global__ __launch_bounds__(256) void pool_pair_sim_loss_kernel(UnivlPool a, UnivlPool b, SimHead h) {
+    __shared__ float red[4];
+    __shared__ float wts[PCHUNK];
+    __shared__ float sim_s[SIM_FOLD_MAX * SIM_FOLD_MAX];
+    __shared__ float diag[SIM_FOLD_MAX];
+    __shared__ int last;
+    if ((int)blockIdx.x < a.B) pool_fwd_body<true>(a, blockIdx.x, red, wts);
+    else pool_fwd_body<true>(b, (int)blockIdx.x - a.B, red, wts);
+    asm volatile("s_waitcnt vmcnt(0)" ::: "memory");
+    __syncthreads();
+    if (threadIdx.x == 0)
+        last = __hip_atomic_fetch_add(h.counter, 1, __ATOMIC_RELAXED, __HIP_MEMORY_SCOPE_AGENT) == a.B + b.B - 1 ? 1 : 0;
+    __syncthreads();
+    if (!last) return;
+    asm volatile("" ::: "memory");
+    const int lane = threadIdx.x & 63, wave = threadIdx.x >> 6, n = h.n;
+    for (int i = wave; i < n; i += 4) {
+        u32x4_t t[PC];
+        sim_row_load(a.out, i, lane, t);
+        for (int j0 = 0; j0 < n; j0 += 4) {
+            u32x4_t v[4][PC];
+#pragma unroll
+            for (int u = 0; u < 4; ++u) sim_row_load(b.out, min(j0 + u, n - 1), lane, v[u]);
+#pragma unroll
+            for (int u = 0; u < 4; ++u) {
+                float acc = 0.f;
+#pragma unroll
+                for (int q = 0; q < PC; ++q)
+#pragma unroll
+                    for (int e = 0; e < 4; ++e) acc = fmaf(__uint_as_float(t[q][e]), __uint_as_float(v[u][q][e]), acc);
+                acc = wave_sum(acc);
+                if (lane == 0 && j0 + u < n) { sim_s[i * n + j0 + u] = acc; h.sim[(long)i * h.ld + j0 + u] = acc; }
+            }
+        }
+    }
+    __syncthreads();
+    if (h.kind == 0) maxmargin_body(sim_s, n, n, h.ld, h.margin, h.weight, h.loss, h.dsim, diag, red);
+    else if (h.kind == 1) crossen_body(sim_s, n, n, h.ld, h.loss, h.dsim, red);
+    else milnce_body(sim_s, n, n / h.n_pair, h.n_pair, h.ld, h.loss, h.dsim, red);
+    if (threadIdx.x == 0) __hip_atomic_store(h.counter, 0, __ATOMIC_RELAXED, __HIP_MEMORY_SCOPE_AGENT);
 }
 
 __global__ void scale_dev_kernel(float* x, long n, const float* s) {
@@ -338,14 +426,58 @@
     return UNIVL_OK;
 }
 
-extern "C" int univl_pool_pair_bwd(const UnivlPool* a, const UnivlPool* b, hipStream_t stream) {
+extern "C" int univl_pool_pair_sim_loss(const UnivlPool* a, const UnivlPool* b, float* sim, float* dsim, int32_t ld, int32_t kind,
+                                        float margin, const float* weight, int32_t n_pair, float* loss, int32_t* counter,
+                                        hipStream_t stream) {
+    UNIVL_ON_STREAM_DEVICE(stream);
+    UNIVL_CHECK_ARG(a && b && a->N == 768 && b->N == 768 && a->B > 0 && b->B == a->B && a->S > 0 && b->S > 0 && a->x && b->x && a->out && b->out &&
+                        aligned16(a->out) && aligned16(b->out),
+                    UNIVL_EINVAL, "univl_pool_pair_sim_loss: bad pooling argument (N must be 768, both sides the same row count)");
+    UNIVL_CHECK_ARG(sim && dsim && loss && counter && ld >= a->B && kind >= UNIVL_SIM_MAXMARGIN && kind <= UNIVL_SIM_MILNCE &&
+                        (kind != UNIVL_SIM_MILNCE || (n_pair > 0 && a->B % n_pair == 0)),
+                    UNIVL_EINVAL, "univl_pool_pair_sim_loss: bad similarity / loss argument");
+    UNIVL_CHECK_ARG(a->B <= SIM_FOLD_MAX, UNIVL_EUNSUPPORTED, "univl_pool_pair_sim_loss: %d rows (one workgroup multiplies the whole matrix: up to %d)",
+                    a->B, SIM_FOLD_MAX);
+    SimHead h;
+    h.sim = sim; h.dsim = dsim; h.loss = loss; h.weight = kind == UNIVL_SIM_MAXMARGIN ? weight : nullptr; h.counter = counter;
+    h.n = a->B; h.ld = ld; h.kind = kind; h.n_pair = n_pair > 0 ? n_pair : 1; h.margin = margin;
+    hipLaunchKernelGGL(pool_pair_sim_loss_kernel, dim3(a->B + b->B), dim3(256), 0, stream, *a, *b, h);
+    UNIVL_LAUNCH_CHECK();
+    return UNIVL_OK;
+}
+
+extern "C" int univl_pool_pair_bwd(const UnivlPool* a, const UnivlPool* b, const UnivlClears* clears, hipStream_t stream) {
     UNIVL_ON_STREAM_DEVICE(stream);
     int rc = pool_bwd_check(a, "univl_pool_pair_bwd");
     if (rc) return rc;
     rc = pool_bwd_check(b, "univl_pool_pair_bwd");
     if (rc) return rc;
-    const int smax = a->S > b->S ? a->S : b->S;
-    hipLaunchKernelGGL(pool_pair_bwd_kernel, dim3(a->B + b->B, (smax + PCHUNK - 1) / PCHUNK), dim3(256), 0, stream, *a, *b);
+    const int smax = a->S > b->S ? a->S : b->S, chunks = (smax + PCHUNK - 1) / PCHUNK;
+    if (clears == nullptr || (clears->n_zero == 0 && clears->table == nullptr)) {
+        hipLaunchKernelGGL(pool_pair_bwd_kernel, dim3(a->B + b->B, chunks), dim3(256), 0, stream, *a, *b);
+        UNIVL_LAUNCH_CHECK();
+        return UNIVL_OK;
+    }
+    UNIVL_CHECK_ARG(clears->n_zero >= 0 && clears->n_zero <= UNIVL_ZERO_MAX, UNIVL_EINVAL, "univl_pool_pair_bwd: %d buffers to clear (0..%d)",
+                    clears->n_zero, UNIVL_ZERO_MAX);
+    UNIVL_CHECK_ARG(!clears->table || (clears->list && clears->meta && clears->rows_total > 0 && aligned16(clears->table)), UNIVL_EINVAL,
+                    "univl_pool_pair_bwd: bad row list");
+    ClearRide c;
+    long most = 0;
+    for (int i = 0; i < clears->n_zero; ++i) {
+        UNIVL_CHECK_ARG(clears->ptr[i] && clears->bytes[i] > 0 && aligned16(clears->ptr[i]), UNIVL_EALIGN,
+                        "univl_pool_pair_bwd: buffer %d to clear must be non-empty and 16-byte aligned", i);
+        c.z.ptr[i] = static_cast<unsigned char*>(clears->ptr[i]);
+        c.z.bytes[i] = clears->bytes[i];
+        most = clears->bytes[i] > most ? clears->bytes[i] : most;
+    }
+    c.nz = clears->n_zero;
+    c.zgx = zero_many_gx(most);
+    c.table = clears->table; c.rows_total = clears->rows_total; c.list = clears->list; c.meta = clears->meta;
+    c.rows_gx = clears->table ? 256 : 0;
+    const int np = (a->B + b->B) * chunks;
+    const long total = (long)np + c.zgx * c.nz + c.rows_gx;
+    hipLaunchKernelGGL(pool_pair_bwd_clears_kernel, dim3((unsigned)total), dim3(256), 0, stream, *a, *b, c, np);
     UNIVL_LAUNCH_CHECK();
     return UNIVL_OK;
 }
diff --git a/univl_amd/engine.py b/univl_amd/engine.py
--- a/univl_amd/engine.py
+++ b/univl_amd/engine.py
@@ -287,11 +287,12 @@
         self.descs[len(self.ops)] = [desc]
         self.ops.append(("call", fn, C.byref(desc), fn_name, stream))
 
-    def add_pair_call(self, fn_name, da, db, stream=0):
+    def add_pair_call(self, fn_name, da, db, stream=0, clears=None, keep=()):
         fn = getattr(_lib.lib(), fn_name)
-        self.keep += [da, db]
+        self.keep += [da, db, clears] + list(keep)
         self.descs[len(self.ops)] = [da, db]
-        self.ops.append(("call2", fn, (da, db), fn_name, stream))
+        arg = (da, db, clears) if fn_name == "univl_pool_pair_bwd" else (da, db)
+        self.ops.append(("call2", fn, arg, fn_name, stream))
 
     def add_gemm_group(self, descs, stream=0, max_blocks=0):
         fn = _lib.lib().univl_gemm_group_limited
@@ -331,10 +332,12 @@
         self.descs[len(self.ops)] = [dgrad, wgrad]
         self.ops.append(("pair_ln", _lib.lib().univl_gemm_pair_ln, (arr, ln_desc, counters), "univl_gemm_pair_ln", stream))
 
-    def add_zeros(self, tensors, stream=0):
+    def add_zeros(self, tensors, stream=0, bump=None):
         ts = [t for t in tensors if t is not None and t.numel() > 0]
         if ts:
-            self.add_callable(lambda: ops.zero_many(ts), stream)
+            self.add_callable(lambda: ops.zero_many(ts, bump), stream)
+        elif bump is not None:
+            self.add_callable(lambda: ops.bump_counter(bump), stream)
 
     def add_callable(self, f, stream=0, eager=False, with_streams=False):
         kind = "eager" if eager else ("pys" if with_streams else "py")
@@ -378,7 +381,10 @@
                 h = handles.get(sidx)
                 if h is None:
                     h = handles[sidx] = C.c_void_p(self._stream(sidx, cur).cuda_stream)
-                rc = a(C.byref(b[0]), C.byref(b[1]), h)
+                if len(b) == 2:
+                    rc = a(C.byref(b[0]), C.byref(b[1]), h)
+                else:
+                    rc = a(C.byref(b[0]), C.byref(b[1]), None if b[2] is None else C.byref(b[2]), h)
                 if rc != 0:
                     _lib.check(rc, name)
             elif kind == "group":
diff --git a/univl_amd/ops.py b/univl_amd/ops.py
--- a/univl_amd/ops.py
+++ b/univl_amd/ops.py
@@ -190,7 +190,7 @@
 
 def embed_text_desc(dtype, B, S, ids, word, pos, gamma, beta, *, type_ids=None, type_emb=None, eps=1e-12, y=None,
                     stats=None, out32=None, out16=None, p_post=0.0, seed=0, off_post=0, seed_dev=None, dout=None,
-                    dword=None, dpos=None, dtype_emb=None, dgamma=None, dbeta=None, drows=None, out16_lo=None):
+                    dword=None, dpos=None, dtype_emb=None, dgamma=None, dbeta=None, drows=None, out16_lo=None, rows=None):
     d = _lib.EmbedText()
     d.dtype, d.B, d.S, d.N = dtype, B, S, 768
     d.ids, d.type_ids = _p(ids), _p(type_ids)
@@ -201,6 +201,10 @@
     d.dout, d.dword, d.dpos, d.dtype_emb, d.dgamma, d.dbeta = _p(dout), _p(dword), _p(dpos), _p(dtype_emb), _p(dgamma), _p(dbeta)
     d.drows = _p(drows)
     d.out16_lo = _p(out16_lo)
+    if rows is not None:
+        lst, meta, reset, ever = rows
+        d.rows_list, d.rows_meta, d.rows_ever = _p(lst), _p(meta), _p(ever)
+        d.rows_total, d.rows_cap, d.rows_reset = (0 if ever is None else ever.numel()), lst.numel(), int(bool(reset))
     return d
 
 
@@ -241,8 +245,31 @@
     _lib.check(_lib.lib().univl_pool_pair_fwd(_BYREF(da), _BYREF(db), _stream()), "pool_pair_fwd")
 
 
-def pool_pair_bwd(da, db):
-    _lib.check(_lib.lib().univl_pool_pair_bwd(_BYREF(da), _BYREF(db), _stream()), "pool_pair_bwd")
+def clears_desc(zeros=(), rows=None):
+    c = _lib.Clears()
+    ts = [t for t in zeros if t is not None and t.numel() > 0]
+    assert len(ts) <= 16, "at most 16 buffers ride in one launch"
+    for i, t in enumerate(ts):
+        c.ptr[i], c.bytes[i] = t.data_ptr(), t.numel() * t.element_size()
+    c.n_zero = len(ts)
+    if rows is not None:
+        table, lst, meta = rows
+        c.table, c.rows_total, c.list, c.meta = _p(table), table.shape[0], _p(lst), _p(meta)
+    return c
+
+
+def pool_pair_bwd(da, db, clears=None):
+    _lib.check(_lib.lib().univl_pool_pair_bwd(_BYREF(da), _BYREF(db), None if clears is None else _BYREF(clears), _stream()), "pool_pair_bwd")
+
+
+def pool_pair_sim_loss(da, db, sim, dsim, kind, loss, counter, margin=0.0, weight=None, n_pair=1):
+    assert dsim.stride(0) == sim.stride(0)
+    rc = _lib.lib().univl_pool_pair_sim_loss(_BYREF(da), _BYREF(db), _p(sim), _p(dsim), sim.stride(0), _lib.SIM_KIND[kind], float(margin),
+                                             _p(weight), int(n_pair), _p(loss), _p(counter), _stream())
+    if rc == _lib.EUNSUPPORTED:
+        return False
+    _lib.check(rc, "pool_pair_sim_loss")
+    return True
 
 
 def maxmargin_loss(sim, margin, weight, loss, dsim):
@@ -265,14 +292,14 @@
     _lib.check(_lib.lib().univl_scale_by_device_scalar(_p(x), x.numel(), _p(s), _stream()), "scale_by_device_scalar")
 
 
-def zero_many(tensors):
+def zero_many(tensors, bump=None):
     import ctypes as C
     L = _lib.lib()
     for i in range(0, len(tensors), 16):
         ts = tensors[i:i + 16]
         ptrs = (C.c_void_p * len(ts))(*[t.data_ptr() for t in ts])
         sizes = (C.c_int64 * len(ts))(*[t.numel() * t.element_size() for t in ts])
-        _lib.check(L.univl_zero_many(ptrs, sizes, len(ts), _stream()), "zero_many")
+        _lib.check(L.univl_zero_many(ptrs, sizes, len(ts), _p(bump) if i == 0 else None, _stream()), "zero_many")
 
 
 def copy_many(pairs):
diff --git a/univl_amd/steps.py b/univl_amd/steps.py
--- a/univl_amd/steps.py
+++ b/univl_amd/steps.py
@@ -87,6 +87,7 @@
         self.dseq, self.dvis = e(self.Tt, H), e(self.Tv, H)
         self.de_op = e(self.Tv, H, dtype=ct)
         self.dvnorm = e(self.Tv, D)
+        self.sim_ctr = e(4, dtype=torch.int32)
         m = cx.model
         self.text = EncoderStack(fl, "bert", m.bert_config.num_hidden_layers, B, W, self.amask, cx.p, cx.seed_dev, cx.sites,
                                  s_main=s_text, s_side=s_text)
@@ -153,7 +154,9 @@
         W32, p, B, W, F, D, Tv = fl.w32, cx.p, self.B, self.W, self.F, self.D, self.Tv
         ST, SV = self.ST, self.SV
         both, stacks = self.branches == ("text", "vis"), [st for st in (self.text, self.vis) if st is not None]
-        fwd.add_zeros([st.yarena for st in stacks if st.zero_y] + [st.ln_ctr for st in stacks if st.ln_ctr is not None], ST)
+        fwd.add_zeros([st.yarena for st in stacks if st.zero_y] + [st.ln_ctr for st in stacks if st.ln_ctr is not None] +
+                      ([self.sim_ctr] if both and _ab.get("sim_fold") else []), ST,
+                      bump=getattr(self, "bump", None))
         if both:
             cx.stamp(fwd, "f_fork", ST)
             fwd.fork(ST, SV)
@@ -247,17 +250,19 @@
         gather = self._gather_dpos()
         if (sparse or gather) and getattr(self, "drows", None) is None:
             self.drows = cx.e(self.Tt, H)
+        rows = getattr(self, "word_rows", None) if not sparse else None
+        rows_in_embed = rows is not None and cx.red is None and bool(_ab.get("rows_append_in_embed"))
         bwd.add("univl_embed_text_bwd", ops.embed_text_desc(
             dt, B, W, self.ids, W32(n["bw"]), W32(n["bp"]), W32(n["blg"]), W32(n["blb"]), type_ids=self.type_ids,
             type_emb=W32(n["bt"]), y=self.te, stats=self.test, p_post=p, seed=cx.seed, off_post=self.off_t,
             seed_dev=cx.seed_dev, dout=dxt, dword=G(n["bw"]), dpos=None if gather else G(n["bp"]), dtype_emb=G(n["bt"]),
-            dgamma=G(n["blg"]), dbeta=G(n["blb"]), drows=self.drows if (sparse or gather) else None), ST)
+            dgamma=G(n["blg"]), dbeta=G(n["blb"]), drows=self.drows if (sparse or gather) else None,
+            rows=(rows[0], rows[1], rows[2], cx.fl.word_ever) if rows_in_embed else None), ST)
         if gather:
             bwd.add_callable(lambda: ops.rows_gather_sum(self.drows, W, G(n["bp"])[:W]), ST)
             if not sparse:
                 bwd.add_callable(lambda: ops.embed_scatter(self.ids.view(-1), self.drows, 1.0, G(n["bw"])), ST)
-        rows = getattr(self, "word_rows", None)
-        if rows is not None and not sparse:
+        if rows is not None and not rows_in_embed:
             lst, meta, reset = rows
             bwd.add_callable(lambda: ops.rows_append(self.ids.view(-1), lst, meta, reset, cx.fl.word_ever), ST)
 
@@ -303,11 +308,24 @@
         self.fused = bool(_ab.get("fused_sim")) and B <= 256
         self.lossfn = SimLoss(cx, loss_kind, B)
         self.loss = self.lossfn.loss
+        self.fold = (self.fused and cx.red is None and bool(_ab.get("sim_fold")) and B <= min(int(_ab.get("sim_fold_max_rows")), 32)
+                     and (loss_kind != "milnce" or B % cx.tc.n_pair == 0))
+        self.sim_ctr = enc.sim_ctr if self.fold else None
 
     def build_forward(self, fwd):
         enc, B = self.enc, self.enc.B
         dt_ = ops.pool_desc(B, enc.W, enc.seq_out, enc.amask, skip_first=True, normalize=self.norm, mean=self.tmean, out=self.tn)
         dv_ = ops.pool_desc(B, enc.F, enc.vis_out, enc.vmask, skip_first=False, normalize=self.norm, mean=self.vmean, out=self.vn)
+        if self.fold:
+            lf, tc = self.lossfn, self.cx.tc
+            sim, dsim, ctr = self.sim[:B], self.dsim[:B], self.sim_ctr
+
+            def univl_pool_pair_sim_loss():
+                if not ops.pool_pair_sim_loss(dt_, dv_, sim, dsim, lf.kind, lf.loss, ctr, margin=float(tc.margin), weight=lf.wts,
+                                              n_pair=tc.n_pair if lf.kind == "milnce" else 1):
+                    raise RuntimeError("univl_pool_pair_sim_loss refused %d rows (sim_fold_max_rows)" % B)
+            fwd.add_callable(univl_pool_pair_sim_loss)
+            return
         if self.fused:
             fwd.add_pair_call("univl_pool_pair_fwd", dt_, dv_)
         else:
@@ -316,15 +334,17 @@
         fwd.add("univl_gemm", _gemm_desc(_lib.DT_F32, self.tn, H, self.vn, H, B, B, H, out32=self.sim, ldc=self.ldp))
         self.lossfn.build(fwd, self.sim[:B], self.dsim[:B])
 
-    def build_backward(self, bwd, gout):
+    def build_backward(self, bwd, gout, clears=None, keep=(), accumulate=True):
         enc, B, ldp = self.enc, self.enc.B, self.ldp
+        assert self.fused or (clears is None and accumulate)
         if self.fused:
             bwd.add_pair_call(
                 "univl_pool_pair_bwd",
                 ops.pool_desc(B, enc.W, enc.seq_out, enc.amask, skip_first=True, normalize=self.norm, mean=self.tmean, out=self.tn,
-                              dx=enc.dseq, accumulate=True, dsim=self.dsim, other=self.vn, n_other=B, transpose=False, gscale=gout),
+                              dx=enc.dseq, accumulate=accumulate, dsim=self.dsim, other=self.vn, n_other=B, transpose=False, gscale=gout),
                 ops.pool_desc(B, enc.F, enc.vis_out, enc.vmask, skip_first=False, normalize=self.norm, mean=self.vmean, out=self.vn,
-                              dx=enc.dvis, accumulate=True, dsim=self.dsim, other=self.tn, n_other=B, transpose=True, gscale=gout))
+                              dx=enc.dvis, accumulate=accumulate, dsim=self.dsim, other=self.tn, n_other=B, transpose=True, gscale=gout),
+                clears=clears, keep=keep)
             return
         bwd.add_callable(lambda: ops.scale_by_device_scalar(self.dsim, gout))
         bwd.add("univl_gemm", _gemm_desc(_lib.DT_F32, self.dsim, ldp, self.vn, H, B, H, B, trans_b=1, out32=self.dtn, ldc=H))
@@ -725,7 +745,8 @@
     fwd.external = model._param_events
     fwd.wait_point("base")
     cx.stamp(fwd, "f_begin")
-    if cx.p > 0:
+    bump_in_clear = cx.p > 0 and cx.red is None and bool(_ab.get("bump_in_clear"))
+    if cx.p > 0 and not bump_in_clear:
         fwd.add_callable(lambda: ops.bump_counter(cx.seed_dev))
     branches = {"features_text": ("text",), "features_vis": ("vis",), "features_vis_shaped": ("vis",)}.get(kind, ("text", "vis"))
     st.enc = enc = EncoderPass(cx, B, W, F, normalized_input=kind in ("features_shaped", "features_vis_shaped"), branches=branches)
@@ -734,6 +755,8 @@
             enc.text.tail_key = ("layer", "cross", 0)
         if kind in ("caption", "pretrain") and model.decoder is not None:
             enc.vis.tail_key = ("layer", "decoder", 0)
+    if bump_in_clear:
+        enc.bump = cx.seed_dev
     enc.build_forward(fwd)
     st.fwd_encoders_len = len(fwd)
     stage_two = bool(model._stage_two)
@@ -806,15 +829,20 @@
                      and enc.Tt * (world if sparse else 1) <= fl.WORD_ROWS_CAP)
         zeros = [fl.sumsq, fl.partials] if fuse else []
         enc.word_rows = None
+        ride = (kind == "joint" and cx.red is None and st.joint is not None and st.joint.fused and bool(_ab.get("bwd_clears_ride")))
+        ride_rows = None
         if rows_mode:
             lst, meta = fl.word_rows()
             enc.word_rows = (lst, meta, fresh)
             if fresh:
                 zeros += fl.v_region_without_word_table()
-                bwd.add_callable(lambda: ops.rows_zero(fl.g(fl.WORD), lst, meta))
+                if ride:
+                    ride_rows = (fl.g(fl.WORD), lst, meta)
+                else:
+                    bwd.add_callable(lambda: ops.rows_zero(fl.g(fl.WORD), lst, meta))
         elif fresh:
             zeros.append(fl.g32[:fl.v_end])
-        zeros += enc.zero_list()
+        zeros += [z for z in enc.zero_list() if not (ride and (z is enc.dseq or z is enc.dvis))]
         if st.enc_m is not None:
             zeros += st.enc_m.zero_list()
         for r in (st.run_pairs, st.run_rows):
@@ -823,7 +851,12 @@
         if st.run_heads is not None:
             zeros.append(st.run_heads.dpostype)
         cx.stamp(bwd, "b_begin")
-        bwd.add_zeros(zeros)
+        ride_zeros = [z for z in zeros if z is not None and z.numel() > 0]
+        if ride and len(ride_zeros) > 16:
+            bwd.add_zeros(ride_zeros[16:])
+            ride_zeros = ride_zeros[:16]
+        if not ride:
+            bwd.add_zeros(zeros)
         g = st.gout
         if st.pooler is not None:
             st.pooler.build_backward(bwd, gs, g)
@@ -835,7 +868,11 @@
             st.heads.build_backward(bwd, gs, g)
             st.run_heads.build_backward(bwd, gs, hook_for(st.run_heads))
         if st.joint is not None:
-            st.joint.build_backward(bwd, g)
+            if ride:
+                st.joint.build_backward(bwd, g, clears=ops.clears_desc(ride_zeros, ride_rows), keep=ride_zeros + list(ride_rows or ()),
+                                        accumulate=False)
+            else:
+                st.joint.build_backward(bwd, g)
         if st.enc_m is not None:
             st.enc_m.build_backward(bwd, gs, None)
         enc.build_backward(bwd, gs, hook)
```

Result: no change. 1870 pairs/s, median of 6 (+0.5%).
